# rgoldade/GeometricMultigridPressureSolver

Measured on AMD Instinct MI355X. Metric: V-cycles/sec, higher is better.
Workload: dtype f32

## Files before the change

geometricmultigridpressuresolver_amd/csrc/mgps_internal.h:

```cpp
#pragma once

#include <cstdint>
#include <cstdlib>
#include <cstddef>
#include <memory>
#include <string>
#include <utility>
#include <vector>

#include "mgps.h"

namespace mgps {

constexpr int kTile = 16;

constexpr int kChunkCells = 1024;
constexpr int kWaveChunkCells = 256;
constexpr int kSegCells = 32;

void *hostBigAlloc(size_t bytes);
void hostBigFree(void *p);
void setHostBigAllocator(void *(*alloc)(size_t), void (*release)(void *));
constexpr size_t kBigBlockBytes = size_t(1) << 20;

// ... 60 lines not shown
constexpr int kBandMaxDepth = 4;
constexpr int kBoxMaxNodes = 8192;
constexpr int kBoxMaxList = 4096;
constexpr int kBoxThreads = 1024;
constexpr int kBoxSlots = kBoxMaxList / kBoxThreads;
constexpr int kBoxMaxGeneral = 384;
constexpr int kBoxInfoInts = 16;
enum BoxNode : uint8_t { kBoxSkip = 0, kBoxFrozen = 1, kBoxZero = 2, kBoxGeneral = 3, kBoxSimple = 4, kBoxFrozenOut = 11, kBoxFrozenFar = 12 };
struct BandBoxes {
    int depth = 0;
    RawVec<int32_t> info;
    RawVec<uint32_t> list;
    RawVec<int32_t> general;
    size_t groups() const { return info.size() / kBoxInfoInts; }
};
void buildBandBoxes(const HostLevel &L, int depth, BandBoxes &out);
struct BandBoxesDev {
    int depth = 0, ngroups = 0;
    int32_t *info = nullptr, *general = nullptr;
    uint32_t *list = nullptr;
    size_t listCount = 0, generalInts = 0;
    bool anyGeneral = false;
};
inline bool boxPlaneFits(const Dims &d) { return size_t(d.nx) * size_t(d.ny) < (size_t(1) << 24); }
int compactBandBoxLists(void *stream, int32_t *info, const uint32_t *list, int ngroups, uint32_t *listOut, size_t *newCount);
int orderBandBoxes(void *stream, const Dims &d, const int32_t *info, int ngroups, int32_t *infoOut);

void buildSlabLevel(const HostLevel &G, int z0, int z1, const float *wx, const float *wy, const float *wz,
                    HostLevel &L, const float *rowsIn = nullptr);
int launchBoundaryRows(void *stream, const Dims &d, const uint8_t *labels, const float *wx, const float *wy, const float *wz,
                       const int32_t *cells, int n, float *rows, int *violations);
void checkInteriorCells(const uint8_t *labels, int nx, int ny, int nz, int *pass);
int hierarchyCreate(mgps_hierarchy **out, int nx, int ny, int nz, const uint8_t *labels, int mg_levels,
                    const mgps_options *opt, bool forceCoarseSolver, bool requireShell, const int *window = nullptr);
void chunkListsFromFlags(HostLevel &L, const uint8_t *segAct, int64_t nseg);
constexpr int kRunSizes[4] = {kChunkCells, kWaveChunkCells, 64, kSegCells};
int chooseRunCells(const int64_t nAct[4]);
inline double runCostFactor(int cells) { return cells >= kChunkCells ? 1.0 : cells >= kWaveChunkCells ? 1.02 : cells >= 64 ? 1.13 : 1.22; }
void runListFromFlags(HostLevel &L, const uint8_t *runAct, int64_t nq, int runCells);
void tileListsFromKinds(HostLevel &L, const int64_t *kind, int tileZOffset);
void tileListsFromKinds(HostLevel &L, const int32_t *kind, int tileZOffset);
int hierarchyLight(mgps_hierarchy **out, int nx, int ny, int nz, int levels, const uint8_t *coarsestLabels, const mgps_options &o,
                   bool needCoarseSolver);
void setLastGlobalError(const std::string &msg);
const char *lastGlobalError();
int apiException(const mgps_solver *h) noexcept;
extern void (*gSetHandleError)(const mgps_solver *h, const char *msg) noexcept;
#define MGPS_API_CATCH(h) catch (...) { return ::mgps::apiException(h); }

struct GridP {
    int nx, ny, nz;
    const uint8_t *lab;
    const float *wx, *wy, *wz;
    const int32_t *bnd;
    const float *rows;
    int nbnd;
    const uint8_t *bandDiag;
    int ghostLo, ghostHi;
    const int32_t *chunks;
    int nchunks, chunkCells;
    const int32_t *planeBlocks;
    int nplaneBlocks, planeZc;
    int streaming;
    int sweepPath;
    int xlo, xhi;
    const uint32_t *plainQ;
    const unsigned long long *plainT;
};
inline size_t plainQuadWords(size_t cells) { return ((cells / 4 + 63) / 64) * 2; }
int launchPlainQuads(void *stream, const uint8_t *lab, int nx, int ny, int nz, uint32_t *plainQ, unsigned long long *plainT);
int launchActiveXRange(void *stream, const uint8_t *lab, int nx, size_t cells, int *range);

struct MixScale {
    const float *sigma = nullptr;
    float c1 = 1.f, c2 = 1.f;
};

constexpr int kPlaneCols = 256;
constexpr int kPlaneRows = 16;
constexpr size_t kPlaneSweepMinPlaneBytes = size_t(4) << 20;
constexpr int kSlabEdgePlanes = kBandMaxDepth + 1;
struct PlaneTiles {
    unsigned nbx, nby, nbz;
    constexpr size_t layer() const { return size_t(nbx) * nby; }
    constexpr size_t count() const { return layer() * nbz; }
    constexpr size_t index(int bx, int by, int bz) const { return (size_t(bz) * nby + size_t(by)) * nbx + size_t(bx); }
};
constexpr PlaneTiles planeTiles(int nx, int ny, int nz, int zc)
{
    return PlaneTiles{unsigned((nx + kPlaneCols - 1) / kPlaneCols), unsigned((ny + kPlaneRows - 1) / kPlaneRows), zc > 0 ? unsigned((nz + zc - 1) / zc) : 0u};
}
inline int planeSweepZc(int nx, int ny, int nz)
{
    if ((nx & 3) != 0 || nx < kPlaneCols || ny < kPlaneRows) return 0;
    int zc = 32;
    while (zc > 4 && planeTiles(nx, ny, nz, zc).count() < 1024) zc >>= 1;
    return zc;
}
struct SeamLayout {
    unsigned ny, nseam;
    constexpr size_t planeFloats() const { return size_t(ny) * nseam * 8u; }
    constexpr unsigned entry(unsigned j, unsigned s, unsigned side) const { return (j * nseam + (s - 1u)) * 8u + side * 4u; }
};
constexpr SeamLayout seamLayout(int nx, int ny) { return SeamLayout{unsigned(ny), planeTiles(nx, ny, 0, 0).nbx - 1u}; }

enum StencilOp { OP_JACOBI = 0, OP_RESIDUAL = 1, OP_APPLY = 2 };

size_t stencilSweptCells(const GridP &g);
int stencilKernelOf(const GridP &g);
int forcedStencilPath();
bool setupTimingOn();
bool hostSetupRequested(const mgps_options &o);
int launchStencil(void *stream, StencilOp op, const GridP &g, float *out, const float *x, const float *b, float omega,
                  bool skipInactive);
size_t applyDotPartialCount(const GridP &g);
int launchApplyDot(void *stream, const GridP &g, float *out, const float *x, double *partials, double *resultDev);
int launchBandJacobi(void *stream, const GridP &g, float *x, const float *b, const int32_t *band, int nband,
                     float *bandTmp, float omega, double *dotPartials = nullptr);
unsigned bandScatterBlocks(int nband);
int launchStencilDot(void *stream, StencilOp op, const GridP &g, float *out, const float *x, const float *b, float omega,
                     double *partials, unsigned *nparts);
int launchFoldDot(void *stream, double *partials, unsigned nparts, double *resultDev);
int launchBandBox(void *stream, const GridP &g, const BandBoxesDev &bx, bool closure, const void *src, const float *b, void *dst, void *snap,
                  float omega, bool half = false, const MixScale &ms = MixScale{}, double *dotPartials = nullptr, const void *dotOld = nullptr,
                  bool outClosure = false);
int launchStrokeFront(void *stream, const GridP &g, const BandBoxesDev &bx, float *out, const float *x, const float *b, float *snap, float omega, const uint32_t *keep);
int launchMarkClosure(void *stream, const GridP &g, const BandBoxesDev &bx, uint32_t *bits);
int launchBandBoxCopy(void *stream, const GridP &g, const BandBoxesDev &bx, const void *src, void *dst, bool half = false);
struct HaloList {
    float *buf = nullptr;
    const int32_t *idx = nullptr;
    int n = 0;
    ptrdiff_t base = 0;
};
int launchHaloListPack(void *stream, const HaloList &lo, const HaloList &hi, const float *a0, const float *a1);
int launchHaloListUnpack(void *stream, const HaloList &lo, const HaloList &hi, float *a0, float *a1);
int launchTiledGS(void *stream, const GridP &g, float *x, const float *b, const int32_t *pureTiles, int npure,
                  const int32_t *mixedTiles, int nmixed, const int32_t *tileBndStart, int forward, double *dotPartials = nullptr,
                  float *snap = nullptr, const uint8_t *snapTile = nullptr);
int launchMarkSnapTiles(void *stream, const GridP &g, const BandBoxesDev &bx, uint8_t *tiles);
int launchTiledGSMixed(void *stream, const GridP &g, void *xH, const float *b, const int32_t *pureTiles, int npure, const int32_t *mixedTiles, int nmixed,
                       const int32_t *tileBndStart, int forward, const MixScale &ms);
int launchPatchSimpleCodes(void *stream, uint8_t *codes, const int32_t *band, const uint8_t *bandDiag, int nbnd, int nband);
int launchRestrict(void *stream, const GridP &coarse, float *coarseOut, const float *fine);
bool residualRestrictFits(const GridP &fine, const GridP &coarse);
std::vector<int32_t> planeBlockEdges(const GridP &g, const std::vector<uint8_t> &flags);
bool residualRestrictXFolds(const GridP &fine);
size_t rzxFloats(const GridP &fine);
int launchResidualZ(void *stream, const GridP &fine, float *rz, const float *x, const float *b, const int32_t *edges, int nedges, const float *rEdge = nullptr,
                    bool xfold = false);
int launchRestrictY(void *stream, const GridP &coarse, float *coarseOut, const float *rzx, const GridP &fine);
int launchResidualEdgePlanes(void *stream, const GridP &g, float *r, const float *x, const float *b);
int launchRestrictXY(void *stream, const GridP &coarse, float *coarseOut, const float *rz);
bool mixedPrecisionShapeOk(int nx, int ny, int nz);
int launchStencilMixed(void *stream, StencilOp op, const GridP &g, void *outH, const void *xH, const float *b, float omega, const MixScale &ms,
                       double *dotPartials = nullptr, unsigned *nparts = nullptr);
int launchScaleResult(void *stream, double *resultDev, const float *sigmaDev, float mul);
int launchRestrictMixed(void *stream, const GridP &coarse, float *coarseOut, const void *fineH, float fm);
int launchProlongAddMixed(void *stream, const GridP &fine, void *fineH, const float *coarse, float pm);
int launchFromHalf(void *stream, float *dst, const void *srcH, const float *sigmaDev, float mul, size_t cells);
int launchMixSigma(void *stream, const double *maxAbsDev, float *sigmaDev);
int launchZeroActiveHalf(void *stream, const GridP &g, void *aH);
int launchProlongAdd(void *stream, const GridP &fine, float *fineInOut, const float *coarse, float *snap = nullptr, const uint8_t *snapTile = nullptr);
bool prolongJacobiPlaneFits(const GridP &g);
int launchProlongJacobi(void *stream, const GridP &g, float *out, const float *x, const float *b, const float *coarse, float omega);
int launchBandBoxClosureProlonged(void *stream, const GridP &g, const BandBoxesDev &bx, const float *src, const float *coarse, const float *b, float *snap,
                                  float omega);
size_t planeBlockCount(const GridP &g);
int launchPlaneBlockFlags(void *stream, const GridP &g, uint8_t *flags);
int launchCoarseAssemble(void *stream, int n, int nx, int ny, const int32_t *cells, const int32_t *index, const uint8_t *lab, double *A,
                         const uint8_t *pinned = nullptr);
int launchCoarseNarrow(void *stream, int n, const double *A, float *inv);
int launchCoarseInverseProject(void *stream, int n, float *inv, const int32_t *comp, int ncomp, const int32_t *counts, double *w, double *T);
int launchCoarseSolve(void *stream, int n, const float *inverse, const int32_t *cells, float *x, const float *b,
                      float *gathered);
int launchAxpy(void *stream, const GridP &g, float *dst, const float *src, const float *scaleDev, float scaleHost,
               float sign);
int launchXpay(void *stream, const GridP &g, float *dst, const float *a, const float *s, const float *scaleDev,
               float scaleHost);
int launchScale(void *stream, const GridP &g, float *v, float scale);
int launchDiagInverse(void *stream, const GridP &g, float *dinv);
int launchMulMasked(void *stream, const GridP &g, float *dst, const float *a, const float *b);
constexpr int kReducePartials = 2048;
int launchReduce(void *stream, int kind, const GridP &g, const float *a, const float *b, double *partials,
                 double *resultDev);
int launchCgUpdate(void *stream, const GridP &g, float *x, const float *p, float *r, const float *t, float alpha, double *partials,
                   double *resultDev, const double *alphaDev = nullptr, double *maxAbsDev = nullptr, double *xWide = nullptr, bool xFirst = false);
int launchHalfDot(void *stream, const GridP &g, const void *xH, const float *r, const float *sigmaDev, float mul, double *partials, double *resultDev);
int launchXpayHalf(void *stream, const GridP &g, float *p, const void *xH, const float *sigmaDev, float mul, const float *betaDev, float betaHost);
int launchCgScalars(void *stream, double *scal, float *beta, int init);
int launchStencil64(void *stream, int mode, const GridP &g, double *out, const double *x, const float *b, float *out32,
                    double *partials, size_t capacity, double *resultDev, const float *dx = nullptr);
int launchNarrowSum(void *stream, const GridP &g, float *x32, const double *x64, bool addDx);
int launchCgUpdate64(void *stream, const GridP &g, double *x, const double *p, double *r, const double *t, double alpha, float *r32,
                     double *partials, size_t capacity, double *resultDev);
int launchXpay64(void *stream, const GridP &g, double *p, const float *z, double beta, int first);
int launchWiden(void *stream, double *dst, const float *src, size_t n);
int launchNarrow(void *stream, float *dst, const double *src, size_t n);
int deviceAlloc(void **p, size_t bytes);
int deviceFree(void *p);
void deviceTrim();
struct SlabWindow {
    int own0 = 0, own1 = 0, need = 0;
};
struct WeightView {
    const float *w[3] = {nullptr, nullptr, nullptr}, *lo[3] = {nullptr, nullptr, nullptr}, *hi[3] = {nullptr, nullptr, nullptr};
    int nz = 0, gw = 0, k0 = 0;
};
int launchCoarsenLabels(void *stream, const Dims &fine, const uint8_t *fineLab, uint8_t *coarseLab, int *activeFlag);
int launchAnyActive(void *stream, const Dims &d, const uint8_t *lab, int *activeFlag);
size_t planeCountScratch(size_t plane, int planes);
int launchPlaneCounts(void *stream, const uint8_t *lab, size_t plane, int planes, uint32_t *partials, uint32_t *counts);
int launchShellCheck(void *stream, const Dims &d, const uint8_t *lab, int *badFlag);
int launchMarkBoundary(void *stream, const Dims &d, uint8_t *lab);
size_t scanScratchInts(size_t n);
int launchExclusiveScan(void *stream, const int32_t *in, int32_t *out, size_t n, int32_t *scratch);
int launchBandCandidates(void *stream, const Dims &d, const uint8_t *lab, int32_t *tileKind, uint8_t *tileBits, int32_t *flags, int32_t *rank,
                         int32_t *list, int32_t *scanScratch, const SlabWindow *win = nullptr);
int launchBandMasks(void *stream, const Dims &d, const uint8_t *lab, int width, uint32_t *mask, uint16_t *prefix, int32_t *tileCount, int32_t *tileKind,
                    int *interiorBad, const int32_t *tiles, int ntiles, const SlabWindow *win = nullptr);
int launchBandFill(void *stream, const Dims &d, const uint32_t *mask, const uint16_t *prefix, const int32_t *tileStart, int32_t *band);
int launchBandClassify(void *stream, const Dims &d, const uint8_t *lab, const float *wx, const float *wy, const float *wz, const int32_t *band, int n,
                       uint8_t *diagS, int32_t *general, int *violations);
int launchBandSplit(void *stream, const Dims &d, const uint8_t *lab, const float *wx, const float *wy, const float *wz, const int32_t *band, int n,
                    const uint8_t *diagS, const int32_t *genRank, int32_t *bandDev, uint8_t *bandDiag, int32_t *bandEntry, float *rows);
int launchBandClassify(void *stream, const Dims &d, const uint8_t *lab, const WeightView &wv, const int32_t *band, int n, uint8_t *diagS, int32_t *general,
                       int *violations, const SlabWindow *win);
int launchBandSplit(void *stream, const Dims &d, const uint8_t *lab, const WeightView &wv, const int32_t *band, int n, const uint8_t *diagS, const int32_t *genRank,
                    int32_t *bandDev, uint8_t *bandDiag, int32_t *bandEntry, float *rows);
int launchShellCheckSlab(void *stream, const Dims &d, const uint8_t *lab, bool zFaceLo, bool zFaceHi, int *badFlag);
int launchOwnedFlags(void *stream, const int32_t *band, const int32_t *general, int n, int32_t c0, int32_t c1, int32_t *own, int32_t *ownGen);
int launchBandSplitOwned(void *stream, const int32_t *band, int n, int32_t c0, const uint8_t *diagS, const int32_t *ownRank, const int32_t *ownGenRank,
                         const int32_t *genRank, const float *rowsAll, int32_t *bandOut, uint8_t *diagOut, float *rowsOut);
int launchHaloMark(void *stream, int nx, int ny, int nzOwn, int ghost, const int32_t *info, const uint32_t *list, int ngroups, uint8_t *lo, uint8_t *hi, int *broken);
int launchAddInt(void *stream, int32_t *out, const int32_t *in, int n, int32_t delta);
int launchRebaseBoxes(void *stream, int32_t *info, int ngroups, int32_t delta);
int launchCheckIndex(void *stream, const int32_t *idx, int n, int32_t limit, int *bad);
int launchGhostPlaneBlockFlags(void *stream, const Dims &d, const uint8_t *lab, int k, int zc, uint8_t *flags);
int launchGather(void *stream, const int32_t *rank, const int32_t *start, int n, int32_t *out);
int launchActivityFlags(void *stream, const Dims &d, const uint8_t *lab, uint8_t *chunkFlags, uint8_t *planeFlags, int zc);
int launchCountRuns(void *stream, const uint8_t *segFlags, size_t nseg, int *counts);
int launchFoldRunFlags(void *stream, const uint8_t *segFlags, size_t nseg, int runCells, uint8_t *runFlags);
int launchRunList(void *stream, const Dims &d, const uint8_t *runFlags, size_t nq, int runCells, int32_t *tmpFlags, int32_t *rank, int32_t *scanScratch,
                  int32_t *base, int32_t *list, int listLen);
int launchBandTileList(void *stream, const int32_t *tileStart, int nt, int32_t *flags, int32_t *rank, int32_t *list, int32_t *scanScratch);
int launchTileClassList(void *stream, const Dims &d, const int32_t *kind, int odd, int mixed, int32_t *flags, int32_t *rank, int32_t *list,
                        int32_t *scanScratch, int tkOffset = 0);
int launchByteList(void *stream, const uint8_t *bytes, int n, int32_t *flags, int32_t *rank, int32_t *list, int32_t *scanScratch);
int launchBoxTileList(void *stream, const Dims &d, const int32_t *tileStart, int32_t *flags, int32_t *rank, int32_t *list, int32_t *scanScratch);
int launchBandBoxesCount(void *stream, const Dims &d, const uint8_t *lab, const uint32_t *mask, const uint16_t *prefix, const int32_t *tileStart,
                         const int32_t *bandEntry, const uint8_t *bandDiag, int depth, const int32_t *tiles, int ntiles, int32_t *const counts[3], int *broken,
                         const SlabWindow *win = nullptr);
int launchBandBoxesFill(void *stream, const Dims &d, const uint8_t *lab, const uint32_t *mask, const uint16_t *prefix, const int32_t *tileStart,
                        const int32_t *bandEntry, const uint8_t *bandDiag, int depth, const int32_t *tiles, int ntiles, const int32_t *const at[3],
                        int32_t *info, uint32_t *list, int32_t *general, int *broken, const SlabWindow *win = nullptr);
int enclosedComponentsDevice(void *stream, const Dims &d, const uint8_t *codes, const float *wx, const float *wy, const float *wz, int32_t **cells,
                             int32_t **offsets, int64_t *m, int64_t *cellCount);
struct EncSlab {
    Dims d;
    int32_t base = 0;
    int32_t *parent = nullptr, *flag = nullptr, *pos = nullptr, *rootRank = nullptr, *scan = nullptr;
    uint8_t *open = nullptr, *touch = nullptr;
    int32_t *sendRoots = nullptr, *recvRoots = nullptr;
    unsigned long long *keys = nullptr, *keysSorted = nullptr;
    void *sortTemp = nullptr;
    size_t sortBytes = 0;
    int32_t *payload = nullptr;
    int32_t *candLocal = nullptr;
    int *bad = nullptr;
    int64_t ncand = 0, npairs = 0;
};
int encSlabLabel(void *stream, EncSlab &st, const uint8_t *codes, const float *wx, const float *wy, const float *wz, const uint8_t *labLo,
                 const uint8_t *labHi);
int encSlabCandidates(void *stream, EncSlab &st, const uint8_t *codes, const uint8_t *labHi, const float *wz, int32_t hiFirst, int *badHost);
int encSlabLists(void *stream, EncSlab &st, const int32_t *grank, int64_t m, int32_t **cells, int32_t **offsets, int64_t *cellCount);
void encSlabRelease(EncSlab &st);
constexpr int kEncChunkCells = 4096;
int launchEnclosedSums(void *stream, const float *v, const int32_t *cells, const int32_t *chunks, int nchunks, const int32_t *compChunk, int64_t m,
                       double *partials, double *sum);
int launchEnclosedSums64(void *stream, const double *v, const int32_t *cells, const int32_t *chunks, int nchunks, const int32_t *compChunk, int64_t m,
                         double *partials, double *sum);
int launchEnclosedSubtract(void *stream, float *v, const int32_t *cells, const int32_t *chunks, int nchunks, const int32_t *count, const double *sum);
int launchEnclosedSubtract64(void *stream, double *v, const int32_t *cells, const int32_t *chunks, int nchunks, const int32_t *count, const double *sum);
int launchEnclosedRanks(void *stream, int32_t *rank, const int32_t *cells, const int32_t *chunks, int nchunks);
int launchWidenAdd(void *stream, double *x64, const float *x32, size_t n);
int launchZero(void *stream, float *a, size_t count);
int launchZeroInactive(void *stream, const GridP &g, float *a);
int launchZeroActive(void *stream, const GridP &g, float *a, bool ghostPlanes = false);
int launchPack(void *stream, float *buf, const float *a, const int32_t *idx, int n);
int launchUnpack(void *stream, float *a, const float *buf, const int32_t *idx, int n);

}

struct mgps_coupling;
struct mgps_fields_slab;
namespace mgps {
void couplingExtents(const mgps_coupling *c, int e[3]);
bool couplingOnSlab(const mgps_coupling *c, int planes[2], int *rank, int *size);
constexpr int kCouplingCommFailed = -1;
int couplingApply64(mgps_coupling *c, void *stream, double *t, const double *p, double *dotDev);
int couplingResidual64(mgps_coupling *c, void *stream, double *r, const double *x, float *r32, double *norm2Dev);
int coupledSolveRefusal(mgps_solver *h, mgps_coupling *coupling, const char *fn);
bool fieldsSlabWindow(const mgps_fields_slab *d, const char *fn);
}

namespace mgps {
// ... 31 lines not shown
```

geometricmultigridpressuresolver_amd/csrc/mgps_kernels.hip:

```cpp
#include <hip/hip_runtime.h>
#include <hip/hip_fp16.h>

#include <algorithm>
#include <cstdlib>
#include <type_traits>

#include "mgps_internal.h"

namespace mgps {

namespace {

typedef float v4f __attribute__((ext_vector_type(4)));
typedef unsigned char v4b __attribute__((ext_vector_type(4)));
__device__ __forceinline__ float4 streamLoad4(const float *p)
{
    const v4f v = __builtin_nontemporal_load(reinterpret_cast<const v4f *>(p));
    return make_float4(v.x, v.y, v.z, v.w);
}
__device__ __forceinline__ uchar4 streamLoad4(const uint8_t *p)
{
    const v4b v = __builtin_nontemporal_load(reinterpret_cast<const v4b *>(p));
    return make_uchar4(v.x, v.y, v.z, v.w);
}
// ... 618 lines not shown
        lc = lcn;
        lcn = lcq;
        buf ^= 1;
    }
}

template <bool XF>
__global__ __launch_bounds__(64 * kPlaneRows, 8) void residualZKernel(GridP g, float *__restrict__ rz, const float *__restrict__ x,
                                                                     const float *__restrict__ b, unsigned nbx, unsigned nby, int zc,
                                                                     const int32_t *__restrict__ blocks, const float *__restrict__ rEdge,
                                                                     float *__restrict__ seam)
{
    __shared__ float plane[2][kPlaneBufFloats];
    const PlaneTile t = planeTile(g, nbx, nby, zc, blocks);
    const bool live = t.live, valid = t.valid, rowTop = t.rowTop, rowBot = t.rowBot, colL = t.colL, colR = t.colR;
    const size_t sz = size_t(t.sz);
    const int k0 = t.k0, k1 = t.k1;
    const int ks = max(k0 - 1, 0), ke = min(k1, g.nz - 1);
    const unsigned offL = unsigned(t.jc) * unsigned(g.nx) + unsigned(min(max(t.ic, g.xlo), max(g.xhi - 4, g.xlo)));
    float *const mine0 = plane[0] + (t.ty + 1) * kPlanePitch + 4 + t.lane * 4;
    const unsigned offHy = (rowTop && t.jc > 0) ? offL - unsigned(g.nx) : (rowBot && t.jc < g.ny - 1) ? offL + unsigned(g.nx) : offL;
    {
        const float4 xm = gLoad4(t.planeOf(x, ks - 1), offL);
        *reinterpret_cast<float4 *>(mine0 + kPlaneBufFloats) = keepIf(xm, live);
    }
    const float *xk = t.planeOf(x, ks);
    float4 xc = gLoad4(xk, offL);
    float4 xp = gLoad4(t.planeOf(x, ks + 1), offL);
    float4 hy = gLoad4(xk, offHy);
    const bool useHx = live && t.hasHx();
    const unsigned offHx = t.offHx(useHx, offL);
    float hx = gLoad1(xk, offHx);
    constexpr float w0 = 0.125f, w1 = 0.375f, w2 = 0.375f, w3 = 0.125f;
    float accPrev[4] = {0.f, 0.f, 0.f, 0.f}, accCur[4] = {0.f, 0.f, 0.f, 0.f};
    const unsigned rowX = t.rowS * (unsigned(g.nx) >> 1) + t.bx * 128u;
    const bool storeX = t.i < g.nx && t.j < g.ny && t.ic >= g.xlo - 4 && t.ic < g.xhi + 4;
    const bool seamL = colL && t.bx > 0, seamR = colR && t.i + 4 < g.nx;
    const bool seamW = valid && (seamL || seamR);
    const SeamLayout sl = seamLayout(g.nx, g.ny);
    auto storeFolded = [&](int K, bool nt) {
        const float4 v = keepIf(make_float4(accPrev[0], accPrev[1], accPrev[2], accPrev[3]), valid);
        storeXFolded(v, scalarBase(rz + size_t(K) * (sz >> 1)), rowX + 2u * laneHere(), storeX, nt, scalarBase(seam + size_t(K) * sl.planeFloats()),
                     colL ? sl.entry(t.rowS, t.bx, 1u) : sl.entry(t.rowS, t.bx + 1u, 0u), seamW);
    };
    if (rEdge && k0 == 0 && g.ghostLo) {
        const float4 e = gLoad4(scalarBase(rEdge - ptrdiff_t(sz)), offL);
        accCur[0] = w0 * e.x;
        accCur[1] = w0 * e.y;
        accCur[2] = w0 * e.z;
        accCur[3] = w0 * e.w;
    }
    const unsigned long long *const pt = g.plainT;
    unsigned long long pw = pt ? plainWord64(pt, t.plainIdx(ks)) : 0ull;
    int buf = 0;
    for (int k = ks; k <= ke; ++k) {
        float *me = mine0 + buf * kPlaneBufFloats;
        xc = keepIf(xc, live);
        stagePlane(me, t, xc, keepIf(hy, live), hx, useHx);
        const float *bk = t.planeOf(b, k);
        const uint8_t *lk = scalarBase(g.lab + size_t(k) * sz);
        const float *xn = t.planeOf(x, k + 1), *xq2 = t.planeOf(x, k + 2);
        unsigned lcw = 0u;
        if (!plainLane(pw)) lcw = gLoadCodesWnt(lk, offL);
        if (pt) pw = plainWord64(pt, t.plainIdx(min(k + 1, g.nz - 1)));
        const float4 bc = gLoad4nt(bk, offL);
        const float hxn = gLoad1(xn, offHx);
        float4 hyn = hy;
        if (rowTop || rowBot) hyn = gLoad4(xn, offHy);
        const float4 xq = gLoad4(xq2, offL);
        __syncthreads();
        const StagedPlane n = readStaged(me, mine0 + (buf ^ 1) * kPlaneBufFloats);
        float res[4];
        simpleQuad<OP_RESIDUAL>(n.xl, xc, n.xr, n.ym, n.yp, n.zm, xp, bc, lcw, 0.f, res);
        if (k & 1) {
#pragma unroll
            for (int e = 0; e < 4; ++e) {
                accPrev[e] = accCur[e] + w2 * res[e];
                accCur[e] = w0 * res[e];
            }
        } else {
#pragma unroll
            for (int e = 0; e < 4; ++e) {
                accPrev[e] += w3 * res[e];
                accCur[e] += w1 * res[e];
            }
            if (XF) {
                if (k >= k0 + 2) storeFolded((k >> 1) - 1, true);
            } else if (valid && k >= k0 + 2) {
                gStore4nt(scalarBase(rz + size_t((k >> 1) - 1) * sz), offL, make_float4(accPrev[0], accPrev[1], accPrev[2], accPrev[3]));
            }
        }
        xc = xp;
        xp = xq;
        hy = hyn;
        hx = hxn;
        buf ^= 1;
    }
    if (k1 == g.nz) {
        if (valid && rEdge && g.ghostHi) {
            const float4 e = gLoad4(scalarBase(rEdge + ptrdiff_t(g.nz) * ptrdiff_t(sz)), offL);
            accPrev[0] += w3 * e.x;
            accPrev[1] += w3 * e.y;
            accPrev[2] += w3 * e.z;
            accPrev[3] += w3 * e.w;
        }
        if (XF) storeFolded((g.nz >> 1) - 1, false);
        else if (valid) gStore4(rz + size_t((g.nz >> 1) - 1) * sz, offL, make_float4(accPrev[0], accPrev[1], accPrev[2], accPrev[3]));
    }
}

template <bool XF>
__global__ __launch_bounds__(64 * kPlaneRows) void residualZEdgeKernel(GridP g, float *__restrict__ rz, const float *__restrict__ x, const float *__restrict__ b,
                                                                      unsigned nbx, unsigned nby, int zc, const int32_t *__restrict__ edges,
                                                                      float *__restrict__ seam)
{
    const unsigned side = unsigned(edges[blockIdx.x]) & 1u;
    PlaneCoords t;
    planeCoords(t, g, unsigned(edges[blockIdx.x]) >> 1, nbx, nby, zc);
    const int lane = t.lane, i = t.i, j = t.j;
    const int k = side == 0 ? t.k0 - 1 : t.k1, K = side == 0 ? (t.k0 >> 1) : (t.k1 >> 1) - 1;
    const float wz = 0.125f;
    if (k < 0 || k >= g.nz) return;
    if (j >= g.ny) return;
    if (!XF && i >= g.nx) return;
    const bool live = i < g.nx && i >= g.xlo && i < g.xhi;
    const size_t sy = size_t(g.nx), sz = size_t(g.nx) * g.ny;
    const size_t c = size_t(k) * sz + size_t(j) * sy + i;
    const float4 zero4 = make_float4(0.f, 0.f, 0.f, 0.f);
    const size_t cym = j > 0 ? c - sy : c, cyp = j < g.ny - 1 ? c + sy : c, czm = k > 0 ? c - sz : c, czp = k < g.nz - 1 ? c + sz : c;
    const float4 xc = live ? *reinterpret_cast<const float4 *>(x + c) : zero4;
    const float4 ym = live ? *reinterpret_cast<const float4 *>(x + cym) : zero4, yp = live ? *reinterpret_cast<const float4 *>(x + cyp) : zero4;
    const float4 zm = live ? *reinterpret_cast<const float4 *>(x + czm) : zero4, zp = live ? *reinterpret_cast<const float4 *>(x + czp) : zero4;
    const float4 bc = live ? *reinterpret_cast<const float4 *>(b + c) : zero4;
    const unsigned labw = live ? *reinterpret_cast<const unsigned *>(g.lab + c) : 0x01010101u * unsigned(MGPS_EXTERIOR_CELL);
    float left = __shfl_up(xc.w, 1), right = __shfl_down(xc.x, 1);
    if (lane == 0) left = (live && i > 0) ? x[c - 1] : 0.f;
    if (lane == kWave - 1 || i + 4 >= g.nx) right = (live && i + 4 < g.nx) ? x[c + 4] : 0.f;
    if (!XF && !live) return;
    float res[4];
    simpleQuad<OP_RESIDUAL>(left, xc, right, ym, yp, zm, zp, bc, labw, 0.f, res);
    const float4 wr = make_float4(wz * res[0], wz * res[1], wz * res[2], wz * res[3]);
    if (!XF) {
        *reinterpret_cast<float4 *>(rz + size_t(K) * sz + size_t(j) * sy + i) = wr;
        return;
    }
    const bool seamL = lane == 0 && t.bx > 0, seamR = lane == kWave - 1 && i + 4 < g.nx;
    const SeamLayout sl = seamLayout(g.nx, g.ny);
    const unsigned offX = unsigned(j) * (unsigned(g.nx) >> 1) + (unsigned(i) >> 1);
    const unsigned seamOff = seamL ? sl.entry(unsigned(j), t.bx, 1u) : sl.entry(unsigned(j), t.bx + 1u, 0u);
    const bool storeX = i < g.nx && i >= g.xlo - 4 && i < g.xhi + 4, seamW = live && (seamL || seamR);
    storeXFolded(keepIf(wr, live), rz + size_t(K) * (sz >> 1), offX, storeX, false, seam + size_t(K) * sl.planeFloats(), seamOff, seamW);
}

template <int OP, bool DOT = false>
__global__ void stencilScalarKernel(GridP g, float *__restrict__ out, const float *__restrict__ x,
                                    const float *__restrict__ b, float omega, double *__restrict__ dotPartials = nullptr)
{
    const size_t n = size_t(g.nx) * g.ny * g.nz;
    const size_t c = size_t(blockIdx.x) * blockDim.x + threadIdx.x;
    double acc = 0.0;
    if (c < n) {
        const unsigned l = g.lab[c];
        const float xc = x[c];
        if (!simpleCell(l)) out[c] = inactiveValue<OP>(xc);
        else {
            const size_t sy = size_t(g.nx), sz = size_t(g.nx) * g.ny;
            const float diag = simpleDiag(l);
            const float lap = diag * xc - (x[c - 1] + x[c + 1] + x[c - sy] + x[c + sy] + x[c - sz] + x[c + sz]);
            const float bc = OP == OP_APPLY ? 0.f : b[c];
            const float res = epilogueRcp<OP>(xc, bc, lap, simpleRcp(diag), omega);
            out[c] = res;
            acc = dotTerm<OP>(xc, bc, res);
        }
    }
    if (DOT) blockDotStore(acc, dotPartials, blockIdx.x);
}

template <int OP, bool DOT = false, class TX = float>
__global__ void boundaryOpKernel(GridP g, TX *__restrict__ out, const TX *__restrict__ x,
                                 const float *__restrict__ b, float omega, unsigned nblocks, double *__restrict__ dotPartials = nullptr,
                                 MixScale ms = MixScale{})
{
    constexpr bool kMixed = !std::is_same<TX, float>::value;
    const unsigned block = remapBlock(blockIdx.x, nblocks);
    const int t = int(block * blockDim.x + threadIdx.x);
    double acc = 0.0;
    if (t < g.nbnd) {
        const size_t c = size_t(g.bnd[t]);
        float lap, diag;
        boundaryRow(g, [&](size_t p) { return Cell<TX>::load1(x + p); }, t, c, lap, diag);
        const float xc = Cell<TX>::load1(x + c), bc = OP == OP_APPLY ? 0.f : b[c];
        float res;
        if (kMixed) {
            const float bm = mixRhsScale(ms);
            res = OP == OP_JACOBI ? xc + omega * ((bm * bc - lap) / diag) : OP == OP_RESIDUAL ? bm * bc - ms.c2 * lap : lap;
        } else
            res = epilogue<OP>(xc, bc, lap, diag, omega);
        Cell<TX>::store1(out + c, res);
        acc = dotTerm<OP>(xc, bc, kMixed ? __half2float(toHalfSat(res)) : res);
    }
    if (DOT) blockDotStore(acc, dotPartials, blockIdx.x);
}

__global__ void bandComputeKernel(GridP g, const float *__restrict__ x, const float *__restrict__ b,
                                  const int32_t *__restrict__ band, int nband, float *__restrict__ tmp, float omega,
                                  unsigned nblocks)
{
    const unsigned block = remapBlock(blockIdx.x, nblocks);
    const int t = int(block * blockDim.x + threadIdx.x);
    if (t >= nband) return;
    const size_t c = size_t(band[t]);
    const size_t sy = size_t(g.nx), sz = size_t(g.nx) * g.ny;
    const float xc = x[c];
    float lap, diag;
    if (t >= g.nbnd) {
        diag = float(g.bandDiag[t]);
        lap = diag * xc - (x[c - 1] + x[c + 1] + x[c - sy] + x[c + sy] + x[c - sz] + x[c + sz]);
        tmp[t] = xc + omega * ((b[c] - lap) * simpleRcp(diag));
    } else {
        boundaryRow(g, [&](size_t p) { return x[p]; }, t, c, lap, diag);
        tmp[t] = xc + omega * ((b[c] - lap) / diag);
    }
}
template <bool DOT = false, class TX = float>
__global__ void bandScatterKernel(TX *__restrict__ x, const int32_t *__restrict__ band, int nband,
                                  const float *__restrict__ tmp, unsigned nblocks, const float *__restrict__ b = nullptr,
                                  double *__restrict__ dotPartials = nullptr)
{
    const int t = int(remapBlock(blockIdx.x, nblocks) * blockDim.x + threadIdx.x);
    double acc = 0.0;
    if (t < nband) {
        const int32_t c = band[t];
        const float v = tmp[t];
        if (DOT) {
            const float stored = std::is_same<TX, float>::value ? v : __half2float(toHalfSat(v));
            acc = (double(stored) - double(Cell<TX>::load1(x + c))) * double(b[c]);
        }
        Cell<TX>::store1(x + c, v);
    }
    if (DOT) blockDotStore(acc, dotPartials, blockIdx.x);
}

__device__ __forceinline__ bool boxBand(unsigned cls) { return cls >= kBoxGeneral && cls <= kBoxSimple + 6; }

template <class TX, bool CLOSURE, bool DOT, bool GEN, bool XZERO, bool PRO = false>
__device__ __forceinline__ void bandBoxBody(const GridP &g, const TX *__restrict__ src, const float *__restrict__ b, TX *dst,
                                            TX *__restrict__ snap, const int32_t *__restrict__ info, const uint32_t *__restrict__ list,
                                            const int32_t *__restrict__ general, float omega, int depth, const MixScale &ms,
                                            double *__restrict__ dotPartials, const TX *dotOld, int outClosure, unsigned group, unsigned slot,
                                            const float *__restrict__ coarse = nullptr)
{
    static_assert(!PRO || (CLOSURE && !XZERO && std::is_same<TX, float>::value), "the prolonged input: closure mode, fp32");
    constexpr bool kMixed = !std::is_same<TX, float>::value;
    constexpr int kGenRows = GEN ? kBoxMaxGeneral : 1;
    __shared__ __attribute__((aligned(16))) float val[2][kBoxMaxNodes];
    __shared__ float grow[7][kGenRows];
    __shared__ float gbv[kGenRows];
    __shared__ uint16_t gnode[kGenRows], gring[kGenRows];
    constexpr bool kStaged = PRO && !GEN;
    constexpr int kCoarseBoxWords = 2048, kCoarseSlots = kCoarseBoxWords / kBoxThreads;
    __shared__ float cbox[kStaged ? kCoarseBoxWords : 1];
    const int32_t *gip = info + kBoxInfoInts * size_t(group);
    int gi[kBoxInfoInts];
#pragma unroll
    for (int q = 0; q < kBoxInfoInts; ++q) gi[q] = __builtin_amdgcn_readfirstlane(gip[q]);
    const int rx = gi[1] & 255, ry = (gi[1] >> 8) & 255, sxy = rx * ry;
    const unsigned sy = unsigned(g.nx), sz = unsigned(g.nx) * unsigned(g.ny);
    const ptrdiff_t origin = gi[0];
    if (!XZERO) src += origin;
    b += origin;
    if (dst) dst += origin;
    if (CLOSURE && snap) snap += origin;
    if (DOT) dotOld += origin;
    const uint32_t *U = list + gi[2];
    const int ngen = GEN ? gi[5] : 0, nList = CLOSURE ? gi[7] : gi[3];
    const int H = depth + (CLOSURE ? 1 : 0);
    const float bm = kMixed ? mixRhsScale(ms) : 1.f;
    const int tid = threadIdx.x;
    auto nodeOf = [&](uint32_t e) { return int(__umul24((e >> 10) & 31u, unsigned(sxy)) + __umul24((e >> 5) & 31u, unsigned(rx)) + (e & 31u)); };
    auto cellOf = [&](uint32_t e) { return (e & 31u) + __umul24((e >> 5) & 31u, sy) + __umul24((e >> 10) & 31u, sz); };
    auto rd = [&](const TX *base, unsigned c) { return Cell<TX>::load1(reinterpret_cast<const TX *>(reinterpret_cast<const char *>(base) + c * unsigned(sizeof(TX)))); };
    auto rdf = [&](const float *base, unsigned c) { return *reinterpret_cast<const float *>(reinterpret_cast<const char *>(base) + c * 4u); };
    auto wr = [&](TX *base, unsigned c, float v) { Cell<TX>::store1(reinterpret_cast<TX *>(reinterpret_cast<char *>(base) + c * unsigned(sizeof(TX))), v); };
    int cbLo[3] = {0, 0, 0}, cbN[3] = {1, 1, 1};
    bool staged = false;
    if (kStaged) {
        const int o3[3] = {int(origin % g.nx), int((origin / g.nx) % g.ny), int(origin / sz)};
        const int r3[3] = {rx, ry, (gi[1] >> 16) & 255}, cn3[3] = {g.nx >> 1, g.ny >> 1, g.nz >> 1};
#pragma unroll
        for (int a = 0; a < 3; ++a) {
            cbLo[a] = min(max((o3[a] - 1) >> 1, 0), cn3[a] - 2);
            cbN[a] = min(max((o3[a] + r3[a] - 2) >> 1, 0), cn3[a] - 2) + 2 - cbLo[a];
        }
        staged = cbN[0] * cbN[1] * cbN[2] <= kCoarseBoxWords;
    }
    uint32_t ue[kBoxSlots];
    float bv[kBoxSlots];
    {
        float cv[kCoarseSlots];
        if (kStaged && staged) {
            const unsigned csy = unsigned(g.nx >> 1), csz = csy * unsigned(g.ny >> 1);
            const unsigned nxy = unsigned(cbN[0] * cbN[1]), nbox = nxy * unsigned(cbN[2]);
            const float *cb = scalarBase(coarse + (size_t(cbLo[2]) * csz + size_t(cbLo[1]) * csy + size_t(cbLo[0])));
#pragma unroll
            for (int m = 0; m < kCoarseSlots; ++m) {
                const unsigned q = unsigned(tid) + unsigned(m) * kBoxThreads, qq = q < nbox ? q : 0u;
// ... 1727 lines not shown
    return int(hipGetLastError());
}
__global__ __launch_bounds__(256) void zeroChunksHalfKernel(__half *__restrict__ a, const int32_t *__restrict__ chunks, int chunkCells, size_t nq)
{
    size_t q;
    if (!listQuad(chunks, chunkCells, blockIdx.x, q)) return;
    if (q < nq) reinterpret_cast<uint2 *>(a)[q] = make_uint2(0u, 0u);
}
int launchZeroActiveHalf(void *stream, const GridP &g, void *aH)
{
    const size_t n = size_t(g.nx) * g.ny * g.nz;
    if (!g.chunks || (n & 3) != 0) return int(hipMemsetAsync(aH, 0, n * sizeof(__half), static_cast<hipStream_t>(stream)));
    const unsigned nb = unsigned(g.nchunks) / unsigned(kChunkCells / g.chunkCells);
    if (nb > 0) zeroChunksHalfKernel<<<nb, 256, 0, static_cast<hipStream_t>(stream)>>>(static_cast<__half *>(aH), g.chunks, g.chunkCells, n >> 2);
    return int(hipGetLastError());
}

int launchTiledGS(void *stream, const GridP &g, float *x, const float *b, const int32_t *pureTiles, int npure,
                  const int32_t *mixedTiles, int nmixed, const int32_t *tileBndStart, int forward, double *dotPartials, float *snap, const uint8_t *snapTile)
{
    hipStream_t s = static_cast<hipStream_t>(stream);
    if (snap && !snapTile) return int(hipErrorInvalidValue);
    if (nmixed > 0 && npure > 0 && nmixed + npure <= 768) {
        if (dotPartials) tiledGSBothKernel<true><<<unsigned(nmixed + npure), 256, 0, s>>>(g, x, b, mixedTiles, nmixed, pureTiles, tileBndStart, forward, dotPartials, snap, snapTile);
        else tiledGSBothKernel<<<unsigned(nmixed + npure), 256, 0, s>>>(g, x, b, mixedTiles, nmixed, pureTiles, tileBndStart, forward, nullptr, snap, snapTile);
        return int(hipGetLastError());
    }
    if (dotPartials) {
        if (nmixed > 0) tiledGSMixedKernel<true><<<unsigned(nmixed), 256, 0, s>>>(g, x, b, mixedTiles, tileBndStart, forward, dotPartials, MixScale{}, snap, snapTile);
        if (npure > 0) tiledGSPureKernel<true><<<unsigned(npure), 256, 0, s>>>(g, x, b, pureTiles, forward, dotPartials + nmixed, MixScale{}, snap, snapTile);
        return int(hipGetLastError());
    }
    if (nmixed > 0) tiledGSMixedKernel<<<unsigned(nmixed), 256, 0, s>>>(g, x, b, mixedTiles, tileBndStart, forward, nullptr, MixScale{}, snap, snapTile);
    if (npure > 0) tiledGSPureKernel<<<unsigned(npure), 256, 0, s>>>(g, x, b, pureTiles, forward, nullptr, MixScale{}, snap, snapTile);
    return int(hipGetLastError());
}

int launchTiledGSMixed(void *stream, const GridP &g, void *xH, const float *b, const int32_t *pureTiles, int npure, const int32_t *mixedTiles, int nmixed,
                       const int32_t *tileBndStart, int forward, const MixScale &ms)
{
    hipStream_t s = static_cast<hipStream_t>(stream);
    __half *x = static_cast<__half *>(xH);
    if (nmixed > 0) tiledGSMixedKernel<false, __half><<<unsigned(nmixed), 256, 0, s>>>(g, x, b, mixedTiles, tileBndStart, forward, nullptr, ms);
    if (npure > 0) tiledGSPureKernel<false, __half><<<unsigned(npure), 256, 0, s>>>(g, x, b, pureTiles, forward, nullptr, ms);
    return int(hipGetLastError());
}

__global__ void patchSimpleCodesKernel(uint8_t *codes, const int32_t *band, const uint8_t *bandDiag, int nbnd, int nband)
{
    const int t = nbnd + int(blockIdx.x * blockDim.x + threadIdx.x);
    if (t >= nband) return;
    const int32_t c = band[t];
    if (codes[c] == MGPS_BOUNDARY_CELL) codes[c] = uint8_t(kCodeSimple + bandDiag[t]);
}

int launchPatchSimpleCodes(void *stream, uint8_t *codes, const int32_t *band, const uint8_t *bandDiag, int nbnd, int nband)
{
    if (nband > nbnd)
        patchSimpleCodesKernel<<<blocksFor(size_t(nband - nbnd), 256), 256, 0, static_cast<hipStream_t>(stream)>>>(codes, band, bandDiag, nbnd, nband);
    return int(hipGetLastError());
}

int launchRestrict(void *stream, const GridP &coarse, float *coarseOut, const float *fine)
{
    const size_t n = size_t(coarse.nx) * coarse.ny * coarse.nz;
    int kc = 16;
    const unsigned nbx = (coarse.nx + 63) / 64, nby = (coarse.ny + 7) / 8;
    while (kc > 4 && size_t(nbx) * nby * ((coarse.nz + kc - 1) / kc) < 8192) kc >>= 1;
    const unsigned nbz = (coarse.nz + kc - 1) / kc;
    const bool runsWin = coarse.chunks && double(coarse.nchunks) * coarse.chunkCells * 1.3 * runCostFactor(coarse.chunkCells) < 0.8 * double(n);
    if (!runsWin && coarse.nx >= 64 && coarse.nz >= kc && nbx * nby * nbz >= 2048u) {
        if ((coarse.nx & 1) == 0) restrictTileKernel<<<nbx * nby * nbz, 256, 0, static_cast<hipStream_t>(stream)>>>(coarse, coarseOut, fine, kc, nbx, nby);
        else restrictMarchKernel<<<nbx * nby * nbz, 256, 0, static_cast<hipStream_t>(stream)>>>(coarse, coarseOut, fine, kc, nbx, nby);
        return int(hipGetLastError());
    }
    const unsigned nb = coarse.chunks ? unsigned(size_t(coarse.nchunks) * size_t(coarse.chunkCells) / 256) : blocksFor(n, 256);
    if (nb > 0) restrictKernel<<<nb, 256, 0, static_cast<hipStream_t>(stream)>>>(coarse, coarseOut, fine);
    return int(hipGetLastError());
}

bool residualRestrictFits(const GridP &fine, const GridP &coarse)
{
    return fine.planeZc >= 4 && (fine.planeZc & 1) == 0 && (fine.nz & 1) == 0 && coarse.nx >= 64 && (coarse.nx & 1) == 0 && 2 * coarse.nx == fine.nx &&
           2 * coarse.ny == fine.ny && 2 * coarse.nz == fine.nz;
}
std::vector<int32_t> planeBlockEdges(const GridP &g, const std::vector<uint8_t> &flags)
{
    const int zc = g.planeZc > 0 ? g.planeZc : 1;
    const PlaneTiles pt = planeTiles(g.nx, g.ny, g.nz, zc);
    const size_t layer = pt.layer(), nbz = pt.nbz;
    std::vector<int32_t> edges;
    for (size_t bid = 0; bid < flags.size() && bid < layer * nbz; ++bid) {
        if (flags[bid]) continue;
        const size_t bz = bid / layer;
        if (bz > 0 && flags[bid - layer]) edges.push_back(int32_t(2 * bid));
        if (bz + 1 < nbz && flags[bid + layer]) edges.push_back(int32_t(2 * bid + 1));
    }
    return edges;
}
int launchResidualEdgePlanes(void *stream, const GridP &g, float *r, const float *x, const float *b)
{
    const size_t sz = size_t(g.nx) * g.ny;
    for (int side = 0; side < 2; ++side) {
        if (!(side == 0 ? g.ghostLo : g.ghostHi)) continue;
        const int k = side == 0 ? 0 : g.nz - 1;
        GridP p = g;
        p.nz = 1;
        p.lab = g.lab + size_t(k) * sz;
        p.plainQ = nullptr;
        p.plainT = nullptr;
        p.ghostLo = (k > 0 || g.ghostLo) ? 1 : 0;
        p.ghostHi = (k < g.nz - 1 || g.ghostHi) ? 1 : 0;
        p.chunks = nullptr;
        p.nchunks = 0;
        p.planeBlocks = nullptr;
        p.nplaneBlocks = 0;
        p.planeZc = 0;
        p.sweepPath = 1;
        p.nbnd = 0;
        p.streaming = 0;
        const int e = launchStencil(stream, OP_RESIDUAL, p, r + size_t(k) * sz, x + size_t(k) * sz, b + size_t(k) * sz, 0.f, true);
        if (e) return e;
    }
    if (g.nbnd > 0) {
        const unsigned nb = blocksFor(size_t(g.nbnd), 256);
        boundaryOpKernel<OP_RESIDUAL><<<nb, 256, 0, static_cast<hipStream_t>(stream)>>>(g, r, x, b, 0.f, nb);
    }
    return int(hipGetLastError());
}
bool residualRestrictXFolds(const GridP &fine) { return fine.nbnd == 0; }
static size_t rzxGridFloats(const GridP &fine) { return (size_t(fine.nx) * fine.ny * fine.nz / 4 + 3) & ~size_t(3); }
size_t rzxFloats(const GridP &fine) { return rzxGridFloats(fine) + size_t(fine.nz / 2) * seamLayout(fine.nx, fine.ny).planeFloats(); }
int launchResidualZ(void *stream, const GridP &fine, float *rz, const float *x, const float *b, const int32_t *edges, int nedges, const float *rEdge, bool xfold)
{
    if (xfold && fine.nbnd > 0) return int(hipErrorInvalidValue);
    const int zc = fine.planeZc;
    const PlaneTiles pt = planeTiles(fine.nx, fine.ny, fine.nz, zc);
    const unsigned nbx = pt.nbx, nby = pt.nby;
    hipStream_t s = static_cast<hipStream_t>(stream);
    const bool list = fine.planeBlocks != nullptr;
    const unsigned nb = list ? unsigned(fine.nplaneBlocks) : unsigned(pt.count());
    if (xfold) {
        float *seam = rz + rzxGridFloats(fine);
        if (nb > 0) residualZKernel<true><<<nb, 64 * kPlaneRows, 0, s>>>(fine, rz, x, b, nbx, nby, zc, list ? fine.planeBlocks : nullptr, rEdge, seam);
        if (list && nedges > 0) residualZEdgeKernel<true><<<unsigned(nedges), 64 * kPlaneRows, 0, s>>>(fine, rz, x, b, nbx, nby, zc, edges, seam);
        return int(hipGetLastError());
    }
    if (nb > 0) residualZKernel<false><<<nb, 64 * kPlaneRows, 0, s>>>(fine, rz, x, b, nbx, nby, zc, list ? fine.planeBlocks : nullptr, rEdge, nullptr);
    if (list && nedges > 0) residualZEdgeKernel<false><<<unsigned(nedges), 64 * kPlaneRows, 0, s>>>(fine, rz, x, b, nbx, nby, zc, edges, nullptr);
    if (fine.nbnd > 0)
        for (int phase = 0; phase < 4; ++phase) residualZGeneralKernel<<<blocksFor(size_t(fine.nbnd), 256), 256, 0, s>>>(fine, rz, x, b, phase);
    return int(hipGetLastError());
}
int launchRestrictXY(void *stream, const GridP &coarse, float *coarseOut, const float *rz)
{
    int kc = 16;
    const unsigned nbx = (coarse.nx + kRtI - 1) / kRtI, nby = (coarse.ny + kRtJ - 1) / kRtJ;
    while (kc > 1 && size_t(nbx) * nby * ((coarse.nz + kc - 1) / kc) < 8192) kc >>= 1;
    const unsigned nbz = (coarse.nz + kc - 1) / kc;
    restrictXYKernel<<<nbx * nby * nbz, 256, 0, static_cast<hipStream_t>(stream)>>>(coarse, coarseOut, rz, kc, nbx, nby);
    return int(hipGetLastError());
}

int launchRestrictY(void *stream, const GridP &coarse, float *coarseOut, const float *rzx, const GridP &fine)
{
    int kc = 16;
    const unsigned nbx = (coarse.nx + kRyI - 1) / kRyI, nby = (coarse.ny + kRyJ - 1) / kRyJ;
    while (kc > 1 && size_t(nbx) * nby * ((coarse.nz + kc - 1) / kc) < 8192) kc >>= 1;
    const unsigned nbz = (coarse.nz + kc - 1) / kc;
    restrictYKernel<<<nbx * nby * nbz, 256, 0, static_cast<hipStream_t>(stream)>>>(coarse, coarseOut, rzx, rzx + rzxGridFloats(fine), kc, nbx, nby);
    return int(hipGetLastError());
}

int launchRestrictMixed(void *stream, const GridP &coarse, float *coarseOut, const void *fineH, float fm)
{
    const __half *fine = static_cast<const __half *>(fineH);
    const size_t n = size_t(coarse.nx) * coarse.ny * coarse.nz;
    const int kc = 16;
    const unsigned nbx = (coarse.nx + 63) / 64, nby = (coarse.ny + 7) / 8, nbz = (coarse.nz + kc - 1) / kc;
    const bool runsWin = coarse.chunks && double(coarse.nchunks) * coarse.chunkCells * 1.3 * runCostFactor(coarse.chunkCells) < 0.8 * double(n);
    if (!runsWin && coarse.nx >= 64 && coarse.nz >= kc && nbx * nby * nbz >= 2048u) {
        restrictMarchKernel<__half><<<nbx * nby * nbz, 256, 0, static_cast<hipStream_t>(stream)>>>(coarse, coarseOut, fine, kc, nbx, nby, fm);
        return int(hipGetLastError());
    }
    const unsigned nb = coarse.chunks ? unsigned(size_t(coarse.nchunks) * size_t(coarse.chunkCells) / 256) : blocksFor(n, 256);
    if (nb > 0) restrictKernel<__half><<<nb, 256, 0, static_cast<hipStream_t>(stream)>>>(coarse, coarseOut, fine, fm);
    return int(hipGetLastError());
}

int launchProlongAddMixed(void *stream, const GridP &fine, void *fineH, const float *coarse, float pm)
{
    const int npj = fine.ny / 2 - 1;
    const int kp0 = 0, kp1 = fine.nz / 2 - 2;
    const size_t total = size_t(fine.nx >> 2) * npj * size_t(std::max(kp1 - kp0 + 1, 0));
    const unsigned nb = blocksFor(total, 256);
    if (nb > 0)
        prolongAddBlockKernel<__half><<<nb, 256, 0, static_cast<hipStream_t>(stream)>>>(fine, static_cast<__half *>(fineH), coarse, nb, npj, kp0, total, pm);
    return int(hipGetLastError());
}
bool mixedPrecisionShapeOk(int nx, int ny, int nz) { return (nx & 3) == 0 && nx >= 8 && (ny & 1) == 0 && (nz & 1) == 0 && ny >= 4 && nz >= 2; }

int launchProlongAdd(void *stream, const GridP &fine, float *fineInOut, const float *coarse, float *snap, const uint8_t *snapTile)
{
    if (snap && !snapTile) return int(hipErrorInvalidValue);
    const size_t n = size_t(fine.nx) * fine.ny * fine.nz;
    const bool runsWin = fine.chunks && double(fine.nchunks) * fine.chunkCells * 3.4 * runCostFactor(fine.chunkCells) < 0.8 * double(n);
    if (!runsWin && (fine.nx & 3) == 0 && fine.nx >= 8 && (fine.ny & 1) == 0 && (fine.nz & 1) == 0 && fine.ny >= 4 && fine.nz >= 2) {
        const int npj = fine.ny / 2 - 1;
        const int kp0 = fine.ghostLo ? -1 : 0, kp1 = fine.ghostHi ? fine.nz / 2 - 1 : fine.nz / 2 - 2;
        const size_t total = size_t(fine.nx >> 2) * npj * size_t(std::max(kp1 - kp0 + 1, 0));
        const unsigned nb = blocksFor(total, 256);
        if (nb > 0)
            prolongAddBlockKernel<<<nb, 256, 0, static_cast<hipStream_t>(stream)>>>(fine, fineInOut, coarse, nb, npj, kp0, total, 1.f, snap, snapTile);
    } else if ((fine.nx & 3) == 0 && fine.nx >= 8) {
        const unsigned nb = fine.chunks ? unsigned(fine.nchunks) / unsigned(kChunkCells / fine.chunkCells) : blocksFor(n >> 2, 256);
        if (nb > 0) prolongAddQuadKernel<<<nb, 256, 0, static_cast<hipStream_t>(stream)>>>(fine, fineInOut, coarse, nb, snap, snapTile);
    } else
        prolongAddKernel<<<blocksFor(n, 256), 256, 0, static_cast<hipStream_t>(stream)>>>(fine, fineInOut, coarse, snap, snapTile);
    return int(hipGetLastError());
}

bool prolongJacobiPlaneFits(const GridP &g)
{
    return g.planeZc > 0 && (g.planeZc & 1) == 0 && (g.nx & 3) == 0 && g.nx >= 8 && (g.ny & 1) == 0 && (g.nz & 1) == 0 && g.ny >= 4 && g.nz >= 4 &&
           !g.ghostLo && !g.ghostHi;
}
int launchProlongJacobi(void *stream, const GridP &g, float *out, const float *x, const float *b, const float *coarse, float omega)
{
    if (!prolongJacobiPlaneFits(g) || !out || !x || !coarse || out == x || g.nbnd > 0) return int(hipErrorInvalidValue);
    const int zc = g.planeZc;
    const PlaneTiles pt = planeTiles(g.nx, g.ny, g.nz, zc);
    const unsigned nb = g.planeBlocks ? unsigned(g.nplaneBlocks) : unsigned(pt.count());
    if (nb > 0) prolongJacobiPlaneKernel<<<nb, 64 * kPlaneRows, 0, static_cast<hipStream_t>(stream)>>>(g, out, x, b, coarse, omega, pt.nbx, pt.nby, zc, g.planeBlocks);
    return int(hipGetLastError());
}

__global__ __launch_bounds__(256) void planeBlockFlagsKernel(const int32_t *__restrict__ blocks, int n, uint8_t *__restrict__ flags)
{
    const int t = int(blockIdx.x * blockDim.x + threadIdx.x);
    if (t < n) flags[blocks[t]] = 1;
}
size_t planeBlockCount(const GridP &g)
{
    return planeTiles(g.nx, g.ny, g.nz, g.planeZc > 0 ? g.planeZc : 1).count();
}
int launchPlaneBlockFlags(void *stream, const GridP &g, uint8_t *flags)
{
    if (!g.planeBlocks || g.nplaneBlocks <= 0) return 0;
    planeBlockFlagsKernel<<<blocksFor(size_t(g.nplaneBlocks), 256), 256, 0, static_cast<hipStream_t>(stream)>>>(g.planeBlocks, g.nplaneBlocks, flags);
    return int(hipGetLastError());
}

__global__ __launch_bounds__(256) void coarseAssembleKernel(int n, int nx, int ny, const int32_t *__restrict__ cells, const int32_t *__restrict__ index,
                                                            const uint8_t *__restrict__ lab, const uint8_t *__restrict__ pinned, double *__restrict__ A)
{
    const int r = int(blockIdx.x * blockDim.x + threadIdx.x);
    if (r >= n) return;
    if (pinned && pinned[r]) {
        A[size_t(r) * n + r] = 1.0;
        return;
    }
    const ptrdiff_t c = cells[r], off[6] = {-1, 1, -ptrdiff_t(nx), ptrdiff_t(nx), -ptrdiff_t(nx) * ny, ptrdiff_t(nx) * ny};
    double diag = 0.0;
#pragma unroll
    for (int q = 0; q < 6; ++q) {
        const unsigned l = lab[c + off[q]];
        if (activeLabel(l)) {
            const int32_t u = index[c + off[q]];
            if (!(pinned && pinned[u])) A[size_t(r) * n + u] = -1.0;
            diag += 1.0;
        } else if (l == MGPS_DIRICHLET_CELL)
            diag += 1.0;
    }
    A[size_t(r) * n + r] = diag;
}
__global__ __launch_bounds__(256) void coarseNarrowKernel(int n, const double *__restrict__ A, float *__restrict__ inv)
{
    const size_t t = blockIdx.x * size_t(blockDim.x) + threadIdx.x;
    if (t >= size_t(n) * n) return;
    const size_t r = t / n, c = t - r * n;
    inv[t] = float(r <= c ? A[t] : A[c * n + r]);
}
int launchCoarseAssemble(void *stream, int n, int nx, int ny, const int32_t *cells, const int32_t *index, const uint8_t *lab, double *A, const uint8_t *pinned)
{
    coarseAssembleKernel<<<blocksFor(size_t(n), 256), 256, 0, static_cast<hipStream_t>(stream)>>>(n, nx, ny, cells, index, lab, pinned, A);
    return int(hipGetLastError());
}
__global__ __launch_bounds__(256) void coarseProjRowKernel(int n, const float *__restrict__ inv, const int32_t *__restrict__ comp,
                                                           const int32_t *__restrict__ counts, double *__restrict__ w)
{
    const int row = blockIdx.x * (blockDim.x / kWave) + threadIdx.x / kWave;
    const int lane = threadIdx.x & (kWave - 1);
    if (row >= n) return;
    const int c = comp[row];
    double acc = 0.0;
    if (c >= 0)
        for (int k = lane; k < n; k += kWave)
            if (comp[k] == c) acc += double(inv[size_t(row) * n + k]);
#pragma unroll
    for (int off = kWave / 2; off > 0; off >>= 1) acc += __shfl_down(acc, off);
    if (lane == 0) w[row] = c >= 0 ? acc / double(counts[c]) : 0.0;
}
__global__ __launch_bounds__(64) void coarseProjMeanKernel(int n, int ncomp, const int32_t *__restrict__ comp, const int32_t *__restrict__ counts,
                                                          const double *__restrict__ w, double *__restrict__ T)
{
    const int c = blockIdx.x * blockDim.x + threadIdx.x;
// ... 778 lines not shown
```

geometricmultigridpressuresolver_amd/csrc/mgps_solver.hip:

```cpp
#include <hip/hip_runtime.h>

#include <dlfcn.h>

#include <algorithm>
#include <chrono>
#include <cmath>
#include <cstdio>
#include <cstring>
#include <functional>
#include <limits>
#include <string>
#include <atomic>
#include <mutex>
#include <thread>
#include <unordered_map>
#include <map>
#include <memory>
#include <vector>

#include "mgps_fields.h"
#include "mgps_internal.h"

using namespace mgps;

namespace {
inline hipError_t cacheMalloc(void **p, size_t bytes) { return hipError_t(mgps::deviceAlloc(p, bytes)); }
inline hipError_t cacheFree(void *p) { return hipError_t(mgps::deviceFree(p)); }
}

namespace {

struct DevLevel {
    Dims d;
    GridP g{};
    uint8_t *codes = nullptr;
    float *x = nullptr, *b = nullptr;
    float *r = nullptr, *tmp = nullptr;
    int32_t *band = nullptr;
    int nband = 0;
    int nbndGeneral = 0;
    float *bandTmp = nullptr;
    float *rows = nullptr;
    uint8_t *bandDiag = nullptr;
    int32_t *pure[2] = {nullptr, nullptr}, *mixed[2] = {nullptr, nullptr};
    int npure[2] = {0, 0}, nmixed[2] = {0, 0};
    int32_t *tileBndStart = nullptr;
    int z0 = 0, z1 = 0;
    int32_t *bandPlane[4] = {nullptr, nullptr, nullptr, nullptr};
    int nbandPlane[4] = {0, 0, 0, 0};
    float *packBuf[4] = {nullptr, nullptr, nullptr, nullptr};
    int32_t *chunks = nullptr, *planeBlocks = nullptr;
    int edgeChunks = 0, edgePlaneBlocks = 0;
    BandBoxesDev bandBoxes;
    uint8_t *planeFlags = nullptr;
    int32_t *rzEdges = nullptr;
    int nrzEdges = 0;
    float *rz = nullptr;
    uint8_t *snapTile = nullptr;
    uint32_t *keepBits = nullptr;
    struct BoxHalo {
        int32_t *sendIdx[2] = {nullptr, nullptr}, *recvIdx[2] = {nullptr, nullptr};
        int nsend[2] = {0, 0}, nrecv[2] = {0, 0};
        float *sendBuf[2] = {nullptr, nullptr}, *recvBuf[2] = {nullptr, nullptr};
    } halo;
    bool boxForm = false;
    bool hasBandPlanes = false;
    GridP gBox{};
    float *extRows = nullptr;
    uint32_t *plainQ = nullptr;
    unsigned long long *plainT = nullptr;
    int elo = 0;
};

}

struct mgps_solver {
    mgps_hierarchy *hier = nullptr;
    std::vector<mgps_hierarchy *> retiredHier;
    mgps_options opt{};
    bool useGS = false;
    int device = 0;
    hipStream_t stream = nullptr;
    std::vector<DevLevel> lv;
    float *w[3] = {nullptr, nullptr, nullptr};
    bool weightsBorrowed = false;
    int cn = 0;
    float *cinv = nullptr, *cvec = nullptr;
    std::shared_ptr<void> cinvShared;
    int32_t *ccells = nullptr;
    bool tailOfSlabRun = false;
    double *partials = nullptr, *resultDev = nullptr, *resultHost = nullptr;
    double *dotPartials = nullptr;
    double *cg64[4] = {nullptr, nullptr, nullptr, nullptr};
    mgps_coupling *coupling = nullptr;
    bool gatherDot = false;
    unsigned dotUsed = 0;
    size_t dotCapacity = 0;
    double *dotTarget = nullptr;
    double *cgScal = nullptr;
    float *pcg[4] = {nullptr, nullptr, nullptr, nullptr};
    float *dinv = nullptr;
    void *mixX = nullptr, *mixTmp = nullptr, *mixR = nullptr;
    float *mixSigma = nullptr;
    int mixExp = 0;
    double *mixMax = nullptr;
    void *mixResult = nullptr;
    std::vector<void *> userGrids;
    int ghost = 1;
    bool dist = false;
    mgps_comm comm{};
    int64_t exchanges = 0;
    std::vector<int> splits;
    int distLevels = 0;
    int totalLevels = 0;
    int requestedLevels = 0;
    mgps_solver *tail = nullptr;
    float *tailX = nullptr, *tailB = nullptr;
    bool profiling = false;
    bool stageProfiling = false;
    std::vector<hipEvent_t> profEvents;
    size_t profUsed = 0;
    int profSweeps = 0;
    struct StageMark {
        int stage, level;
    };
    std::vector<StageMark> stageMarks;
    std::vector<hipEvent_t> stageEvents;
    double stageMs[6] = {0, 0, 0, 0, 0, 0};
    double stageMsFine[6] = {0, 0, 0, 0, 0, 0};
    double stageMsFineLast[6] = {0, 0, 0, 0, 0, 0};
    int stageCycles = 0;
    int64_t encM = 0, encCells = 0;
    int32_t *encCellList = nullptr, *encOffsets = nullptr, *encChunks = nullptr, *encCompChunk = nullptr, *encCount = nullptr;
    std::vector<int32_t> encCountHost;
    int encNChunks = 0;
    double *encPartials = nullptr, *encSum = nullptr;
    std::vector<double> encSumHost;
    float *encB = nullptr;
    std::string lastError = "";
};

namespace {
void setHandleError(const mgps_solver *h, const char *msg) noexcept
{
    try {
        const_cast<mgps_solver *>(h)->lastError = msg;
    } catch (...) {
    }
}
const bool handleErrorHookInstalled = [] {
    mgps::gSetHandleError = setHandleError;
    return true;
}();
}

namespace {

int failH(mgps_solver *h, int code, const std::string &msg)
{
    static std::mutex guard;
    std::lock_guard<std::mutex> lock(guard);
    if (h) h->lastError = msg;
    else setLastGlobalError(msg);
    return code;
}

#define MGPS_HIP(h, call)                                                                                 \
    do {                                                                                                  \
        hipError_t e_ = (call);                                                                           \
        if (e_ != hipSuccess)                                                                             \
            return failH(h, MGPS_ERR_HIP, std::string(#call) + ": " + hipGetErrorString(e_));             \
    } while (0)
#define MGPS_LAUNCH(h, call)                                                                              \
    do {                                                                                                  \
        int e_ = (call);                                                                                  \
        if (e_ != 0)                                                                                      \
            return failH(h, MGPS_ERR_HIP, std::string(#call) + ": " + hipGetErrorString(hipError_t(e_))); \
    } while (0)
#define MGPS_TRY(call)                \
    do {                              \
        int s_ = (call);              \
        if (s_ != MGPS_OK) return s_; \
    } while (0)
#define MGPS_COMM(h, call)                                                           \
    do {                                                                             \
        int s_ = (call);                                                             \
        if (s_ != 0) return failH(h, MGPS_ERR_COMM, std::string(#call) + " failed"); \
    } while (0)
#define MGPS_COUPLE(h, call)                                                                                                     \
    do {                                                                                                                         \
        int e_ = (call);                                                                                                         \
        if (e_ == mgps::kCouplingCommFailed) return failH(h, MGPS_ERR_COMM, std::string(#call) + ": the all-reduce of g failed"); \
        if (e_ != 0) return failH(h, MGPS_ERR_HIP, std::string(#call) + ": " + hipGetErrorString(hipError_t(e_)));              \
    } while (0)


struct DeviceCache {
    struct Block {
        void *p;
        uint64_t age;
    };
    using FreeMap = std::multimap<std::pair<int, size_t>, Block>;
    std::mutex guard;
    FreeMap free;
    std::unordered_map<void *, std::pair<int, size_t>> live;
    uint64_t clock = 0;
    struct PerDevice {
        size_t cached = 0, cap = 0;
        bool capKnown = false;
        std::map<uint64_t, FreeMap::iterator> byAge;
    };
    std::map<int, PerDevice> dev;
// ... 47 lines not shown
        const auto it = c.free.find({dev, want});
        if (it != c.free.end()) {
            *p = it->second.p;
            D.cached -= want;
            D.byAge.erase(it->second.age);
            c.free.erase(it);
            return hipSuccess;
        }
    }
    if (needCap) {
        const size_t cap = deviceCapOfCurrent();
        std::lock_guard<std::mutex> lock(c.guard);
        DeviceCache::PerDevice &D = c.dev[dev];
        if (!D.capKnown) {
            D.cap = cap;
            D.capKnown = true;
        }
    }
    hipError_t e = hipMalloc(p, want);
    if (e != hipSuccess) {
        (void)hipGetLastError();
        std::vector<void *> drop;
        {
            std::lock_guard<std::mutex> lock(c.guard);
            deviceTrimLocked(c, drop);
        }
        for (void *b : drop) (void)hipFree(b);
        e = hipMalloc(p, want);
    }
    if (e != hipSuccess) return int(e);
    std::lock_guard<std::mutex> lock(c.guard);
    c.live[*p] = {dev, want};
    return hipSuccess;
}
int deviceFree(void *p)
{
    if (!p) return hipSuccess;
    DeviceCache &c = deviceCache();
    std::vector<void *> drop;
    {
        std::lock_guard<std::mutex> lock(c.guard);
        const auto it = c.live.find(p);
        if (it == c.live.end()) drop.push_back(p);
        else {
            DeviceCache::PerDevice &D = c.dev[it->second.first];
            if (it->second.second > D.cap) {
                c.live.erase(it);
                drop.push_back(p);
            } else {
                const uint64_t age = c.clock++;
                D.byAge[age] = c.free.emplace(it->second, DeviceCache::Block{p, age});
                D.cached += it->second.second;
                while (D.cached > D.cap && !D.byAge.empty()) {
                    const auto oldest = D.byAge.begin()->second;
                    drop.push_back(oldest->second.p);
                    D.cached -= oldest->first.second;
                    c.live.erase(oldest->second.p);
                    c.free.erase(oldest);
                    D.byAge.erase(D.byAge.begin());
                }
            }
        }
    }
    hipError_t e = hipSuccess;
    for (void *b : drop) {
        const hipError_t eb = hipFree(b);
        if (eb != hipSuccess) e = eb;
    }
    return int(e);
}
void deviceTrim()
{
    DeviceCache &c = deviceCache();
    std::vector<void *> drop;
    {
        std::lock_guard<std::mutex> lock(c.guard);
        deviceTrimLocked(c, drop);
    }
    for (void *b : drop) (void)hipFree(b);
}
}
namespace {

template <class T>
int devAlloc(mgps_solver *h, T **p, size_t count, bool zero)
{
    *p = nullptr;
    if (count == 0) count = 1;
    hipError_t e = cacheMalloc(reinterpret_cast<void **>(p), count * sizeof(T));
    if (e != hipSuccess) return failH(h, MGPS_ERR_ALLOC, std::string("hipMalloc: ") + hipGetErrorString(e));
    if (zero) MGPS_HIP(h, hipMemsetAsync(*p, 0, count * sizeof(T), h->stream));
    return MGPS_OK;
}

template <class T, class A>
int devUpload(mgps_solver *h, T **p, const std::vector<T, A> &v)
{
    MGPS_TRY(devAlloc(h, p, v.size(), false));
    if (!v.empty()) MGPS_HIP(h, hipMemcpy(*p, v.data(), v.size() * sizeof(T), hipMemcpyHostToDevice));
    return MGPS_OK;
}

int gridAlloc(mgps_solver *h, float **p, const Dims &d)
{
    const size_t plane = size_t(d.nx) * d.ny;
    float *base = nullptr;
    MGPS_TRY(devAlloc(h, &base, (size_t(d.nz) + 2 * size_t(h->ghost)) * plane, true));
    *p = base + size_t(h->ghost) * plane;
    return MGPS_OK;
}
void gridFree(const mgps_solver *h, float *p, const Dims &d)
{
    if (p) (void)cacheFree(p - size_t(h->ghost) * size_t(d.nx) * d.ny);
}

void freeAll(mgps_solver *h)
{
    if (!h) return;
    (void)hipSetDevice(h->device);
    (void)hipDeviceSynchronize();
    if (h->tail) freeAll(h->tail);
    for (auto &L : h->lv) {
        (void)cacheFree(L.codes);
        gridFree(h, L.x, L.d);
        gridFree(h, L.b, L.d);
        gridFree(h, L.r, L.d);
        gridFree(h, L.tmp, L.d);
        (void)cacheFree(L.band);
        (void)cacheFree(L.bandTmp);
        (void)cacheFree(L.rows);
        (void)cacheFree(L.bandDiag);
        for (int c = 0; c < 2; ++c) {
            (void)cacheFree(L.pure[c]);
            (void)cacheFree(L.mixed[c]);
        }
        (void)cacheFree(L.tileBndStart);
        for (int q = 0; q < 4; ++q) {
            (void)cacheFree(L.bandPlane[q]);
            (void)cacheFree(L.packBuf[q]);
        }
        (void)cacheFree(L.chunks);
        (void)cacheFree(L.planeBlocks);
        for (int q = 0; q < 2; ++q) {
            (void)cacheFree(L.halo.sendIdx[q]);
            (void)cacheFree(L.halo.recvIdx[q]);
            (void)cacheFree(L.halo.sendBuf[q]);
            (void)cacheFree(L.halo.recvBuf[q]);
        }
        (void)cacheFree(L.extRows);
        (void)cacheFree(L.bandBoxes.info);
        (void)cacheFree(L.bandBoxes.list);
        (void)cacheFree(L.planeFlags);
        (void)cacheFree(L.keepBits);
        (void)cacheFree(L.snapTile);
        (void)cacheFree(L.rz);
        (void)cacheFree(L.rzEdges);
        (void)cacheFree(L.bandBoxes.general);
        (void)cacheFree(L.plainQ);
        (void)cacheFree(L.plainT);
    }
    for (int a = 0; a < 3 && !h->weightsBorrowed; ++a) (void)cacheFree(h->w[a]);
    if (!h->cinvShared) (void)cacheFree(h->cinv);
    (void)cacheFree(h->cvec);
    (void)cacheFree(h->ccells);
    (void)cacheFree(h->partials);
    (void)cacheFree(h->resultDev);
    (void)cacheFree(h->dotPartials);
    (void)cacheFree(h->cgScal);
    (void)cacheFree(h->mixX);
    (void)cacheFree(h->mixTmp);
    (void)cacheFree(h->mixR);
    (void)cacheFree(h->mixSigma);
    (void)cacheFree(h->mixMax);
    for (double *g64 : h->cg64)
        if (g64) (void)cacheFree(g64 - size_t(h->lv[0].d.nx) * h->lv[0].d.ny);
    if (h->resultHost) (void)hipHostFree(h->resultHost);
    if (!h->lv.empty()) {
        for (int q = 0; q < 4; ++q) gridFree(h, h->pcg[q], h->lv[0].d);
        gridFree(h, h->dinv, h->lv[0].d);
    }
    for (void *p : {(void *)h->encCellList, (void *)h->encOffsets, (void *)h->encChunks, (void *)h->encCompChunk, (void *)h->encPartials, (void *)h->encSum, (void *)h->encCount})
        (void)cacheFree(p);
    if (!h->lv.empty()) gridFree(h, h->encB, h->lv[0].d);
    for (void *p : h->userGrids) (void)cacheFree(p);
    for (hipEvent_t e : h->profEvents) (void)hipEventDestroy(e);
    for (hipEvent_t e : h->stageEvents) (void)hipEventDestroy(e);
    mgps_hierarchy_destroy(h->hier);
    for (mgps_hierarchy *r : h->retiredHier) mgps_hierarchy_destroy(r);
    delete h;
}

int checkLevel(mgps_solver *h, int level, const char *who)
{
    if (!h) return failH(nullptr, MGPS_ERR_INVALID_ARGUMENT, std::string(who) + ": NULL handle");
    if (level < 0 || level >= int(h->lv.size()))
        return failH(h, MGPS_ERR_INVALID_ARGUMENT, std::string(who) + ": level out of range");
    (void)hipSetDevice(h->device);
    return MGPS_OK;
}


enum GhostMode { GHOST_NONE = 0, GHOST_FULL = 1, GHOST_BAND = 2 };

int exchangeGhosts(mgps_solver *h, int l, float *a, GhostMode mode = GHOST_FULL, hipStream_t on = nullptr)
{
    if (!h->dist || mode == GHOST_NONE) return MGPS_OK;
    DevLevel &L = h->lv[l];
    const size_t plane = size_t(L.d.nx) * L.d.ny;
    const bool lo = h->comm.rank > 0, hi = h->comm.rank < h->comm.size - 1;
    if (mode == GHOST_BAND && !L.hasBandPlanes) mode = GHOST_FULL;
    if (mode == GHOST_FULL) {
        const size_t bytes = plane * sizeof(float);
        ++h->exchanges;
        MGPS_COMM(h, h->comm.exchange(h->comm.user, lo ? a : nullptr, bytes, lo ? a - plane : nullptr, bytes,
                                      hi ? a + (size_t(L.d.nz) - 1) * plane : nullptr, bytes,
                                      hi ? a + size_t(L.d.nz) * plane : nullptr, bytes, on ? on : h->stream));
        return MGPS_OK;
    }
    const int *n = L.nbandPlane;
    if (lo) MGPS_LAUNCH(h, launchPack(h->stream, L.packBuf[0], a, L.bandPlane[0], n[0]));
    if (hi) MGPS_LAUNCH(h, launchPack(h->stream, L.packBuf[2], a, L.bandPlane[2], n[2]));
    ++h->exchanges;
    MGPS_COMM(h, h->comm.exchange(h->comm.user, lo ? L.packBuf[0] : nullptr, size_t(n[0]) * sizeof(float),
                                  lo ? L.packBuf[1] : nullptr, size_t(n[1]) * sizeof(float),
                                  hi ? L.packBuf[2] : nullptr, size_t(n[2]) * sizeof(float),
                                  hi ? L.packBuf[3] : nullptr, size_t(n[3]) * sizeof(float), h->stream));
    if (lo) MGPS_LAUNCH(h, launchUnpack(h->stream, a, L.packBuf[1], L.bandPlane[1], n[1]));
    if (hi) MGPS_LAUNCH(h, launchUnpack(h->stream, a, L.packBuf[3], L.bandPlane[3], n[3]));
    return MGPS_OK;
}


int haloListExchange(mgps_solver *h, int l, float *a0, float *a1, bool withPlane)
{
    DevLevel &L = h->lv[l];
    DevLevel::BoxHalo &H = L.halo;
    const size_t plane = size_t(L.d.nx) * L.d.ny, G = size_t(h->ghost);
    const bool lo = h->comm.rank > 0, hi = h->comm.rank < h->comm.size - 1;
    if (!lo && !hi) return MGPS_OK;
    const size_t per = a1 ? 2 : 1;
    HaloList sLo, sHi, rLo, rHi;
    if (lo) {
        sLo = HaloList{H.sendBuf[0], H.sendIdx[0], H.nsend[0], 0};
        rLo = HaloList{H.recvBuf[0], H.recvIdx[0], H.nrecv[0], -ptrdiff_t(G * plane)};
    }
    if (hi) {
        sHi = HaloList{H.sendBuf[1], H.sendIdx[1], H.nsend[1], 0};
        rHi = HaloList{H.recvBuf[1], H.recvIdx[1], H.nrecv[1], ptrdiff_t(size_t(L.d.nz) * plane)};
    }
    MGPS_LAUNCH(h, launchHaloListPack(h->stream, sLo, sHi, a0, a1));
    const size_t pb = plane * sizeof(float);
    const size_t sb[2] = {size_t(H.nsend[0]) * per * sizeof(float), size_t(H.nsend[1]) * per * sizeof(float)};
    const size_t rb[2] = {size_t(H.nrecv[0]) * per * sizeof(float), size_t(H.nrecv[1]) * per * sizeof(float)};
    ++h->exchanges;
    if (withPlane && h->comm.exchange2) {
        mgps_xfer2 seg[4];
        if (lo) {
            seg[0] = mgps_xfer2{{a0, H.sendBuf[0]}, {pb, sb[0]}};
            seg[1] = mgps_xfer2{{a0 - plane, H.recvBuf[0]}, {pb, rb[0]}};
        }
        if (hi) {
            seg[2] = mgps_xfer2{{a0 + (size_t(L.d.nz) - 1) * plane, H.sendBuf[1]}, {pb, sb[1]}};
            seg[3] = mgps_xfer2{{a0 + size_t(L.d.nz) * plane, H.recvBuf[1]}, {pb, rb[1]}};
        }
        MGPS_COMM(h, h->comm.exchange2(h->comm.user, lo ? &seg[0] : nullptr, lo ? &seg[1] : nullptr, hi ? &seg[2] : nullptr, hi ? &seg[3] : nullptr, h->stream));
    } else {
        if (withPlane) MGPS_TRY(exchangeGhosts(h, l, a0, GHOST_FULL));
        MGPS_COMM(h, h->comm.exchange(h->comm.user, lo ? H.sendBuf[0] : nullptr, sb[0], lo ? H.recvBuf[0] : nullptr, rb[0], hi ? H.sendBuf[1] : nullptr, sb[1],
                                      hi ? H.recvBuf[1] : nullptr, rb[1], h->stream));
    }
    MGPS_LAUNCH(h, launchHaloListUnpack(h->stream, rLo, rHi, a0, a1));
    return MGPS_OK;
}

double *takeDotSink(mgps_solver *h, unsigned n)
{
    double *p = h->dotPartials + h->dotUsed;
    h->dotUsed += n;
    return p;
}

bool levelHasBoxes(const mgps_solver *h, int l)
{
    if (h->lv[l].boxForm) return true;
    return h->lv[l].bandBoxes.ngroups > 0 && h->lv[l].bandBoxes.depth == h->opt.band_iterations;
}
int boxesUnavailable(mgps_solver *h, int l)
{
    if (l == 0 && h->opt.precision == 1)
        return failH(h, MGPS_ERR_INVALID_ARGUMENT,
                     "options.precision = 1 (mixed precision) needs the fused band stage on the fine level: with band_iterations = 4 a band "
                     "box of this domain holds more than " + std::to_string(kBoxMaxGeneral) + " general cells (use band_iterations <= 3)");
    if (h->opt.print_stats) std::printf("  level %d: band boxes exceed %d general cells per group; band stage pass by pass\n", l, kBoxMaxGeneral);
    return MGPS_OK;
}
const GridP &boxGrid(const mgps_solver *h, int l) { return h->lv[l].boxForm ? h->lv[l].gBox : h->lv[l].g; }

int bandPasses(mgps_solver *h, int l, float *x, const float *b, GhostMode first, bool dot = false)
{
    DevLevel &L = h->lv[l];
    if (levelHasBoxes(h, l)) {
        double *s = dot ? takeDotSink(h, unsigned(L.bandBoxes.ngroups)) : nullptr;
        if (x == L.r || b == L.r) return failH(h, MGPS_ERR_INVALID_ARGUMENT, "band stage: the level's residual grid is its scratch");
        if (L.boxForm) MGPS_TRY(haloListExchange(h, l, x, const_cast<float *>(b), true));
        MGPS_LAUNCH(h, launchBandBox(h->stream, boxGrid(h, l), L.bandBoxes, false, x, b, L.r, nullptr, h->opt.jacobi_weight, false, MixScale{}, s, x));
        MGPS_LAUNCH(h, launchBandBoxCopy(h->stream, L.g, L.bandBoxes, L.r, x));
        return MGPS_OK;
    }
    for (int it = 0; it < h->opt.band_iterations; ++it) {
        MGPS_TRY(exchangeGhosts(h, l, x, it == 0 ? first : GHOST_BAND));
        double *sink = dot && L.nband > 0 ? takeDotSink(h, bandScatterBlocks(L.nband)) : nullptr;
        MGPS_LAUNCH(h, launchBandJacobi(h->stream, L.g, x, b, L.band, L.nband, L.bandTmp, h->opt.jacobi_weight, sink));
    }
    return MGPS_OK;
}

enum Stage { ST_BAND = 0, ST_SMOOTH = 1, ST_RESIDUAL = 2, ST_RESTRICT = 3, ST_COARSE = 4, ST_PROLONG = 5 };
const char *const kStageNames[6] = {"Boundary smoother time", "Smoother time", "Compute residual time", "Downsample time", "Direct solve time",
                                    "Upsample and add time"};
inline bool stageTimingOn(const mgps_solver *h) { return (h->opt.print_stats || h->stageProfiling) && !h->tailOfSlabRun; }
void stageFlush(mgps_solver *h);
struct StageScope {
    mgps_solver *h;
    bool on;
    size_t slot = 0;
    StageScope(mgps_solver *hh, int stage, int level) : h(hh), on(stageTimingOn(hh))
    {
        if (!on) return;
        if (h->stageMarks.size() >= 65536) stageFlush(h);
        slot = h->stageMarks.size();
        while (h->stageEvents.size() < 2 * (slot + 1)) {
            hipEvent_t e = nullptr;
            if (hipEventCreate(&e) != hipSuccess) {
                on = false;
                return;
            }
            h->stageEvents.push_back(e);
        }
        h->stageMarks.push_back({stage, level});
        (void)hipEventRecord(h->stageEvents[2 * slot], h->stream);
    }
    ~StageScope()
    {
        if (on) (void)hipEventRecord(h->stageEvents[2 * slot + 1], h->stream);
    }
};
void stageFlush(mgps_solver *h)
{
    if (h->stageMarks.empty()) return;
    (void)hipStreamSynchronize(h->stream);
    for (size_t q = 0; q < h->stageMarks.size(); ++q) {
        float ms = 0.f;
        if (hipEventElapsedTime(&ms, h->stageEvents[2 * q], h->stageEvents[2 * q + 1]) != hipSuccess) continue;
        h->stageMs[h->stageMarks[q].stage] += ms;
        if (h->stageMarks[q].level == 0) h->stageMsFine[h->stageMarks[q].stage] += ms;
        if (h->opt.print_stats && (!h->dist || h->comm.rank == 0))
            std::printf("      level %d  %s: %.4f ms\n", h->stageMarks[q].level, kStageNames[h->stageMarks[q].stage], double(ms));
    }
    h->stageMarks.clear();
}

void stageCycleDone(mgps_solver *h)
{
    if (stageTimingOn(h)) ++h->stageCycles;
    if (h->opt.print_stats) stageFlush(h);
}

int profMark(mgps_solver *h, bool begin)
{
    if (begin && h->profUsed + 2 > h->profEvents.size()) {
        hipEvent_t e0, e1;
        MGPS_HIP(h, hipEventCreate(&e0));
        MGPS_HIP(h, hipEventCreate(&e1));
        h->profEvents.push_back(e0);
        h->profEvents.push_back(e1);
    }
    MGPS_HIP(h, hipEventRecord(h->profEvents[h->profUsed + (begin ? 0 : 1)], h->stream));
    if (!begin) h->profUsed += 2;
    return MGPS_OK;
}
template <class Launch> int timedSweep(mgps_solver *h, bool on, int sweeps, Launch &&launch)
{
    if (on) MGPS_TRY(profMark(h, true));
    MGPS_TRY(launch());
    if (!on) return MGPS_OK;
    MGPS_TRY(profMark(h, false));
    h->profSweeps += sweeps;
    return MGPS_OK;
}
inline bool sweepTimed(const mgps_solver *h, int l) { return h->profiling && l == 0; }

int gsHalfSweep(mgps_solver *h, int l, float *x, const float *b, int odd, int forward, GhostMode ghosts = GHOST_FULL, bool dot = false,
                bool snap = false, bool timed = false, int sweeps = 0)
{
    DevLevel &L = h->lv[l];
    MGPS_TRY(exchangeGhosts(h, l, x, ghosts));
    double *sink = dot ? takeDotSink(h, unsigned(L.npure[odd] + L.nmixed[odd])) : nullptr;
    return timedSweep(h, timed, sweeps, [&]() -> int {
        MGPS_LAUNCH(h, launchTiledGS(h->stream, L.g, x, b, L.pure[odd], L.npure[odd], L.mixed[odd], L.nmixed[odd], L.tileBndStart, forward, sink,
                                     snap ? L.r : nullptr, snap ? L.snapTile : nullptr));
        return MGPS_OK;
    });
}
int gsSweep(mgps_solver *h, int l, float *x, const float *b, bool down, GhostMode before, bool dot, bool snap = false)
{
    const int first = down ? 1 : 0, forward = down ? 1 : 0;
    MGPS_TRY(gsHalfSweep(h, l, x, b, first, forward, before, dot, snap, sweepTimed(h, l), 0));
    return gsHalfSweep(h, l, x, b, 1 - first, forward, GHOST_FULL, dot, snap, sweepTimed(h, l), 1);
}

int ensureSnapTiles(mgps_solver *h, int l)
{
    DevLevel &L = h->lv[l];
    if (L.snapTile) return MGPS_OK;
    const size_t nt = size_t((L.d.nx + kTile - 1) / kTile) * size_t((L.d.ny + kTile - 1) / kTile) * size_t((L.d.nz + kTile - 1) / kTile);
    MGPS_TRY(devAlloc(h, &L.snapTile, nt, true));
    MGPS_LAUNCH(h, launchMarkSnapTiles(h->stream, L.g, L.bandBoxes, L.snapTile));
    return MGPS_OK;
}
int ensureKeepBits(mgps_solver *h, int l)
{
    DevLevel &L = h->lv[l];
    if (L.keepBits) return MGPS_OK;
    MGPS_TRY(devAlloc(h, &L.keepBits, L.d.cells() / 32, true));
    MGPS_LAUNCH(h, launchMarkClosure(h->stream, L.g, L.bandBoxes, L.keepBits));
    return MGPS_OK;
}

enum StrokeForm {
    SF_GS_SNAPSHOT,
    SF_THREE_LAUNCH,
    SF_FRONT,
    SF_PROLONG_FUSED,
    SF_FIRST_FUSED,
    SF_GENERIC,
};

StrokeForm strokeForm(const mgps_solver *h, int l, bool down, const float *cur, const float *other, const float *b, bool dot)
{
    static const bool gsSnapshots = [] {
        const char *e = getenv("MGPS_GS_SNAPSHOT");
        return !(e && e[0] == '0');
    }();
    static const int fuseUp = [] {
        const char *e = getenv("MGPS_FUSE_UP");
        return !e ? -1 : (e[0] == '0' ? 0 : 1);
    }();
    const DevLevel &L = h->lv[l];
    const bool boxes = h->opt.band_iterations > 0 && levelHasBoxes(h, l) && (!L.r || (cur != L.r && other != L.r && b != L.r));
    if (h->useGS) return boxes && gsSnapshots && !h->dist ? SF_GS_SNAPSHOT : SF_GENERIC;
    const int reps = down ? h->opt.pre_sweeps : h->opt.post_sweeps;
    if (!boxes || reps != 1) return boxes && reps > 1 && !L.boxForm ? SF_FIRST_FUSED : SF_GENERIC;
    const bool planes = size_t(L.g.nx) * L.g.ny * sizeof(float) >= kPlaneSweepMinPlaneBytes;
    if (!down && fuseUp != 0 && (fuseUp > 0 || planes) && l + 1 < int(h->lv.size()) && !dot && !h->dist && !h->tailOfSlabRun && h->opt.precision == 0 &&
        !L.boxForm && prolongJacobiPlaneFits(L.g) && boxPlaneFits(L.d))
        return SF_PROLONG_FUSED;
    if (!dot && !sweepTimed(h, l) && !stageTimingOn(h) && !h->dist && L.d.cells() <= (size_t(1) << 24) && stencilKernelOf(L.g) == 1 && (L.d.cells() & 31) == 0)
        return SF_FRONT;
    return SF_THREE_LAUNCH;
}

bool strokeTakesZero(const mgps_solver *h, int l, const float *cur, const float *other, const float *b, bool dot)
{
    static const bool allowed = [] {
        const char *e = getenv("MGPS_ZERO_START");
        return !(e && e[0] == '0');
    }();
    const StrokeForm f = strokeForm(h, l, true, cur, other, b, dot);
    return allowed && !dot && (f == SF_THREE_LAUNCH || f == SF_FRONT) && (!h->dist || h->lv[l].boxForm) && stencilKernelOf(h->lv[l].g) != 3 && !sweepTimed(h, l);
}

bool residualRestrictFuses(const mgps_solver *h, int l)
{
    static const int mode = [] {
        const char *e = getenv("MGPS_FUSE_RR");
        return !e ? -1 : (e[0] == '0' ? 0 : 1);
    }();
    if (mode == 0 || l + 1 >= int(h->lv.size()) || (h->opt.precision != 0 && l == 0)) return false;
    const GridP &F = h->lv[l].g;
    if (mode < 0 && size_t(F.nx) * F.ny * sizeof(float) < kPlaneSweepMinPlaneBytes) return false;
    return residualRestrictFits(F, h->lv[l + 1].g);
}
bool residualRestrictXFolded(const mgps_solver *h, int l)
{
    static const bool allowed = [] {
        const char *e = getenv("MGPS_RZ_XFOLD");
        return !(e && e[0] == '0');
    }();
    return allowed && residualRestrictFuses(h, l) && residualRestrictXFolds(h->lv[l].g);
}
int residualRestrict(mgps_solver *h, int l, const float *x, const float *rhs, float *out = nullptr)
{
    DevLevel &F = h->lv[l], &C = h->lv[l + 1];
    const bool xfold = residualRestrictXFolded(h, l);
    if (!F.rz) {
        MGPS_TRY(devAlloc(h, &F.rz, xfold ? rzxFloats(F.g) : F.d.cells() / 2, true));
        if (F.g.planeBlocks) {
            if (!F.planeFlags) {
                MGPS_TRY(devAlloc(h, &F.planeFlags, planeBlockCount(F.g), true));
                MGPS_LAUNCH(h, launchPlaneBlockFlags(h->stream, F.g, F.planeFlags));
            }
            std::vector<uint8_t> flags(planeBlockCount(F.g));
            MGPS_HIP(h, hipMemcpyAsync(flags.data(), F.planeFlags, flags.size(), hipMemcpyDeviceToHost, h->stream));
            MGPS_HIP(h, hipStreamSynchronize(h->stream));
            const std::vector<int32_t> edges = planeBlockEdges(F.g, flags);
            F.nrzEdges = int(edges.size());
            if (F.nrzEdges) MGPS_TRY(devUpload(h, &F.rzEdges, edges));
        }
    }
    {
        StageScope scope(h, ST_RESIDUAL, l);
        const bool cut = h->dist && (F.g.ghostLo || F.g.ghostHi);
        if (cut) {
            MGPS_TRY(exchangeGhosts(h, l, const_cast<float *>(x), F.boxForm ? GHOST_FULL : h->opt.band_iterations > 0 ? GHOST_BAND : GHOST_FULL));
            MGPS_LAUNCH(h, launchResidualEdgePlanes(h->stream, F.g, F.r, x, rhs));
            MGPS_TRY(exchangeGhosts(h, l, F.r, GHOST_FULL));
        }
        MGPS_LAUNCH(h, launchResidualZ(h->stream, F.g, F.rz, x, rhs, F.rzEdges, F.nrzEdges, cut ? F.r : nullptr, xfold));
    }
    StageScope scope(h, ST_RESTRICT, l);
    if (xfold) MGPS_LAUNCH(h, launchRestrictY(h->stream, C.g, out ? out : C.b, F.rz, F.g));
    else MGPS_LAUNCH(h, launchRestrictXY(h->stream, C.g, out ? out : C.b, F.rz));
    return MGPS_OK;
}

int prolongAdd(mgps_solver *h, int l, float *cur, float *coarse, bool snap)
{
    DevLevel &F = h->lv[l];
    StageScope scope(h, ST_PROLONG, l);
    MGPS_TRY(exchangeGhosts(h, l + 1, coarse));
    if (snap) MGPS_TRY(ensureSnapTiles(h, l));
    MGPS_LAUNCH(h, launchProlongAdd(h->stream, F.g, cur, coarse, snap ? F.r : nullptr, snap ? F.snapTile : nullptr));
    return MGPS_OK;
}

int gsSnapshotStroke(mgps_solver *h, int l, float *cur, const float *b, bool down, bool fresh, bool dot, bool preSnap)
{
    DevLevel &L = h->lv[l];
    MGPS_TRY(ensureSnapTiles(h, l));
    {
        StageScope scope(h, ST_BAND, l);
        if (down && fresh)
            MGPS_LAUNCH(h, launchBandBox(h->stream, L.g, L.bandBoxes, false, nullptr, b, cur, nullptr, h->opt.jacobi_weight));
        else if (preSnap)
            MGPS_LAUNCH(h, launchBandBox(h->stream, L.g, L.bandBoxes, false, L.r, b, cur, nullptr, h->opt.jacobi_weight));
        else
            MGPS_TRY(bandPasses(h, l, cur, b, GHOST_NONE));
    }
    const int reps = down ? h->opt.pre_sweeps : h->opt.post_sweeps;
    for (int rep = 0; rep < reps; ++rep) {
        StageScope scope(h, ST_SMOOTH, l);
        const bool last = rep == reps - 1;
        MGPS_TRY(gsSweep(h, l, cur, b, down, GHOST_NONE, dot && last, last));
    }
    StageScope scope(h, ST_BAND, l);
    double *sink = dot ? takeDotSink(h, unsigned(L.bandBoxes.ngroups)) : nullptr;
    MGPS_LAUNCH(h, launchBandBox(h->stream, L.g, L.bandBoxes, false, L.r, b, cur, nullptr, h->opt.jacobi_weight, false, MixScale{}, sink, L.r));
    return MGPS_OK;
}

int threeLaunchStroke(mgps_solver *h, int l, float *&cur, float *&other, const float *b, bool dot, bool xZero)
{
    DevLevel &L = h->lv[l];
    const float *src = xZero ? nullptr : cur;
    {
        StageScope scope(h, ST_BAND, l);
        if (L.boxForm && xZero) MGPS_TRY(haloListExchange(h, l, const_cast<float *>(b), nullptr, false));
        else if (L.boxForm) MGPS_TRY(haloListExchange(h, l, cur, const_cast<float *>(b), true));
        MGPS_LAUNCH(h, launchBandBox(h->stream, boxGrid(h, l), L.bandBoxes, true, src, b, nullptr, L.r, h->opt.jacobi_weight));
    }
    {
        StageScope scope(h, ST_SMOOTH, l);
        MGPS_TRY(timedSweep(h, sweepTimed(h, l), 1, [&]() -> int {
            if (dot) {
                unsigned used = 0;
                MGPS_LAUNCH(h, launchStencilDot(h->stream, OP_JACOBI, L.g, other, cur, b, h->opt.jacobi_weight, h->dotPartials + h->dotUsed, &used));
                h->dotUsed += used;
                return MGPS_OK;
            }
            GridP gs = L.g;
            gs.nbnd = 0;
            MGPS_LAUNCH(h, launchStencil(h->stream, OP_JACOBI, gs, other, src, b, h->opt.jacobi_weight, true));
            return MGPS_OK;
        }));
    }
    double *sinkB = dot ? takeDotSink(h, unsigned(L.bandBoxes.ngroups)) : nullptr;
    StageScope scope(h, ST_BAND, l);
    std::swap(cur, other);
    if (L.boxForm) MGPS_TRY(haloListExchange(h, l, L.r, nullptr, false));
    MGPS_LAUNCH(h, launchBandBox(h->stream, boxGrid(h, l), L.bandBoxes, false, L.r, b, cur, nullptr, h->opt.jacobi_weight, false, MixScale{}, sinkB, cur, true));
    return MGPS_OK;
}

int frontStroke(mgps_solver *h, int l, float *&cur, float *&other, const float *b, bool xZero)
{
    DevLevel &L = h->lv[l];
    MGPS_TRY(ensureKeepBits(h, l));
    MGPS_LAUNCH(h, launchStrokeFront(h->stream, L.g, L.bandBoxes, other, xZero ? nullptr : cur, b, L.r, h->opt.jacobi_weight, L.keepBits));
    std::swap(cur, other);
    MGPS_LAUNCH(h, launchBandBox(h->stream, L.g, L.bandBoxes, false, L.r, b, cur, nullptr, h->opt.jacobi_weight, false, MixScale{}, nullptr, nullptr, true));
    return MGPS_OK;
}

int prolongFusedStroke(mgps_solver *h, int l, float *&cur, float *&other, const float *b, const float *coarse)
{
    DevLevel &L = h->lv[l];
    {
        StageScope scope(h, ST_BAND, l);
        MGPS_LAUNCH(h, launchBandBoxClosureProlonged(h->stream, L.g, L.bandBoxes, cur, coarse, b, L.r, h->opt.jacobi_weight));
    }
    {
        StageScope scope(h, ST_SMOOTH, l);
        GridP gs = L.g;
        gs.nbnd = 0;
        MGPS_TRY(timedSweep(h, sweepTimed(h, l), 1, [&]() -> int {
            MGPS_LAUNCH(h, launchProlongJacobi(h->stream, gs, other, cur, b, coarse, h->opt.jacobi_weight));
            return MGPS_OK;
        }));
    }
    StageScope scope(h, ST_BAND, l);
    std::swap(cur, other);
    MGPS_LAUNCH(h, launchBandBox(h->stream, L.g, L.bandBoxes, false, L.r, b, cur, nullptr, h->opt.jacobi_weight, false, MixScale{}, nullptr, nullptr, true));
    return MGPS_OK;
}

int sweepsThenBands(mgps_solver *h, int l, float *&cur, float *&other, const float *b, bool down, int from, GhostMode before, bool dot)
{
    DevLevel &L = h->lv[l];
    const int reps = down ? h->opt.pre_sweeps : h->opt.post_sweeps;
    for (int rep = from; rep < reps; ++rep) {
        StageScope scope(h, ST_SMOOTH, l);
        const GhostMode ghosts = rep == from ? before : GHOST_FULL;
        const bool d = dot && rep == reps - 1;
        if (h->useGS) {
            MGPS_TRY(gsSweep(h, l, cur, b, down, ghosts, d));
            continue;
        }
        MGPS_TRY(exchangeGhosts(h, l, cur, ghosts));
        MGPS_TRY(timedSweep(h, sweepTimed(h, l), 1, [&]() -> int {
            if (d) {
                unsigned used = 0;
                MGPS_LAUNCH(h, launchStencilDot(h->stream, OP_JACOBI, L.g, other, cur, b, h->opt.jacobi_weight, h->dotPartials + h->dotUsed, &used));
                h->dotUsed += used;
            } else
                MGPS_LAUNCH(h, launchStencil(h->stream, OP_JACOBI, L.g, other, cur, b, h->opt.jacobi_weight, true));
            return MGPS_OK;
        }));
        std::swap(cur, other);
    }
    StageScope scope(h, ST_BAND, l);
    return bandPasses(h, l, cur, b, GHOST_FULL, dot);
}

int firstFusedStroke(mgps_solver *h, int l, float *&cur, float *&other, const float *b, bool down, bool dot)
{
    DevLevel &L = h->lv[l];
    {
        StageScope scope(h, ST_SMOOTH, l);
        GridP gs = L.g;
        gs.nbnd = 0;
        MGPS_TRY(timedSweep(h, sweepTimed(h, l), 1, [&]() -> int {
            MGPS_LAUNCH(h, launchStencil(h->stream, OP_JACOBI, gs, other, cur, b, h->opt.jacobi_weight, true));
            return MGPS_OK;
        }));
    }
    {
        StageScope scope(h, ST_BAND, l);
        MGPS_LAUNCH(h, launchBandBox(h->stream, L.g, L.bandBoxes, true, cur, b, other, nullptr, h->opt.jacobi_weight));
        std::swap(cur, other);
    }
    return sweepsThenBands(h, l, cur, other, b, down, 1, GHOST_FULL, dot);
}

int smoothStroke(mgps_solver *h, int l, float *&cur, float *&other, const float *b, bool down, bool ghostsFresh, bool dot = false, bool xZero = false,
                 float *coarse = nullptr)
{
    const StrokeForm form = strokeForm(h, l, down, cur, other, b, dot);
    if (coarse && form != SF_PROLONG_FUSED) MGPS_TRY(prolongAdd(h, l, cur, coarse, form == SF_GS_SNAPSHOT));
    switch (form) {
    case SF_GS_SNAPSHOT: return gsSnapshotStroke(h, l, cur, b, down, ghostsFresh, dot, coarse != nullptr);
    case SF_THREE_LAUNCH: return threeLaunchStroke(h, l, cur, other, b, dot, xZero);
    case SF_FRONT: return frontStroke(h, l, cur, other, b, xZero);
    case SF_PROLONG_FUSED: return prolongFusedStroke(h, l, cur, other, b, coarse);
    case SF_FIRST_FUSED: return firstFusedStroke(h, l, cur, other, b, down, dot);
    case SF_GENERIC: break;
    }
    {
        StageScope scope(h, ST_BAND, l);
        MGPS_TRY(bandPasses(h, l, cur, b, ghostsFresh ? GHOST_NONE : GHOST_FULL));
    }
    const GhostMode afterBands = h->opt.band_iterations > 0 ? GHOST_BAND : (ghostsFresh ? GHOST_NONE : GHOST_FULL);
    return sweepsThenBands(h, l, cur, other, b, down, 0, afterBands, dot);
}

int vcycle(mgps_solver *h, float *x, const float *b, bool useInitialGuess, bool ownGrid = false, bool wantDot = false);

int poisonSpares(mgps_solver *h, int l, float *a, float *b2)
{
    static const bool on = [] {
        const char *e = getenv("MGPS_POISON_SPARES");
        return e && e[0] == '1';
    }();
    if (!on) return MGPS_OK;
    const float nan = std::numeric_limits<float>::quiet_NaN();
    MGPS_LAUNCH(h, launchScale(h->stream, h->lv[l].g, a, nan));
    MGPS_LAUNCH(h, launchScale(h->stream, h->lv[l].g, b2, nan));
    return MGPS_OK;
}

int collapsedTail(mgps_solver *h)
{
    DevLevel &C = h->lv[h->distLevels];
    const size_t bytes = C.d.cells() * sizeof(float);
    const int P = h->comm.size;
    bool uniform = true;
    for (int r = 1; r < P; ++r) uniform = uniform && (h->splits[size_t(r) + 1] - h->splits[size_t(r)]) == (h->splits[1] - h->splits[0]);
    std::vector<size_t> counts, displs;
    if (!uniform) {
        const size_t planeBytes = size_t(C.d.nx) * C.d.ny * sizeof(float);
        for (int r = 0; r < P; ++r) {
            displs.push_back(size_t(h->splits[size_t(r)] >> h->distLevels) * planeBytes);
            counts.push_back(size_t((h->splits[size_t(r) + 1] - h->splits[size_t(r)]) >> h->distLevels) * planeBytes);
        }
    }
    if (uniform) MGPS_COMM(h, h->comm.gather(h->comm.user, C.b, h->comm.rank == 0 ? h->tailB : nullptr, bytes, 0, h->stream));
    else MGPS_COMM(h, h->comm.gatherv(h->comm.user, C.b, bytes, h->comm.rank == 0 ? h->tailB : nullptr, counts.data(), displs.data(), 0, h->stream));
    if (h->comm.rank == 0) {
        h->tail->stream = h->stream;
        const int rc = vcycle(h->tail, h->tailX, h->tailB, false);
        if (rc != MGPS_OK) return failH(h, rc, "collapsed tail: " + h->tail->lastError);
    }
    if (uniform) MGPS_COMM(h, h->comm.scatter(h->comm.user, h->comm.rank == 0 ? h->tailX : nullptr, C.x, bytes, 0, h->stream));
    else MGPS_COMM(h, h->comm.scatterv(h->comm.user, h->comm.rank == 0 ? h->tailX : nullptr, counts.data(), displs.data(), C.x, bytes, 0, h->stream));
    return MGPS_OK;
}

int zeroGrid(mgps_solver *h, float *a, const Dims &d, bool withGhosts)
{
    const size_t plane = size_t(d.nx) * d.ny;
    if (withGhosts) MGPS_LAUNCH(h, launchZero(h->stream, a - plane, d.cells() + 2 * plane));
    else MGPS_LAUNCH(h, launchZero(h->stream, a, d.cells()));
    return MGPS_OK;
}

int zeroOwnGrid(mgps_solver *h, int l, float *a, bool withGhosts)
{
    DevLevel &L = h->lv[l];
    MGPS_LAUNCH(h, launchZeroActive(h->stream, L.g, a, withGhosts && h->dist));
    return MGPS_OK;
}

int downStrokeFromZero(mgps_solver *h, int l, float *&cur, float *&other, const float *b, bool own, bool dot)
{
    const bool zero = own && strokeTakesZero(h, l, cur, other, b, dot);
    if (zero) MGPS_TRY(poisonSpares(h, l, cur, other));
    else if (own) MGPS_TRY(zeroOwnGrid(h, l, cur, true));
    else MGPS_TRY(zeroGrid(h, cur, h->lv[l].d, h->dist));
    return smoothStroke(h, l, cur, other, b, true, true, dot, zero);
}

int cycleLevels(mgps_solver *h, int first, float *&x, float *spare, const float *b, bool poll)
{
    const int nlv = int(h->lv.size()), bottom = nlv - 1;
    std::vector<float *> cur(nlv, nullptr), other(nlv, nullptr);
    cur[first] = x;
    other[first] = spare;
    auto rhsOf = [&](int l) -> const float * { return l == first ? b : h->lv[l].b; };
    auto stopRequested = [&] { return poll && h->opt.interrupt && h->opt.interrupt(h->opt.interrupt_user); };
    for (int l = first; l < bottom; ++l) {
        DevLevel &F = h->lv[l], &C = h->lv[l + 1];
        if (l > 0) {
            if (stopRequested()) return failH(h, MGPS_ERR_INTERRUPTED, "mgps_apply_vcycle: interrupted");
            if (l > first) {
                cur[l] = F.x;
                other[l] = F.tmp;
            }
            MGPS_TRY(downStrokeFromZero(h, l, cur[l], other[l], rhsOf(l), true, false));
        }
        if (residualRestrictFuses(h, l)) {
            MGPS_TRY(residualRestrict(h, l, cur[l], rhsOf(l)));
            continue;
        }
        {
            StageScope scope(h, ST_RESIDUAL, l);
            MGPS_TRY(exchangeGhosts(h, l, cur[l], F.boxForm ? GHOST_FULL : h->opt.band_iterations > 0 ? GHOST_BAND : GHOST_FULL));
            MGPS_LAUNCH(h, launchStencil(h->stream, OP_RESIDUAL, F.g, F.r, cur[l], rhsOf(l), 0.f, true));
        }
        StageScope scope(h, ST_RESTRICT, l);
        MGPS_TRY(exchangeGhosts(h, l, F.r));
        MGPS_LAUNCH(h, launchRestrict(h->stream, C.g, C.b, F.r));
    }
    DevLevel &B = h->lv[bottom];
    {
        StageScope scope(h, ST_COARSE, bottom);
        if (h->dist) MGPS_TRY(collapsedTail(h));
        else MGPS_LAUNCH(h, launchCoarseSolve(h->stream, h->cn, h->cinv, h->ccells, B.x, B.b, h->cvec));
    }
    cur[bottom] = B.x;
    for (int l = bottom - 1; l >= first; --l) {
        if (stopRequested()) return failH(h, MGPS_ERR_INTERRUPTED, "mgps_apply_vcycle: interrupted");
        MGPS_TRY(smoothStroke(h, l, cur[l], other[l], rhsOf(l), false, false, h->gatherDot && l == 0, false, cur[l + 1]));
    }
    x = cur[first];
    return MGPS_OK;
}

int vcycle(mgps_solver *h, float *x, const float *b, bool useInitialGuess, bool ownGrid, bool wantDot)
{
    h->gatherDot = wantDot && !h->dist && h->dotPartials != nullptr;
    h->dotUsed = 0;
    const int nlv = int(h->lv.size());
    if (h->tailOfSlabRun && nlv == 1) {
        MGPS_TRY(zeroGrid(h, x, h->lv[0].d, false));
        MGPS_LAUNCH(h, launchCoarseSolve(h->stream, h->cn, h->cinv, h->ccells, x, b, h->cvec));
        return MGPS_OK;
    }
    const bool hasBottom = nlv > 1;
    float *cur = x, *other = h->lv[0].tmp;
    if (useInitialGuess) MGPS_TRY(smoothStroke(h, 0, cur, other, b, true, false, h->gatherDot && !hasBottom));
    else MGPS_TRY(downStrokeFromZero(h, 0, cur, other, b, ownGrid, h->gatherDot && !hasBottom));
    if (hasBottom) MGPS_TRY(cycleLevels(h, 0, cur, other, b, !h->dist && !h->tailOfSlabRun));
    if (cur != x)
        MGPS_HIP(h, hipMemcpyAsync(x, cur, h->lv[0].d.cells() * sizeof(float), hipMemcpyDeviceToDevice, h->stream));
    if (h->gatherDot) MGPS_LAUNCH(h, launchFoldDot(h->stream, h->dotPartials, h->dotUsed, h->dotTarget ? h->dotTarget : h->resultDev));
    stageCycleDone(h);
    return MGPS_OK;
}

int ensureMixedGrids(mgps_solver *h)
{
    if (h->mixX) return MGPS_OK;
    const size_t n = h->lv[0].d.cells();
    uint16_t *p[3] = {nullptr, nullptr, nullptr};
    for (int q = 0; q < 3; ++q) MGPS_TRY(devAlloc(h, &p[q], n, true));
    h->mixX = p[0];
    h->mixTmp = p[1];
    h->mixR = p[2];
    MGPS_TRY(devAlloc(h, &h->mixSigma, 1, true));
    MGPS_TRY(devAlloc(h, &h->mixMax, 1, true));
    const Dims d = h->lv[0].d;
    const double bound = 0.5 * double(std::max(d.nx, std::max(d.ny, d.nz))) * double(std::max(d.nx, std::max(d.ny, d.nz)));
    h->mixExp = std::max(0, int(std::ceil(std::log2(bound / 16384.0))));
    return MGPS_OK;
}

int vcycleMixed(mgps_solver *h, float *x, const float *b, bool useInitialGuess, const double *maxAbsDev = nullptr, double *dotDev = nullptr)
{
    MGPS_TRY(ensureMixedGrids(h));
    DevLevel &F = h->lv[0];
    if (useInitialGuess && x) {
        MGPS_LAUNCH(h, launchStencil(h->stream, OP_RESIDUAL, F.g, F.r, x, b, 0.f, true));
        MGPS_TRY(vcycleMixed(h, nullptr, F.r, false));
        MGPS_LAUNCH(h, launchXpayHalf(h->stream, F.g, x, h->mixResult, h->mixSigma, std::ldexp(1.f, h->mixExp), nullptr, 1.f));
        return MGPS_OK;
    }
    const int nlv = int(h->lv.size());
    const size_t n = F.d.cells();
    const float xs = std::ldexp(1.f, -h->mixExp), xsInv = std::ldexp(1.f, h->mixExp);
    const float omega = h->opt.jacobi_weight;
    if (!maxAbsDev) {
        MGPS_LAUNCH(h, launchReduce(h->stream, 3, F.g, b, nullptr, h->partials, h->mixMax));
        maxAbsDev = h->mixMax;
    }
    MGPS_LAUNCH(h, launchMixSigma(h->stream, maxAbsDev, h->mixSigma));
    void *cur = h->mixX, *other = h->mixTmp;
    const bool gatherDown = dotDev != nullptr && h->dotPartials != nullptr && nlv == 1;
    const bool zeroStart = strokeTakesZero(h, 0, h->lv[0].x, h->lv[0].tmp, b, gatherDown) && (F.g.nx & 3) == 0;
    if (!zeroStart) MGPS_LAUNCH(h, launchZeroActiveHalf(h->stream, F.g, cur));
    const MixScale smooth{h->mixSigma, xs, 1.f};
    const bool gather = dotDev != nullptr && h->dotPartials != nullptr && !h->useGS;
    h->dotUsed = 0;
    auto bandStage = [&](bool dot) -> int {
        double *sink = dot && F.bandBoxes.ngroups > 0 ? takeDotSink(h, unsigned(F.bandBoxes.ngroups)) : nullptr;
        MGPS_LAUNCH(h, launchBandBox(h->stream, F.g, F.bandBoxes, false, cur, b, h->mixR, nullptr, omega, true, smooth, sink, cur));
        MGPS_LAUNCH(h, launchBandBoxCopy(h->stream, F.g, F.bandBoxes, h->mixR, cur, true));
        return MGPS_OK;
    };
    auto sweep = [&](bool d, bool patchGeneral, bool xZero) -> int {
        unsigned used = 0;
        GridP gs = F.g;
        if (!patchGeneral) gs.nbnd = 0;
        MGPS_TRY(timedSweep(h, h->profiling, 1, [&]() -> int {
            MGPS_LAUNCH(h, launchStencilMixed(h->stream, OP_JACOBI, gs, other, xZero ? nullptr : cur, b, omega, smooth, d ? h->dotPartials + h->dotUsed : nullptr, &used));
            return MGPS_OK;
        }));
        h->dotUsed += used;
        return MGPS_OK;
    };
    auto stroke = [&](bool down, bool dot, bool xZero) -> int {
        const int reps = down ? h->opt.pre_sweeps : h->opt.post_sweeps;
        if (reps == 1 && F.bandBoxes.ngroups > 0 && !h->useGS) {
            MGPS_LAUNCH(h, launchBandBox(h->stream, F.g, F.bandBoxes, true, xZero ? nullptr : cur, b, nullptr, h->mixR, omega, true, smooth));
            MGPS_TRY(sweep(dot, dot, xZero));
            double *sinkB = dot ? takeDotSink(h, unsigned(F.bandBoxes.ngroups)) : nullptr;
            std::swap(cur, other);
            MGPS_LAUNCH(h, launchBandBox(h->stream, F.g, F.bandBoxes, false, h->mixR, b, cur, nullptr, omega, true, smooth, sinkB, cur, true));
            return MGPS_OK;
        }
        MGPS_TRY(bandStage(false));
        for (int rep = 0; rep < reps; ++rep) {
            if (h->useGS) {
                const int first = down ? 1 : 0, forward = down ? 1 : 0;
                MGPS_TRY(timedSweep(h, h->profiling, 1, [&]() -> int {
                    for (int pass = 0; pass < 2; ++pass) {
                        const int odd = pass == 0 ? first : 1 - first;
                        MGPS_LAUNCH(h, launchTiledGSMixed(h->stream, F.g, cur, b, F.pure[odd], F.npure[odd], F.mixed[odd], F.nmixed[odd], F.tileBndStart, forward, smooth));
                    }
                    return MGPS_OK;
                }));
                continue;
            }
            MGPS_TRY(sweep(dot && rep == reps - 1, true, false));
            std::swap(cur, other);
        }
        MGPS_TRY(bandStage(dot));
        return MGPS_OK;
    };
    MGPS_TRY(stroke(true, gather && nlv == 1, zeroStart));
    if (nlv > 1) {
        DevLevel &C = h->lv[1];
        const MixScale res{h->mixSigma, 256.f, 256.f * xsInv};
        MGPS_LAUNCH(h, launchStencilMixed(h->stream, OP_RESIDUAL, F.g, h->mixR, cur, b, 0.f, res));
        MGPS_LAUNCH(h, launchRestrictMixed(h->stream, C.g, C.b, h->mixR, 1.f / 256.f));
        float *corr = C.x;
        MGPS_TRY(cycleLevels(h, 1, corr, C.tmp, C.b, false));
        MGPS_LAUNCH(h, launchProlongAddMixed(h->stream, F.g, cur, corr, xs));
        MGPS_TRY(stroke(false, gather, false));
    }
    if (gather) {
        MGPS_LAUNCH(h, launchFoldDot(h->stream, h->dotPartials, h->dotUsed, dotDev));
        MGPS_LAUNCH(h, launchScaleResult(h->stream, dotDev, h->mixSigma, xsInv));
    }
    h->mixResult = cur;
    if (dotDev && !gather) MGPS_LAUNCH(h, launchHalfDot(h->stream, F.g, cur, b, h->mixSigma, xsInv, h->partials, dotDev));
    if (x) MGPS_LAUNCH(h, launchFromHalf(h->stream, x, cur, h->mixSigma, xsInv, n));
    stageCycleDone(h);
    return MGPS_OK;
}

int fetchReduction(mgps_solver *h, int kind, double *out)
{
    MGPS_HIP(h, hipMemcpyAsync(h->resultHost, h->resultDev, sizeof(double), hipMemcpyDeviceToHost, h->stream));
    MGPS_HIP(h, hipStreamSynchronize(h->stream));
    *out = *h->resultHost;
    if (h->dist) MGPS_COMM(h, h->comm.allreduce(h->comm.user, out, 1, kind <= 1 ? 0 : 1));
    return MGPS_OK;
}

int reduceToHost(mgps_solver *h, int kind, int level, const float *a, const float *b, double *out)
{
    DevLevel &L = h->lv[level];
    MGPS_LAUNCH(h, launchReduce(h->stream, kind, L.g, a, b, h->partials, h->resultDev));
    return fetchReduction(h, kind, out);
}

int ensurePcgGrids(mgps_solver *h, bool needDiag)
{
    for (int q = 0; q < 4; ++q)
        if (!h->pcg[q]) MGPS_TRY(gridAlloc(h, &h->pcg[q], h->lv[0].d));
    if (!h->cgScal) MGPS_TRY(devAlloc(h, &h->cgScal, 8, true));
    if (!h->dotPartials) {
        const DevLevel &F = h->lv[0];
        const size_t tiles = size_t(F.npure[0]) + F.npure[1] + F.nmixed[0] + F.nmixed[1];
        const size_t scatters = size_t(std::max(1, h->opt.band_iterations)) * bandScatterBlocks(F.nband) + 2 * size_t(F.bandBoxes.ngroups);
        h->dotCapacity = applyDotPartialCount(F.g) + tiles + scatters + 64 + 2048;
        MGPS_TRY(devAlloc(h, &h->dotPartials, h->dotCapacity, true));
    }
    if (needDiag && !h->dinv) {
        MGPS_TRY(gridAlloc(h, &h->dinv, h->lv[0].d));
        MGPS_LAUNCH(h, launchDiagInverse(h->stream, h->lv[0].g, h->dinv));
    }
    return MGPS_OK;
}

// ... 2870 lines not shown
    if (rc != MGPS_OK) return bail(rc);
    int tailRc = MGPS_OK;
    if (rank == 0) {
        tailRc = [&]() -> int {
            const HostLevel &C = hier->lv[D];
            mgps_hierarchy *tailHier = nullptr;
            int trc = hierarchyCreate(&tailHier, C.d.nx, C.d.ny, C.d.nz, C.labels.data(), hier->levels - D, &o, true, false);
            if (trc != MGPS_OK) return failH(h, trc, std::string("collapsed tail hierarchy: ") + lastGlobalError());
            trc = createWhole(&h->tail, tailHier, nullptr, nullptr, nullptr, h->useGS, o, device, true);
            if (trc != MGPS_OK) return failH(h, trc, std::string("collapsed tail: ") + lastGlobalError());
            trc = gridAlloc(h->tail, &h->tailX, C.d);
            if (trc == MGPS_OK) trc = gridAlloc(h->tail, &h->tailB, C.d);
            if (trc != MGPS_OK) return trc;
            h->tail->userGrids.push_back(h->tailX - size_t(C.d.nx) * C.d.ny);
            h->tail->userGrids.push_back(h->tailB - size_t(C.d.nx) * C.d.ny);
            if (hipDeviceSynchronize() != hipSuccess) return failH(h, MGPS_ERR_HIP, "device synchronize failed");
            return MGPS_OK;
        }();
    }
    sclock.lap("slab: common state + tail");
    double failed = tailRc != MGPS_OK ? double(tailRc) : 0.0;
    if (h->comm.allreduce(h->comm.user, &failed, 1, 1) != 0) return bail(failH(h, MGPS_ERR_COMM, "all-reduce failed during set-up"));
    if (failed != 0.0) {
        if (tailRc == MGPS_OK) failH(h, int(failed), "the collapsed tail could not be built on rank 0 (status " + std::to_string(int(failed)) + ")");
        return bail(tailRc != MGPS_OK ? tailRc : int(failed));
    }
    if (int rc2 = setupEnclosedSlab(h, sclock); rc2 != MGPS_OK) return bail(rc2);
    *out = h;
    return MGPS_OK;
}
}
extern "C" {
int mgps_create_slab_ranges(mgps_solver **out, int nx, int ny, int nz_global, const uint8_t *labels_global_host, const float *wx_slab,
                            const float *wy_slab, const float *wz_slab, int mg_levels, int use_gauss_seidel, const mgps_options *opt,
                            const mgps_comm *comm, const int *splits)
try {
    return createSlabImpl(out, nx, ny, nz_global, labels_global_host, wx_slab, wy_slab, wz_slab, mg_levels, use_gauss_seidel, opt, comm, splits, false);
}
MGPS_API_CATCH(nullptr)
int mgps_create_slab_device_weights(mgps_solver **out, int nx, int ny, int nz_global, const uint8_t *labels_global_host, const float *wx_slab_dev,
                                    const float *wy_slab_dev, const float *wz_slab_dev, int mg_levels, int use_gauss_seidel, const mgps_options *opt,
                                    const mgps_comm *comm, const int *splits)
try {
    return createSlabImpl(out, nx, ny, nz_global, labels_global_host, wx_slab_dev, wy_slab_dev, wz_slab_dev, mg_levels, use_gauss_seidel, opt, comm, splits, true);
}
MGPS_API_CATCH(nullptr)
int mgps_create_slab_device_labels(mgps_solver **out, int nx, int ny, int nz_global, const uint8_t *labels_slab_dev, const float *wx_slab_dev,
                                   const float *wy_slab_dev, const float *wz_slab_dev, int mg_levels, int use_gauss_seidel, const mgps_options *opt,
                                   const mgps_comm *comm, const int *splits)
try {
    if (!labels_slab_dev) {
        if (out) *out = nullptr;
        return failH(nullptr, MGPS_ERR_INVALID_ARGUMENT, "mgps_create_slab_device_labels: the rank's label planes are required");
    }
    return createSlabImpl(out, nx, ny, nz_global, nullptr, wx_slab_dev, wy_slab_dev, wz_slab_dev, mg_levels, use_gauss_seidel, opt, comm, splits, true, labels_slab_dev);
}
MGPS_API_CATCH(nullptr)

int mgps_create_slab(mgps_solver **out, int nx, int ny, int nz_global, const uint8_t *labels_global_host, const float *wx_slab,
                     const float *wy_slab, const float *wz_slab, int mg_levels, int use_gauss_seidel, const mgps_options *opt,
                     const mgps_comm *comm)
try {
    if (!comm || comm->size < 1) return failH(nullptr, MGPS_ERR_INVALID_ARGUMENT, "mgps_create_slab: a comm is required");
    if (nz_global % comm->size != 0)
        return failH(nullptr, MGPS_ERR_INVALID_ARGUMENT, "mgps_create_slab: nz must divide evenly over the ranks (or pass cuts to mgps_create_slab_ranges)");
    std::vector<int> cuts(size_t(comm->size) + 1);
    for (int r = 0; r <= comm->size; ++r) cuts[size_t(r)] = nz_global / comm->size * r;
    return mgps_create_slab_ranges(out, nx, ny, nz_global, labels_global_host, wx_slab, wy_slab, wz_slab, mg_levels, use_gauss_seidel, opt, comm,
                                   cuts.data());
}
MGPS_API_CATCH(nullptr)

void mgps_destroy(mgps_solver *h) { freeAll(h); }
int mgps_levels(const mgps_solver *h) { return h ? h->totalLevels : 0; }
const mgps_hierarchy *mgps_get_hierarchy(const mgps_solver *hc)
try {
    auto *h = const_cast<mgps_solver *>(hc);
    if (h && h->hier && h->hier->windowed) {
        mgps_hierarchy *full = nullptr;
        const Dims d0 = h->hier->lv[0].d;
        if (hierarchyCreate(&full, d0.nx, d0.ny, d0.nz, h->hier->lv[0].labels.data(), h->totalLevels, &h->opt, false, true) != MGPS_OK) {
            failH(h, MGPS_ERR_HIERARCHY, std::string("mgps_get_hierarchy: ") + lastGlobalError());
            return nullptr;
        }
        h->retiredHier.push_back(h->hier);
        h->hier = full;
        return full;
    }
    if (!h || !h->hier || !h->hier->light) return h ? h->hier : nullptr;
    if (h->dist) {
        failH(h, MGPS_ERR_INVALID_ARGUMENT, "mgps_get_hierarchy: a slab rank set up on the device has no host hierarchy (options.host_setup = 1 builds one)");
        return nullptr;
    }
    (void)hipSetDevice(h->device);
    const Dims d = h->lv[0].d;
    RawVec<uint8_t> labels(d.cells());
    if (hipMemcpy(labels.data(), h->lv[0].g.lab, d.cells(), hipMemcpyDeviceToHost) != hipSuccess) {
        failH(h, MGPS_ERR_HIP, "mgps_get_hierarchy: copying the labels to the host failed");
        return nullptr;
    }
    for (uint8_t &l : labels)
        if (l > MGPS_BOUNDARY_CELL) l = MGPS_BOUNDARY_CELL;
    mgps_hierarchy *full = nullptr;
    if (hierarchyCreate(&full, d.nx, d.ny, d.nz, labels.data(), h->requestedLevels, &h->opt, false, true) != MGPS_OK) {
        failH(h, MGPS_ERR_HIERARCHY, std::string("mgps_get_hierarchy: ") + lastGlobalError());
        return nullptr;
    }
    mgps_hierarchy_destroy(h->hier);
    h->hier = full;
    return full;
} catch (...) {
    return nullptr;
}

int mgps_level_array(mgps_solver *h, int level, int which, void *out, int64_t *count)
try {
    MGPS_TRY(checkLevel(h, level, "mgps_level_array"));
    if (!count) return failH(h, MGPS_ERR_INVALID_ARGUMENT, "mgps_level_array: count is NULL");
    const DevLevel &L = h->lv[level];
    const int nt = ((L.d.nx + kTile - 1) / kTile) * ((L.d.ny + kTile - 1) / kTile) * ((L.d.nz + kTile - 1) / kTile);
    const void *src = nullptr;
    size_t n = 0, elem = 4;
    switch (which) {
    case 0: src = L.g.lab, n = L.d.cells(), elem = 1; break;
    case 1: src = L.band, n = size_t(L.nband); break;
    case 2: src = L.bandDiag, n = size_t(L.nband), elem = 1; break;
    case 3: src = L.rows, n = size_t(7) * size_t(L.nbndGeneral); break;
    case 4: src = L.chunks, n = size_t(L.g.nchunks); break;
    case 5: src = L.planeBlocks, n = size_t(L.g.nplaneBlocks); break;
    case 6: src = L.pure[0], n = size_t(L.npure[0]); break;
    case 7: src = L.pure[1], n = size_t(L.npure[1]); break;
    case 8: src = L.mixed[0], n = size_t(L.nmixed[0]); break;
    case 9: src = L.mixed[1], n = size_t(L.nmixed[1]); break;
    case 10: src = L.tileBndStart, n = size_t(nt) + 1; break;
    case 11: src = L.bandBoxes.info, n = size_t(kBoxInfoInts) * size_t(L.bandBoxes.ngroups); break;
    case 12: src = L.bandBoxes.list, n = L.bandBoxes.listCount; break;
    case 13: src = L.bandBoxes.general, n = L.bandBoxes.generalInts; break;
    case 14: {
        if (level != 0 || h->opt.enclosed_liquid != 1)
            return failH(h, MGPS_ERR_INVALID_ARGUMENT, "mgps_level_array: array 14 exists on level 0 with options.enclosed_liquid only");
        *count = int64_t(L.d.cells());
        if (!out) return MGPS_OK;
        int32_t *rank = nullptr;
        MGPS_TRY(devAlloc(h, &rank, L.d.cells(), false));
        int rc = MGPS_OK;
        if (hipMemsetAsync(rank, 0xff, L.d.cells() * sizeof(int32_t), h->stream) != hipSuccess ||
            launchEnclosedRanks(h->stream, rank, h->encCellList, h->encChunks, h->encNChunks) != 0 || hipStreamSynchronize(h->stream) != hipSuccess ||
            hipMemcpy(out, rank, L.d.cells() * sizeof(int32_t), hipMemcpyDeviceToHost) != hipSuccess)
            rc = failH(h, MGPS_ERR_HIP, "mgps_level_array: enclosed-component ranks");
        (void)cacheFree(rank);
        return rc;
    }
    case 15: src = L.g.plainQ, n = L.g.plainQ ? (L.d.cells() / 4 + 31) / 32 : 0; break;
    case 16: src = L.g.plainT, n = L.g.plainT ? size_t(L.d.ny) * L.d.nz * planeTiles(L.d.nx, L.d.ny, L.d.nz, 0).nbx : 0, elem = 8; break;
    default: return failH(h, MGPS_ERR_INVALID_ARGUMENT, "mgps_level_array: unknown array");
    }
    *count = int64_t(n);
    if (out && n) {
        MGPS_HIP(h, hipStreamSynchronize(h->stream));
        MGPS_HIP(h, hipMemcpy(out, src, n * elem, hipMemcpyDeviceToHost));
    }
    return MGPS_OK;
}
MGPS_API_CATCH(h)
int mgps_distributed_levels(const mgps_solver *h) { return h ? h->distLevels : 0; }
int mgps_ghost_planes(const mgps_solver *h) { return h ? h->ghost : 1; }
int mgps_residual_restrict_fused(const mgps_solver *h, int level, int *fused)
try {
    if (!h || !fused || level < 0 || level >= int(h->lv.size())) return MGPS_ERR_INVALID_ARGUMENT;
    *fused = residualRestrictFuses(h, level) ? 1 : 0;
    return MGPS_OK;
}
MGPS_API_CATCH(h)
int mgps_residual_restrict_xfolded(const mgps_solver *h, int level, int *xfolded)
try {
    if (!h || !xfolded || level < 0 || level >= int(h->lv.size())) return MGPS_ERR_INVALID_ARGUMENT;
    *xfolded = residualRestrictXFolded(h, level) ? 1 : 0;
    return MGPS_OK;
}
MGPS_API_CATCH(h)
int mgps_up_stroke_fused(const mgps_solver *h, int level, int *fused)
try {
    if (!h || !fused || level < 0 || level >= int(h->lv.size())) return MGPS_ERR_INVALID_ARGUMENT;
    *fused = strokeForm(h, level, false, nullptr, nullptr, nullptr, false) == SF_PROLONG_FUSED ? 1 : 0;
    return MGPS_OK;
}
MGPS_API_CATCH(h)
int mgps_band_stage_form(const mgps_solver *h, int level, int *form)
try {
    if (!h || !form || level < 0 || level >= int(h->lv.size())) return MGPS_ERR_INVALID_ARGUMENT;
    *form = levelHasBoxes(h, level) ? 1 : 0;
    return MGPS_OK;
}
MGPS_API_CATCH(h)
int64_t mgps_overlapped_exchanges(const mgps_solver *) { return 0; }
int64_t mgps_exchange_count(const mgps_solver *h) { return h ? h->exchanges : 0; }

int mgps_level_dims(const mgps_solver *h, int level, int out_dims[3])
try {
    if (!h || !out_dims || level < 0) return failH(nullptr, MGPS_ERR_INVALID_ARGUMENT, "mgps_level_dims: bad arguments");
    if (level < int(h->lv.size())) {
        out_dims[0] = h->lv[level].d.nx;
        out_dims[1] = h->lv[level].d.ny;
        out_dims[2] = h->lv[level].d.nz;
        return MGPS_OK;
    }
    return mgps_hierarchy_level_dims(h->hier, level, out_dims);
}
MGPS_API_CATCH(h)

int mgps_slab_range(const mgps_solver *h, int level, int *z0, int *z1)
try {
    if (!h || !z0 || !z1 || level < 0 || level >= int(h->lv.size()))
        return failH(nullptr, MGPS_ERR_INVALID_ARGUMENT, "mgps_slab_range: bad arguments");
    *z0 = h->lv[level].z0;
    *z1 = h->lv[level].z1;
    return MGPS_OK;
}
MGPS_API_CATCH(h)

int mgps_set_stream(mgps_solver *h, void *hip_stream)
try {
    if (!h) return failH(nullptr, MGPS_ERR_INVALID_ARGUMENT, "mgps_set_stream: NULL handle");
    h->stream = static_cast<hipStream_t>(hip_stream);
    return MGPS_OK;
}
MGPS_API_CATCH(h)

int mgps_synchronize(mgps_solver *h)
try {
    MGPS_TRY(checkLevel(h, 0, "mgps_synchronize"));
    MGPS_HIP(h, hipStreamSynchronize(h->stream));
    return MGPS_OK;
}
MGPS_API_CATCH(h)

int mgps_grid_alloc(mgps_solver *h, int level, float **out_dev)
try {
    MGPS_TRY(checkLevel(h, level, "mgps_grid_alloc"));
    if (!out_dev) return failH(h, MGPS_ERR_INVALID_ARGUMENT, "mgps_grid_alloc: out is NULL");
    MGPS_TRY(gridAlloc(h, out_dev, h->lv[level].d));
    h->userGrids.push_back(*out_dev - size_t(h->ghost) * size_t(h->lv[level].d.nx) * h->lv[level].d.ny);
    return MGPS_OK;
}
MGPS_API_CATCH(h)

int mgps_grid_free(mgps_solver *h, float *dev)
try {
    MGPS_TRY(checkLevel(h, 0, "mgps_grid_free"));
    for (auto it = h->userGrids.begin(); it != h->userGrids.end(); ++it)
        for (const DevLevel &L : h->lv)
            if (static_cast<float *>(*it) + size_t(h->ghost) * size_t(L.d.nx) * L.d.ny == dev) {
                void *base = *it;
                h->userGrids.erase(it);
                MGPS_HIP(h, hipStreamSynchronize(h->stream));
                MGPS_HIP(h, cacheFree(base));
                return MGPS_OK;
            }
    return failH(h, MGPS_ERR_INVALID_ARGUMENT, "mgps_grid_free: not a grid of this solver");
}
MGPS_API_CATCH(h)

int mgps_grid_upload(mgps_solver *h, int level, float *dst_dev, const float *src_host)
try {
    MGPS_TRY(checkLevel(h, level, "mgps_grid_upload"));
    if (!dst_dev || !src_host) return failH(h, MGPS_ERR_INVALID_ARGUMENT, "mgps_grid_upload: NULL pointer");
    MGPS_HIP(h, hipMemcpyAsync(dst_dev, src_host, h->lv[level].d.cells() * sizeof(float), hipMemcpyHostToDevice, h->stream));
    MGPS_HIP(h, hipStreamSynchronize(h->stream));
    return MGPS_OK;
}
MGPS_API_CATCH(h)

int mgps_grid_download(mgps_solver *h, int level, float *dst_host, const float *src_dev)
try {
    MGPS_TRY(checkLevel(h, level, "mgps_grid_download"));
    if (!dst_host || !src_dev) return failH(h, MGPS_ERR_INVALID_ARGUMENT, "mgps_grid_download: NULL pointer");
    MGPS_HIP(h, hipMemcpyAsync(dst_host, src_dev, h->lv[level].d.cells() * sizeof(float), hipMemcpyDeviceToHost, h->stream));
    MGPS_HIP(h, hipStreamSynchronize(h->stream));
    return MGPS_OK;
}
MGPS_API_CATCH(h)

int mgps_copy_to_host(mgps_solver *h, void *dst_host, const void *src_dev, size_t bytes)
try {
    MGPS_TRY(checkLevel(h, 0, "mgps_copy_to_host"));
    MGPS_HIP(h, hipMemcpyAsync(dst_host, src_dev, bytes, hipMemcpyDeviceToHost, h->stream));
    MGPS_HIP(h, hipStreamSynchronize(h->stream));
    return MGPS_OK;
}
MGPS_API_CATCH(h)

int mgps_copy_to_device(mgps_solver *h, void *dst_dev, const void *src_host, size_t bytes)
try {
    MGPS_TRY(checkLevel(h, 0, "mgps_copy_to_device"));
    MGPS_HIP(h, hipMemcpyAsync(dst_dev, src_host, bytes, hipMemcpyHostToDevice, h->stream));
    MGPS_HIP(h, hipStreamSynchronize(h->stream));
    return MGPS_OK;
}
MGPS_API_CATCH(h)

int mgps_apply_vcycle(mgps_solver *h, float *x_dev, const float *b_dev, int use_initial_guess)
try {
    MGPS_TRY(checkLevel(h, 0, "mgps_apply_vcycle"));
    if (!x_dev || !b_dev || x_dev == b_dev) return failH(h, MGPS_ERR_INVALID_ARGUMENT, "mgps_apply_vcycle: bad grid pointers");
    if (h->opt.precision == 1) return vcycleMixed(h, x_dev, b_dev, use_initial_guess != 0);
    if (hasEnclosed(h)) {
        const float *pb = nullptr;
        MGPS_TRY(projectedRhs(h, b_dev, &pb));
        MGPS_TRY(vcycle(h, x_dev, pb, use_initial_guess != 0));
        return projectEnclosed(h, x_dev);
    }
    return vcycle(h, x_dev, b_dev, use_initial_guess != 0);
}
MGPS_API_CATCH(h)

int mgps_jacobi_smooth(mgps_solver *h, int level, float *x_dev, const float *b_dev)
try {
    MGPS_TRY(checkLevel(h, level, "mgps_jacobi_smooth"));
    if (!x_dev || !b_dev) return failH(h, MGPS_ERR_INVALID_ARGUMENT, "mgps_jacobi_smooth: NULL grid");
    DevLevel &L = h->lv[level];
    if (!L.tmp) return failH(h, MGPS_ERR_INVALID_ARGUMENT, "mgps_jacobi_smooth: level has no work grids");
    MGPS_TRY(applyOp(h, OP_JACOBI, level, L.tmp, x_dev, b_dev));
    MGPS_HIP(h, hipMemcpyAsync(x_dev, L.tmp, L.d.cells() * sizeof(float), hipMemcpyDeviceToDevice, h->stream));
    return MGPS_OK;
}
MGPS_API_CATCH(h)

int mgps_tiled_gs_smooth(mgps_solver *h, int level, float *x_dev, const float *b_dev, int smooth_odd_tiles,
                         int smooth_forward)
try {
    MGPS_TRY(checkLevel(h, level, "mgps_tiled_gs_smooth"));
    if (!x_dev || !b_dev) return failH(h, MGPS_ERR_INVALID_ARGUMENT, "mgps_tiled_gs_smooth: NULL grid");
    return gsHalfSweep(h, level, x_dev, b_dev, smooth_odd_tiles ? 1 : 0, smooth_forward != 0);
}
MGPS_API_CATCH(h)

int mgps_boundary_jacobi_smooth(mgps_solver *h, int level, float *x_dev, const float *b_dev)
try {
    MGPS_TRY(checkLevel(h, level, "mgps_boundary_jacobi_smooth"));
    if (!x_dev || !b_dev) return failH(h, MGPS_ERR_INVALID_ARGUMENT, "mgps_boundary_jacobi_smooth: NULL grid");
    DevLevel &L = h->lv[level];
    MGPS_TRY(exchangeGhosts(h, level, x_dev));
    MGPS_LAUNCH(h, launchBandJacobi(h->stream, L.g, x_dev, b_dev, L.band, L.nband, L.bandTmp, h->opt.jacobi_weight));
    return MGPS_OK;
}
MGPS_API_CATCH(h)

int mgps_boundary_jacobi_stage(mgps_solver *h, int level, float *x_dev, const float *b_dev)
try {
    MGPS_TRY(checkLevel(h, level, "mgps_boundary_jacobi_stage"));
    if (!x_dev || !b_dev) return failH(h, MGPS_ERR_INVALID_ARGUMENT, "mgps_boundary_jacobi_stage: NULL grid");
    return bandPasses(h, level, x_dev, b_dev, GHOST_FULL);
}
MGPS_API_CATCH(h)

int mgps_apply_poisson(mgps_solver *h, int level, float *y_dev, const float *x_dev)
try {
    MGPS_TRY(checkLevel(h, level, "mgps_apply_poisson"));
    if (!y_dev || !x_dev || y_dev == x_dev) return failH(h, MGPS_ERR_INVALID_ARGUMENT, "mgps_apply_poisson: bad grid pointers");
    return applyOp(h, OP_APPLY, level, y_dev, const_cast<float *>(x_dev), nullptr);
}
MGPS_API_CATCH(h)

int mgps_residual(mgps_solver *h, int level, float *r_dev, const float *x_dev, const float *b_dev)
try {
    MGPS_TRY(checkLevel(h, level, "mgps_residual"));
    if (!r_dev || !x_dev || !b_dev || r_dev == x_dev)
        return failH(h, MGPS_ERR_INVALID_ARGUMENT, "mgps_residual: bad grid pointers");
    return applyOp(h, OP_RESIDUAL, level, r_dev, const_cast<float *>(x_dev), b_dev);
}
MGPS_API_CATCH(h)

int mgps_downsample(mgps_solver *h, int fine_level, float *coarse_dev, const float *fine_dev)
try {
    MGPS_TRY(checkLevel(h, fine_level + 1, "mgps_downsample"));
    if (fine_level < 0 || !coarse_dev || !fine_dev) return failH(h, MGPS_ERR_INVALID_ARGUMENT, "mgps_downsample: bad arguments");
    MGPS_TRY(exchangeGhosts(h, fine_level, const_cast<float *>(fine_dev)));
    MGPS_LAUNCH(h, launchZero(h->stream, coarse_dev, h->lv[fine_level + 1].d.cells()));
    MGPS_LAUNCH(h, launchRestrict(h->stream, h->lv[fine_level + 1].g, coarse_dev, fine_dev));
    return MGPS_OK;
}
MGPS_API_CATCH(h)

int mgps_residual_downsample(mgps_solver *h, int fine_level, float *coarse_dev, const float *x_dev, const float *b_dev)
try {
    MGPS_TRY(checkLevel(h, fine_level + 1, "mgps_residual_downsample"));
    if (fine_level < 0 || !coarse_dev || !x_dev || !b_dev) return failH(h, MGPS_ERR_INVALID_ARGUMENT, "mgps_residual_downsample: bad arguments");
    if (h->opt.precision == 1 && fine_level == 0) return failH(h, MGPS_ERR_INVALID_ARGUMENT, "mgps_residual_downsample: fp32 levels only");
    DevLevel &F = h->lv[fine_level];
    MGPS_LAUNCH(h, launchZero(h->stream, coarse_dev, h->lv[fine_level + 1].d.cells()));
    if (residualRestrictFuses(h, fine_level)) return residualRestrict(h, fine_level, x_dev, b_dev, coarse_dev);
    if (!F.r) return failH(h, MGPS_ERR_INVALID_ARGUMENT, "mgps_residual_downsample: level has no work grids");
    MGPS_TRY(applyOp(h, OP_RESIDUAL, fine_level, F.r, const_cast<float *>(x_dev), b_dev, true));
    MGPS_TRY(exchangeGhosts(h, fine_level, F.r));
    MGPS_LAUNCH(h, launchRestrict(h->stream, h->lv[fine_level + 1].g, coarse_dev, F.r));
    return MGPS_OK;
}
MGPS_API_CATCH(h)

int mgps_upsample_add(mgps_solver *h, int fine_level, float *fine_dev, const float *coarse_dev)
try {
    MGPS_TRY(checkLevel(h, fine_level + 1, "mgps_upsample_add"));
    if (fine_level < 0 || !coarse_dev || !fine_dev) return failH(h, MGPS_ERR_INVALID_ARGUMENT, "mgps_upsample_add: bad arguments");
    MGPS_TRY(exchangeGhosts(h, fine_level + 1, const_cast<float *>(coarse_dev)));
    MGPS_LAUNCH(h, launchProlongAdd(h->stream, h->lv[fine_level].g, fine_dev, coarse_dev));
    return MGPS_OK;
}
MGPS_API_CATCH(h)

int mgps_coarse_solve(mgps_solver *h, float *x_dev, const float *b_dev)
try {
    MGPS_TRY(checkLevel(h, 0, "mgps_coarse_solve"));
    if (!x_dev || !b_dev) return failH(h, MGPS_ERR_INVALID_ARGUMENT, "mgps_coarse_solve: NULL grid");
    if (h->dist) return failH(h, MGPS_ERR_INVALID_ARGUMENT, "mgps_coarse_solve: not available on a slab solver");
    MGPS_LAUNCH(h, launchCoarseSolve(h->stream, h->cn, h->cinv, h->ccells, x_dev, b_dev, h->cvec));
    return MGPS_OK;
}
MGPS_API_CATCH(h)

int mgps_dot(mgps_solver *h, int level, const float *a_dev, const float *b_dev, double *out)
try {
    MGPS_TRY(checkLevel(h, level, "mgps_dot"));
    if (!a_dev || !b_dev || !out) return failH(h, MGPS_ERR_INVALID_ARGUMENT, "mgps_dot: NULL pointer");
    return reduceToHost(h, 0, level, a_dev, b_dev, out);
}
MGPS_API_CATCH(h)

int mgps_squared_l2_norm(mgps_solver *h, int level, const float *a_dev, double *out)
try {
    MGPS_TRY(checkLevel(h, level, "mgps_squared_l2_norm"));
    if (!a_dev || !out) return failH(h, MGPS_ERR_INVALID_ARGUMENT, "mgps_squared_l2_norm: NULL pointer");
    return reduceToHost(h, 1, level, a_dev, nullptr, out);
}
MGPS_API_CATCH(h)

int mgps_l2_norm(mgps_solver *h, int level, const float *a_dev, double *out)
try {
    MGPS_TRY(mgps_squared_l2_norm(h, level, a_dev, out));
    *out = std::sqrt(*out);
    return MGPS_OK;
}
MGPS_API_CATCH(h)

int mgps_inf_norm(mgps_solver *h, int level, const float *a_dev, int reference_signed_max, double *out)
try {
    MGPS_TRY(checkLevel(h, level, "mgps_inf_norm"));
    if (!a_dev || !out) return failH(h, MGPS_ERR_INVALID_ARGUMENT, "mgps_inf_norm: NULL pointer");
    return reduceToHost(h, reference_signed_max ? 2 : 3, level, a_dev, nullptr, out);
}
MGPS_API_CATCH(h)

int mgps_add_to_vector(mgps_solver *h, int level, float *dst_dev, const float *src_dev, double scale)
try {
    MGPS_TRY(checkLevel(h, level, "mgps_add_to_vector"));
    if (!dst_dev || !src_dev) return failH(h, MGPS_ERR_INVALID_ARGUMENT, "mgps_add_to_vector: NULL grid");
    MGPS_LAUNCH(h, launchAxpy(h->stream, h->lv[level].g, dst_dev, src_dev, nullptr, float(scale), 1.f));
    return MGPS_OK;
}
MGPS_API_CATCH(h)

int mgps_add_vectors(mgps_solver *h, int level, float *dst_dev, const float *a_dev, const float *scaled_dev, double scale)
try {
    MGPS_TRY(checkLevel(h, level, "mgps_add_vectors"));
    if (!dst_dev || !a_dev || !scaled_dev) return failH(h, MGPS_ERR_INVALID_ARGUMENT, "mgps_add_vectors: NULL grid");
    MGPS_LAUNCH(h, launchXpay(h->stream, h->lv[level].g, dst_dev, a_dev, scaled_dev, nullptr, float(scale)));
    return MGPS_OK;
}
MGPS_API_CATCH(h)

int mgps_scale_vector(mgps_solver *h, int level, float *v_dev, double scale)
try {
    MGPS_TRY(checkLevel(h, level, "mgps_scale_vector"));
    if (!v_dev) return failH(h, MGPS_ERR_INVALID_ARGUMENT, "mgps_scale_vector: NULL grid");
    MGPS_LAUNCH(h, launchScale(h->stream, h->lv[level].g, v_dev, float(scale)));
    return MGPS_OK;
}
MGPS_API_CATCH(h)

int mgps_zero_inactive(mgps_solver *h, int level, float *grid_dev)
try {
    MGPS_TRY(checkLevel(h, level, "mgps_zero_inactive"));
    if (!grid_dev) return failH(h, MGPS_ERR_INVALID_ARGUMENT, "mgps_zero_inactive: NULL grid");
    MGPS_LAUNCH(h, launchZeroInactive(h->stream, h->lv[level].g, grid_dev));
    return MGPS_OK;
}
MGPS_API_CATCH(h)

int mgps_solve_pcg(mgps_solver *h, float *x_dev, const float *b_dev, double tolerance, int max_iterations,
                   int use_mg_preconditioner, mgps_pcg_stats *stats)
try {
    MGPS_TRY(checkLevel(h, 0, "mgps_solve_pcg"));
    if (!x_dev || !b_dev || x_dev == b_dev || !(tolerance >= 0) || max_iterations < 0)
        return failH(h, MGPS_ERR_INVALID_ARGUMENT, "mgps_solve_pcg: bad arguments");
    return pcg(h, x_dev, const_cast<float *>(b_dev), tolerance, max_iterations, use_mg_preconditioner != 0, stats);
}
MGPS_API_CATCH(h)

}

namespace mgps {
int coupledSolveRefusal(mgps_solver *h, mgps_coupling *coupling, const char *fn)
{
    if (h->opt.precision == 1)
        return failH(h, MGPS_ERR_INVALID_ARGUMENT, std::string(fn) + ": not available with options.precision = 1 (mixed precision)");
    int planes[2], cplRank = 0, cplSize = 1;
    const bool slabCoupling = couplingOnSlab(coupling, planes, &cplRank, &cplSize), slabSolver = h->dist || h->tailOfSlabRun;
    if (slabSolver && !slabCoupling)
        return failH(h, MGPS_ERR_INVALID_ARGUMENT,
                     std::string(fn) + ": a slab solver cannot take a whole-grid coupling (its list lives on one device); make one with mgps_coupling_create_slab");
    if (!slabSolver && slabCoupling)
        return failH(h, MGPS_ERR_INVALID_ARGUMENT, std::string(fn) + ": a slab coupling needs the slab solver of its ranks, this solver holds a whole grid");
    if (h->tailOfSlabRun) return failH(h, MGPS_ERR_INVALID_ARGUMENT, std::string(fn) + ": the collapsed tail of a slab run takes no coupling");
    if (hasEnclosed(h))
        return failH(h, MGPS_ERR_INVALID_ARGUMENT,
                     std::string(fn) + ": the solver has an enclosed liquid component (options.enclosed_liquid); a moving body changes its null space");
    int e[3];
    couplingExtents(coupling, e);
    const Dims &d = h->lv[0].d;
    const int nzWhole = slabSolver ? h->splits.back() : d.nz;
    if (e[0] != d.nx || e[1] != d.ny || e[2] != nzWhole)
        return failH(h, MGPS_ERR_INVALID_ARGUMENT,
                     std::string(fn) + ": the coupling's expanded extents " + std::to_string(e[0]) + " x " + std::to_string(e[1]) + " x " + std::to_string(e[2]) +
                         " differ from the solver's " + std::to_string(d.nx) + " x " + std::to_string(d.ny) + " x " + std::to_string(nzWhole));
    if (slabSolver && (planes[0] != h->lv[0].z0 || planes[1] != h->lv[0].z1 || cplRank != h->comm.rank || cplSize != h->comm.size))
        return failH(h, MGPS_ERR_INVALID_ARGUMENT,
                     std::string(fn) + ": the coupling's window, expanded planes " + std::to_string(planes[0]) + " .. " + std::to_string(planes[1]) + " of rank " +
                         std::to_string(cplRank) + " of " + std::to_string(cplSize) + ", is not this slab solver's (planes " + std::to_string(h->lv[0].z0) + " .. " +
                         std::to_string(h->lv[0].z1) + " of rank " + std::to_string(h->comm.rank) + " of " + std::to_string(h->comm.size) + ")");
    return MGPS_OK;
}
}

extern "C" {

int mgps_solve_pcg_coupled(mgps_solver *h, mgps_coupling *coupling, float *x_dev, const float *b_dev, double tolerance, int max_iterations,
                           int use_mg_preconditioner, mgps_pcg_stats *stats)
try {
    const char *fn = "mgps_solve_pcg_coupled";
    MGPS_TRY(checkLevel(h, 0, fn));
    if (!coupling) return failH(h, MGPS_ERR_INVALID_ARGUMENT, std::string(fn) + ": NULL coupling");
    if (!x_dev || !b_dev || x_dev == b_dev || !(tolerance >= 0) || max_iterations < 0)
        return failH(h, MGPS_ERR_INVALID_ARGUMENT, std::string(fn) + ": bad arguments");
    MGPS_TRY(mgps::coupledSolveRefusal(h, coupling, fn));
    mgps_pcg_stats local{};
    if (!stats) stats = &local;
    std::memset(stats, 0, sizeof(*stats));
    struct Attached {
        mgps_solver *h;
// ... 235 lines not shown
```

geometricmultigridpressuresolver_amd/solver.py:

```python
import ctypes as C

import numpy as np
import torch

from . import _lib
from ._lib import Options, PcgStats, check, lib

PCG_OUTCOMES = {0: "converged", 1: "rhs_zero", 2: "already_converged", 3: "max_iterations"}


def _pcg_stats(st):
    return {
        "outcome": PCG_OUTCOMES.get(st.outcome, st.outcome),
        "iterations": st.iterations,
        "rel_residual": st.rel_residual,
        "rel_residual_recomputed": st.rel_residual_recomputed,
        "rhs_norm2": st.rhs_norm2,
        "solve_ms": st.solve_ms,
    }


def _check_pcg(status, handle, st):
    try:
        check(status, handle)
# ... 56 lines not shown


def unit_test_boundary_cells(labels, weights=None):
    labels = _np_u8(labels)
    nz, ny, nx = labels.shape
    ok = C.c_int()
    w = [None] * 3 if weights is None else [_p(_np_f32(a)) for a in weights]
    keep = weights
    check(lib().mgps_check_boundary_cells(_p(labels), w[0], w[1], w[2], nx, ny, nz, C.byref(ok)))
    return bool(ok.value)


def unit_test_exterior_cells(labels):
    labels = _np_u8(labels)
    nz, ny, nx = labels.shape
    ok = C.c_int()
    check(lib().mgps_check_exterior_cells(_p(labels), nx, ny, nz, C.byref(ok)))
    return bool(ok.value)


def unit_test_coarsening(coarse, fine):
    coarse, fine = _np_u8(coarse), _np_u8(fine)
    nz, ny, nx = fine.shape
    ok = C.c_int()
    check(lib().mgps_check_coarsening(_p(coarse), _p(fine), nx, ny, nz, C.byref(ok)))
    return bool(ok.value)


class Hierarchy:

    def __init__(self, labels=None, mg_levels=None, options=None, _borrowed=None):
        self._own = _borrowed is None
        if _borrowed is not None:
            self.h = C.c_void_p(_borrowed)
            return
        labels = _np_u8(labels)
        nz, ny, nx = labels.shape
        h = C.c_void_p()
        opt = options if options is not None else default_options()
        check(lib().mgps_hierarchy_create(C.byref(h), nx, ny, nz, _p(labels), int(mg_levels), C.byref(opt)))
        self.h = h

    def close(self):
        if self._own and self.h:
            lib().mgps_hierarchy_destroy(self.h)
        self.h = None

    def __del__(self):
        try:
            self.close()
        except Exception:
            pass

    @property
    def levels(self):
        return lib().mgps_hierarchy_levels(self.h)

    def level_shape(self, level):
        d = (C.c_int * 3)()
        check(lib().mgps_hierarchy_level_dims(self.h, level, d))
        return (d[2], d[1], d[0])

    def level_labels(self, level):
        out = np.empty(self.level_shape(level), dtype=np.uint8)
        check(lib().mgps_hierarchy_level_labels(self.h, level, _p(out)))
        return out

    def band_cells(self, level):
        n = lib().mgps_hierarchy_band_count(self.h, level)
        out = np.empty((max(n, 0), 3), dtype=np.int32)
        if n > 0:
            check(lib().mgps_hierarchy_band_cells(self.h, level, _p(out)))
        return out

    def check_band_boxes(self, level, depth=3, weights=None):
        g, n, q = C.c_int64(), C.c_int64(), C.c_int64()
        w = [None, None, None]
        if weights is not None:
            w = [_np_f32(a) for a in weights]
        check(lib().mgps_hierarchy_check_band_boxes(self.h, int(level), int(depth), *[(_p(a) if a is not None else None) for a in w],
                                                    C.byref(g), C.byref(n), C.byref(q)))
        return g.value, n.value, q.value

    @property
    def coarse_unknowns(self):
        return lib().mgps_hierarchy_coarse_unknowns(self.h)

    def coarse_solve(self, b):
        b = _np_f32(b)
        x = np.zeros_like(b)
        check(lib().mgps_hierarchy_coarse_solve(self.h, _p(x), _p(b)))
        return x


class GeometricMultigridPoissonSolver:

    def __init__(self, labels, weights, mg_levels, use_gauss_seidel, do_print_stats=False, device=None, options=None):
        on_device = all(torch.is_tensor(a) and a.is_cuda for a in weights)
        labels_on_device = on_device and torch.is_tensor(labels) and labels.is_cuda and labels.dtype == torch.uint8
        if labels_on_device:
            labels = labels.contiguous()
        else:
            if torch.is_tensor(labels):
                labels = labels.cpu().numpy()
            labels = _np_u8(labels)
        nz, ny, nx = labels.shape
        if on_device:
            w = [a.contiguous() for a in weights]
            assert all(a.dtype == torch.float32 for a in w)
        else:
            w = [_np_f32(a) for a in weights]
        assert tuple(w[0].shape) == (nz, ny, nx + 1) and tuple(w[1].shape) == (nz, ny + 1, nx) and tuple(w[2].shape) == (nz + 1, ny, nx)
        opt = options if options is not None else default_options()
        opt.print_stats = int(do_print_stats) if not isinstance(do_print_stats, bool) else int(do_print_stats)
        if device is not None:
            opt.device = torch.device(device).index if not isinstance(device, int) else device
        elif on_device:
            opt.device = w[0].device.index
        self.h = C.c_void_p()
        wp = [C.c_void_p(a.data_ptr()) for a in w] if on_device else [_p(a) for a in w]
        create = lib().mgps_create_device if labels_on_device else lib().mgps_create_device_weights if on_device else lib().mgps_create
        lp = C.c_void_p(labels.data_ptr()) if labels_on_device else _p(labels)
        check(create(C.byref(self.h), nx, ny, nz, lp, wp[0], wp[1], wp[2], int(mg_levels), int(bool(use_gauss_seidel)), C.byref(opt)))
        self.shape = (nz, ny, nx)
        self.use_gauss_seidel = bool(use_gauss_seidel)
        dev_index = opt.device if opt.device >= 0 else torch.cuda.current_device()
        self.device = torch.device("cuda", dev_index)
        self.use_torch_stream()

    def close(self):
        if getattr(self, "h", None):
            lib().mgps_destroy(self.h)
            self.h = None

    def __del__(self):
        try:
            self.close()
        except Exception:
            pass

    def use_torch_stream(self):
        s = torch.cuda.current_stream(self.device).cuda_stream
        check(lib().mgps_set_stream(self.h, C.c_void_p(s)), self.h)

    def synchronize(self):
        check(lib().mgps_synchronize(self.h), self.h)

    def hierarchy(self):
        return Hierarchy(_borrowed=lib().mgps_get_hierarchy(self.h))

    LEVEL_ARRAYS = {"codes": (0, np.uint8), "band": (1, np.int32), "band_diag": (2, np.uint8), "rows": (3, np.float32), "chunks": (4, np.int32),
                    "plane_blocks": (5, np.int32), "pure_even": (6, np.int32), "pure_odd": (7, np.int32), "mixed_even": (8, np.int32),
                    "mixed_odd": (9, np.int32), "tile_bnd_start": (10, np.int32), "box_info": (11, np.int32), "box_list": (12, np.uint32),
                    "box_general": (13, np.int32), "plain_quads": (15, np.uint32), "plain_tiles": (16, np.uint64)}

    def level_array(self, level, name):
        which, dt = self.LEVEL_ARRAYS[name]
        n = C.c_int64()
        check(lib().mgps_level_array(self.h, int(level), which, None, C.byref(n)), self.h)
        out = np.empty(n.value, dtype=dt)
        if n.value:
            check(lib().mgps_level_array(self.h, int(level), which, _p(out), C.byref(n)), self.h)
        return out

    def level_shape(self, level):
        d = (C.c_int * 3)()
        check(lib().mgps_level_dims(self.h, level, d), self.h)
        return (d[2], d[1], d[0])

    def new_grid(self, level=0):
        return torch.zeros(self.level_shape(level), dtype=torch.float32, device=self.device)

    def to_device(self, a, level=0):
        t = torch.from_numpy(_np_f32(a)).to(self.device)
        assert tuple(t.shape) == self.level_shape(level)
        return t

    def _g(self, t, level=0):
        assert t.is_cuda and t.dtype == torch.float32 and t.is_contiguous() and t.device == self.device
        assert tuple(t.shape) == self.level_shape(level), (tuple(t.shape), self.level_shape(level))
        return C.c_void_p(t.data_ptr())

    def getMGLevels(self):
        return lib().mgps_levels(self.h)

    def applyVCycle(self, solution, rhs, use_initial_guess=False):
        check(lib().mgps_apply_vcycle(self.h, self._g(solution), self._g(rhs), int(bool(use_initial_guess))), self.h)

    def jacobiPoissonSmoother(self, solution, rhs, level=0):
        check(lib().mgps_jacobi_smooth(self.h, level, self._g(solution, level), self._g(rhs, level)), self.h)

    def tiledGaussSeidelPoissonSmoother(self, solution, rhs, do_smooth_odd_tiles, do_smooth_forward, level=0):
        check(
            lib().mgps_tiled_gs_smooth(
                self.h, level, self._g(solution, level), self._g(rhs, level), int(bool(do_smooth_odd_tiles)), int(bool(do_smooth_forward))
            ),
            self.h,
        )

    def boundaryJacobiPoissonSmoother(self, solution, rhs, level=0):
        check(lib().mgps_boundary_jacobi_smooth(self.h, level, self._g(solution, level), self._g(rhs, level)), self.h)

    def boundaryJacobiStage(self, solution, rhs, level=0):
        check(lib().mgps_boundary_jacobi_stage(self.h, level, self._g(solution, level), self._g(rhs, level)), self.h)

    def applyPoissonMatrix(self, destination, source, level=0):
        check(lib().mgps_apply_poisson(self.h, level, self._g(destination, level), self._g(source, level)), self.h)

    def computePoissonResidual(self, residual, solution, rhs, level=0):
        check(lib().mgps_residual(self.h, level, self._g(residual, level), self._g(solution, level), self._g(rhs, level)), self.h)

    def downsample(self, destination, source, fine_level=0):
        check(lib().mgps_downsample(self.h, fine_level, self._g(destination, fine_level + 1), self._g(source, fine_level)), self.h)

    def residualDownsample(self, destination, solution, rhs, fine_level=0):
        check(lib().mgps_residual_downsample(self.h, fine_level, self._g(destination, fine_level + 1), self._g(solution, fine_level), self._g(rhs, fine_level)), self.h)

    def upsampleAndAdd(self, destination, source, fine_level=0):
        check(lib().mgps_upsample_add(self.h, fine_level, self._g(destination, fine_level), self._g(source, fine_level + 1)), self.h)

    def coarseDirectSolve(self, solution, rhs):
        L = self.getMGLevels() - 1
        check(lib().mgps_coarse_solve(self.h, self._g(solution, L), self._g(rhs, L)), self.h)

    def dotProduct(self, a, b, level=0):
        out = C.c_double()
        check(lib().mgps_dot(self.h, level, self._g(a, level), self._g(b, level), C.byref(out)), self.h)
        return out.value

    def squaredL2Norm(self, a, level=0):
        out = C.c_double()
        check(lib().mgps_squared_l2_norm(self.h, level, self._g(a, level), C.byref(out)), self.h)
        return out.value

    def l2Norm(self, a, level=0):
        out = C.c_double()
        check(lib().mgps_l2_norm(self.h, level, self._g(a, level), C.byref(out)), self.h)
        return out.value

    def infNorm(self, a, level=0, reference_signed_max=True):
        out = C.c_double()
        check(lib().mgps_inf_norm(self.h, level, self._g(a, level), int(bool(reference_signed_max)), C.byref(out)), self.h)
        return out.value

    def addToVector(self, destination, source, scale, level=0):
        check(lib().mgps_add_to_vector(self.h, level, self._g(destination, level), self._g(source, level), C.c_double(scale)), self.h)

    def addVectors(self, destination, source, scaled_source, scale, level=0):
        check(
            lib().mgps_add_vectors(
                self.h, level, self._g(destination, level), self._g(source, level), self._g(scaled_source, level), C.c_double(scale)
            ),
            self.h,
        )

    def scaleVector(self, vector, scale, level=0):
        check(lib().mgps_scale_vector(self.h, level, self._g(vector, level), C.c_double(scale)), self.h)

    def zeroInactive(self, grid, level=0):
        check(lib().mgps_zero_inactive(self.h, level, self._g(grid, level)), self.h)

    def solveGeometricConjugateGradient(self, solution, rhs, tolerance=1e-5, max_iterations=2500, use_mg_preconditioner=True):
        st = PcgStats()
        _check_pcg(
            lib().mgps_solve_pcg(
                self.h, self._g(solution), self._g(rhs), C.c_double(tolerance), int(max_iterations), int(bool(use_mg_preconditioner)), C.byref(st)
            ),
            self.h,
            st,
        )
        return _pcg_stats(st)

    def solve_pcg_coupled(self, coupling, solution, rhs, tolerance=1e-5, max_iterations=2500, use_mg_preconditioner=True):
        st = PcgStats()
        _check_pcg(
            lib().mgps_solve_pcg_coupled(
                self.h, coupling.h, self._g(solution), self._g(rhs), C.c_double(tolerance), int(max_iterations), int(bool(use_mg_preconditioner)), C.byref(st)
            ),
            self.h,
            st,
        )
        return _pcg_stats(st)

    def enclosed_components(self):
        m, n = C.c_int64(), C.c_int64()
        check(lib().mgps_enclosed_components(self.h, C.byref(m), C.byref(n)), self.h)
        return m.value, n.value

    def enclosed_ranks(self):
        n = C.c_int64()
        check(lib().mgps_level_array(self.h, 0, 14, None, C.byref(n)), self.h)
        out = np.empty(n.value, dtype=np.int32)
        check(lib().mgps_level_array(self.h, 0, 14, _p(out), C.byref(n)), self.h)
        return out

    def project_enclosed(self, v):
        out = C.c_double()
        check(lib().mgps_project_enclosed(self.h, self._g(v), C.byref(out)), self.h)
        return out.value

    def profile_enable(self, on=True):
        check(lib().mgps_profile_enable(self.h, int(on)), self.h)

    def profile_read(self):
        ms, n = C.c_double(), C.c_int()
        check(lib().mgps_profile_read(self.h, C.byref(ms), C.byref(n)), self.h)
        return ms.value, n.value

    def stage_times(self):
        ms = (C.c_double * 6)()
        n = C.c_int()
        check(lib().mgps_stage_times(self.h, ms, C.byref(n)), self.h)
        names = ("boundary_smoother", "smoother", "residual", "downsample", "direct_solve", "upsample_add")
        out = {k: ms[i] for i, k in enumerate(names)}
        out["cycles"] = n.value
        fine = (C.c_double * 6)()
        check(lib().mgps_stage_times_fine(self.h, fine), self.h)
        out["fine"] = {k: fine[i] for i, k in enumerate(names)}
        return out

    def swept_cells(self, level=0):
        a, b = C.c_longlong(), C.c_longlong()
        check(lib().mgps_swept_cells(self.h, int(level), C.byref(a), C.byref(b)), self.h)
        return a.value, b.value

    def residual_restrict_fused(self, level=0):
        f = C.c_int()
        check(lib().mgps_residual_restrict_fused(self.h, int(level), C.byref(f)), self.h)
        return bool(f.value)

    def residual_restrict_xfolded(self, level=0):
        f = C.c_int()
        check(lib().mgps_residual_restrict_xfolded(self.h, int(level), C.byref(f)), self.h)
        return bool(f.value)

    def up_stroke_fused(self, level=0):
        f = C.c_int()
        check(lib().mgps_up_stroke_fused(self.h, int(level), C.byref(f)), self.h)
        return bool(f.value)

    def stencil_kernel(self, level=0):
        k = C.c_int()
        check(lib().mgps_stencil_kernel(self.h, int(level), C.byref(k)), self.h)
        return {1: "quad", 2: "plane", 3: "scalar"}[k.value]

    def applyVCycleHost(self, solution, rhs, use_initial_guess=False):
        if np.asarray(solution).dtype == np.float64:
            x = np.ascontiguousarray(solution, dtype=np.float64)
            b = np.ascontiguousarray(rhs, dtype=np.float64)
            check(lib().mgps_apply_vcycle_host_f64(self.h, _p(x), _p(b), int(bool(use_initial_guess))), self.h)
            return x
        x = _np_f32(solution)
        b = _np_f32(rhs)
        check(lib().mgps_apply_vcycle_host(self.h, _p(x), _p(b), int(bool(use_initial_guess))), self.h)
        return x

    def solvePcgHost(self, solution, rhs, tolerance=1e-5, max_iterations=2500, use_mg_preconditioner=True):

        def run(fn, x, b):
            st = PcgStats()
            try:
                _check_pcg(fn(self.h, _p(x), _p(b), C.c_double(tolerance), int(max_iterations), int(bool(use_mg_preconditioner)), C.byref(st)), self.h, st)
            except _lib.MgpsError as e:
                e.solution = x
                raise
            return x, {"outcome": PCG_OUTCOMES.get(st.outcome, st.outcome), "iterations": st.iterations, "rel_residual": st.rel_residual}

        if np.asarray(solution).dtype == np.float64:
            x = np.ascontiguousarray(solution, dtype=np.float64)
            b = np.ascontiguousarray(rhs, dtype=np.float64)
            return run(lib().mgps_solve_pcg_host_f64, x, b)
        x = _np_f32(solution)
        b = _np_f32(rhs)
        return run(lib().mgps_solve_pcg_host, x, b)
```

include/mgps.h:

```cpp
#ifndef MGPS_H
#define MGPS_H

#include <stddef.h>
#include <stdint.h>

#ifdef __cplusplus
extern "C" {
#endif

#define MGPS_VERSION 1

enum { MGPS_INTERIOR_CELL = 0, MGPS_EXTERIOR_CELL = 1, MGPS_DIRICHLET_CELL = 2, MGPS_BOUNDARY_CELL = 3 };

typedef enum mgps_status {
    MGPS_OK = 0,
    MGPS_ERR_INVALID_ARGUMENT = 1,
    MGPS_ERR_NO_DEVICE = 2,
    MGPS_ERR_HIP = 3,
    MGPS_ERR_ALLOC = 4,
    MGPS_ERR_HIERARCHY = 5,
    MGPS_ERR_COARSE_TOO_LARGE = 6,
    MGPS_ERR_COARSE_FACTOR = 7,
    MGPS_ERR_COMM = 8,
    MGPS_ERR_INTERRUPTED = 9,
    MGPS_ERR_INTERNAL = 10
} mgps_status;

enum { MGPS_PCG_CONVERGED = 0, MGPS_PCG_RHS_ZERO = 1, MGPS_PCG_ALREADY_CONVERGED = 2, MGPS_PCG_MAX_ITERATIONS = 3 };

typedef struct mgps_solver mgps_solver;
typedef struct mgps_hierarchy mgps_hierarchy;

typedef struct mgps_options {
    int struct_size;
    int band_width;
    int band_iterations;
    float jacobi_weight;
    int device;
    int print_stats;
    int max_coarse_unknowns;
    int fuse_band_passes;
    int deep_band_halo;
    int min_cells_per_rank;
    int pcg_fp64_vectors;
    int (*interrupt)(void *user);
    void *interrupt_user;
    int pre_sweeps, post_sweeps;
    int stencil_path;
    int precision;
    int host_setup;
    int borrow_device_weights;
    int enclosed_liquid;
} mgps_options;

typedef struct mgps_pcg_stats {
    int outcome;
    int iterations;
    double rel_residual;
    double rel_residual_recomputed;
    double rhs_norm2;
    double solve_ms;
} mgps_pcg_stats;

void mgps_default_options(mgps_options *opt);
const char *mgps_status_string(int status);
const char *mgps_last_error(const mgps_solver *h);
int mgps_device_count(int *count);
int mgps_level_array(mgps_solver *h, int level, int which, void *out, int64_t *count);

int mgps_expanded_layout(int bnx, int bny, int bnz, int levels_in, int power_of_two,
                         int out_dims[3], int *out_offset, int *out_levels);
int mgps_expand_labels(uint8_t *expanded, const uint8_t *base, int bnx, int bny, int bnz,
                       int enx, int eny, int enz, int offset);
int mgps_expand_weights(float *expanded, const float *base, int axis, int bnx, int bny, int bnz,
                        int enx, int eny, int enz, int offset);
int mgps_set_boundary_labels(uint8_t *labels, const float *wx, const float *wy, const float *wz,
                             int nx, int ny, int nz);
int mgps_check_boundary_cells(const uint8_t *labels, const float *wx, const float *wy,
                              const float *wz, int nx, int ny, int nz, int *pass);
int mgps_check_exterior_cells(const uint8_t *labels, int nx, int ny, int nz, int *pass);
int mgps_check_coarsening(const uint8_t *coarse, const uint8_t *fine, int fnx, int fny, int fnz, int *pass);

int mgps_hierarchy_create(mgps_hierarchy **out, int nx, int ny, int nz, const uint8_t *labels,
                          int mg_levels, const mgps_options *opt);
void mgps_hierarchy_destroy(mgps_hierarchy *hier);
int mgps_hierarchy_levels(const mgps_hierarchy *hier);
int mgps_hierarchy_level_dims(const mgps_hierarchy *hier, int level, int out_dims[3]);
int mgps_hierarchy_level_labels(const mgps_hierarchy *hier, int level, uint8_t *out);
int64_t mgps_hierarchy_band_count(const mgps_hierarchy *hier, int level);
int mgps_hierarchy_band_cells(const mgps_hierarchy *hier, int level, int32_t *out_ijk);
int mgps_hierarchy_check_band_boxes(const mgps_hierarchy *hier, int level, int depth, const float *wx, const float *wy, const float *wz,
                                    int64_t *out_groups, int64_t *out_region_cells, int64_t *out_general);
int mgps_hierarchy_coarse_unknowns(const mgps_hierarchy *hier);
int mgps_hierarchy_coarse_solve(const mgps_hierarchy *hier, float *x, const float *b);

int mgps_create(mgps_solver **out, int nx, int ny, int nz, const uint8_t *labels_host,
                const float *wx_host, const float *wy_host, const float *wz_host, int mg_levels,
                int use_gauss_seidel, const mgps_options *opt);
int mgps_create_device_weights(mgps_solver **out, int nx, int ny, int nz, const uint8_t *labels_host,
                               const float *wx_dev, const float *wy_dev, const float *wz_dev, int mg_levels,
                               int use_gauss_seidel, const mgps_options *opt);
int mgps_create_device(mgps_solver **out, int nx, int ny, int nz, const uint8_t *labels_dev, const float *wx_dev,
                       const float *wy_dev, const float *wz_dev, int mg_levels, int use_gauss_seidel,
                       const mgps_options *opt);
void mgps_destroy(mgps_solver *h);
void mgps_trim_host_cache(void);
void mgps_trim_device_cache(void);
void *mgps_host_alloc(size_t bytes);
void mgps_host_free(void *p);
int mgps_levels(const mgps_solver *h);
int mgps_level_dims(const mgps_solver *h, int level, int out_dims[3]);
const mgps_hierarchy *mgps_get_hierarchy(const mgps_solver *h);
int mgps_set_stream(mgps_solver *h, void *hip_stream);
int mgps_synchronize(mgps_solver *h);

int mgps_grid_alloc(mgps_solver *h, int level, float **out_dev);
int mgps_grid_free(mgps_solver *h, float *dev);
int mgps_grid_upload(mgps_solver *h, int level, float *dst_dev, const float *src_host);
int mgps_grid_download(mgps_solver *h, int level, float *dst_host, const float *src_dev);

int mgps_apply_vcycle(mgps_solver *h, float *x_dev, const float *b_dev, int use_initial_guess);

int mgps_jacobi_smooth(mgps_solver *h, int level, float *x_dev, const float *b_dev);
int mgps_tiled_gs_smooth(mgps_solver *h, int level, float *x_dev, const float *b_dev,
                         int smooth_odd_tiles, int smooth_forward);
int mgps_boundary_jacobi_smooth(mgps_solver *h, int level, float *x_dev, const float *b_dev);
int mgps_boundary_jacobi_stage(mgps_solver *h, int level, float *x_dev, const float *b_dev);
int mgps_apply_poisson(mgps_solver *h, int level, float *y_dev, const float *x_dev);
int mgps_residual(mgps_solver *h, int level, float *r_dev, const float *x_dev, const float *b_dev);
int mgps_downsample(mgps_solver *h, int fine_level, float *coarse_dev, const float *fine_dev);
int mgps_residual_downsample(mgps_solver *h, int fine_level, float *coarse_dev, const float *x_dev, const float *b_dev);

int mgps_upsample_add(mgps_solver *h, int fine_level, float *fine_dev, const float *coarse_dev);
int mgps_coarse_solve(mgps_solver *h, float *x_dev, const float *b_dev);
int mgps_dot(mgps_solver *h, int level, const float *a_dev, const float *b_dev, double *out);
int mgps_squared_l2_norm(mgps_solver *h, int level, const float *a_dev, double *out);
int mgps_l2_norm(mgps_solver *h, int level, const float *a_dev, double *out);
int mgps_inf_norm(mgps_solver *h, int level, const float *a_dev, int reference_signed_max, double *out);
int mgps_add_to_vector(mgps_solver *h, int level, float *dst_dev, const float *src_dev, double scale);
int mgps_add_vectors(mgps_solver *h, int level, float *dst_dev, const float *a_dev,
                     const float *scaled_dev, double scale);
int mgps_scale_vector(mgps_solver *h, int level, float *v_dev, double scale);

int mgps_zero_inactive(mgps_solver *h, int level, float *grid_dev);

int mgps_solve_pcg(mgps_solver *h, float *x_dev, const float *b_dev, double tolerance,
                   int max_iterations, int use_mg_preconditioner, mgps_pcg_stats *stats);

int mgps_enclosed_components(const mgps_solver *h, int64_t *components, int64_t *cells);
int mgps_project_enclosed(mgps_solver *h, float *v_dev, double *max_abs_mean_removed);

struct mgps_xfer2;
typedef struct mgps_comm {
    int struct_size;
    int rank, size;
    void *user;
    int (*exchange)(void *user, const void *send_lo, size_t send_lo_bytes, void *recv_lo, size_t recv_lo_bytes,
                    const void *send_hi, size_t send_hi_bytes, void *recv_hi, size_t recv_hi_bytes,
                    void *hip_stream);
    int (*allreduce)(void *user, double *values, int count, int op);
    int (*gather)(void *user, const void *send_dev, void *recv_dev, size_t bytes, int root, void *hip_stream);
    int (*scatter)(void *user, const void *send_dev, void *recv_dev, size_t bytes, int root, void *hip_stream);
    void (*destroy)(void *user);
    int (*gatherv)(void *user, const void *send_dev, size_t send_bytes, void *recv_dev, const size_t *counts, const size_t *displs,
                   int root, void *hip_stream);
    int (*scatterv)(void *user, const void *send_dev, const size_t *counts, const size_t *displs, void *recv_dev, size_t recv_bytes,
                    int root, void *hip_stream);
    int (*allreduce_device)(void *user, double *values_dev, int count, int op, void *hip_stream);
    int (*exchange2)(void *user, const struct mgps_xfer2 *send_lo, const struct mgps_xfer2 *recv_lo, const struct mgps_xfer2 *send_hi,
                     const struct mgps_xfer2 *recv_hi, void *hip_stream);
} mgps_comm;
typedef struct mgps_xfer2 {
    void *ptr[2];
    size_t bytes[2];
} mgps_xfer2;

int mgps_rccl_unique_id(unsigned char out_id[128]);
int mgps_comm_create_rccl(mgps_comm *out, int rank, int size, const unsigned char id[128], int device);
int mgps_comm_rccl_selftest(mgps_comm *comm, size_t floats);
int mgps_comm_rccl_selfbench(mgps_comm *comm, size_t floats, int reps, double *us_per_exchange);
int mgps_comm_preflight(const mgps_comm *comm, size_t floats, int *ranks_seen);
void mgps_comm_destroy(mgps_comm *comm);

int mgps_create_slab(mgps_solver **out, int nx, int ny, int nz_global, const uint8_t *labels_global_host,
                     const float *wx_slab, const float *wy_slab, const float *wz_slab, int mg_levels,
                     int use_gauss_seidel, const mgps_options *opt, const mgps_comm *comm);
int mgps_slab_partition(int nx, int ny, int nz, const uint8_t *labels_global_host, int mg_levels, int size, int use_gauss_seidel,
                        const mgps_options *opt, int *out_splits);
int mgps_create_slab_ranges(mgps_solver **out, int nx, int ny, int nz_global, const uint8_t *labels_global_host,
                            const float *wx_slab, const float *wy_slab, const float *wz_slab, int mg_levels,
                            int use_gauss_seidel, const mgps_options *opt, const mgps_comm *comm, const int *splits);
int mgps_create_slab_device_weights(mgps_solver **out, int nx, int ny, int nz_global, const uint8_t *labels_global_host,
                                    const float *wx_slab_dev, const float *wy_slab_dev, const float *wz_slab_dev, int mg_levels,
                                    int use_gauss_seidel, const mgps_options *opt, const mgps_comm *comm, const int *splits);
int mgps_create_slab_device_labels(mgps_solver **out, int nx, int ny, int nz_global, const uint8_t *labels_slab_dev,
                                   const float *wx_slab_dev, const float *wy_slab_dev, const float *wz_slab_dev, int mg_levels,
                                   int use_gauss_seidel, const mgps_options *opt, const mgps_comm *comm, const int *splits);
int mgps_slab_partition_device(int nx, int ny, int nz_global, const uint8_t *labels_slab_dev, const int *splits_now, int mg_levels,
                               int use_gauss_seidel, const mgps_options *opt, const mgps_comm *comm, int *out_splits);
int mgps_label_plane_counts(int nx, int ny, int planes, const uint8_t *labels_dev, int64_t *active, int64_t *boundary);
int mgps_slab_range(const mgps_solver *h, int level, int *z0, int *z1);
int mgps_distributed_levels(const mgps_solver *h);
int mgps_ghost_planes(const mgps_solver *h);
int mgps_band_stage_form(const mgps_solver *h, int level, int *form);
int mgps_residual_restrict_fused(const mgps_solver *h, int level, int *fused);
int mgps_residual_restrict_xfolded(const mgps_solver *h, int level, int *xfolded);
int mgps_up_stroke_fused(const mgps_solver *h, int level, int *fused);
int64_t mgps_overlapped_exchanges(const mgps_solver *h);
int64_t mgps_exchange_count(const mgps_solver *h);
int mgps_copy_to_host(mgps_solver *h, void *dst_host, const void *src_dev, size_t bytes);
int mgps_copy_to_device(mgps_solver *h, void *dst_dev, const void *src_host, size_t bytes);

int mgps_profile_enable(mgps_solver *h, int enable);
int mgps_stage_times(mgps_solver *h, double out_ms[6], int *cycles);
int mgps_stage_times_fine(mgps_solver *h, double out_ms[6]);
int mgps_profile_read(mgps_solver *h, double *fine_smoother_ms, int *fine_smoother_launches);
int mgps_swept_cells(const mgps_solver *h, int level, long long *stencil_cells, long long *gs_cells);
int mgps_stencil_kernel(const mgps_solver *h, int level, int *kernel);

int mgps_apply_vcycle_host(mgps_solver *h, float *x_host, const float *b_host, int use_initial_guess);
int mgps_solve_pcg_host(mgps_solver *h, float *x_host, const float *b_host, double tolerance,
                        int max_iterations, int use_mg_preconditioner, mgps_pcg_stats *stats);
int mgps_apply_vcycle_host_f64(mgps_solver *h, double *x_host, const double *b_host, int use_initial_guess);
int mgps_solve_pcg_host_f64(mgps_solver *h, double *x_host, const double *b_host, double tolerance,
                            int max_iterations, int use_mg_preconditioner, mgps_pcg_stats *stats);

#ifdef __cplusplus
}
#endif
#endif
```

Before: 122.2.

## Fuse final down-stroke Jacobi sweep with residual and z-restriction

Adds a fused kernel that performs the last Jacobi smoothing sweep of the fine-level down stroke and computes the residual plus z-direction restriction from the freshly smoothed values held in shared memory. This avoids a separate residual pass that re-reads x and b from global memory. Cross-tile seam contributions that depend on neighbouring tiles are corrected by a follow-up seam-fix kernel using saved column values. Kept-cell tile masks are precomputed so that cells which must stay fixed keep their values. The cost is extra kernels, more shared memory and more code, and the fused path only applies to single-device, even-sized levels without ghosts.

```diff
diff --git a/geometricmultigridpressuresolver_amd/csrc/mgps_internal.h b/geometricmultigridpressuresolver_amd/csrc/mgps_internal.h
--- a/geometricmultigridpressuresolver_amd/csrc/mgps_internal.h
+++ b/geometricmultigridpressuresolver_amd/csrc/mgps_internal.h
@@ -236,6 +236,12 @@
 int launchRestrictY(void *stream, const GridP &coarse, float *coarseOut, const float *rzx, const GridP &fine);
 int launchResidualEdgePlanes(void *stream, const GridP &g, float *r, const float *x, const float *b);
 int launchRestrictXY(void *stream, const GridP &coarse, float *coarseOut, const float *rz);
+bool downFusedFits(const GridP &fine);
+size_t keptTileWords(const GridP &g);
+int launchKeptTiles(void *stream, const GridP &g, const uint32_t *keep, unsigned long long *keptT);
+size_t downFusedColumnFloats(const GridP &fine);
+int launchDownFused(void *stream, const GridP &fine, float *out, float *rz, const float *x, const float *b, float omega, const int32_t *edges, int nedges,
+                    const uint32_t *keep, const unsigned long long *keptT, float *colX);
 bool mixedPrecisionShapeOk(int nx, int ny, int nz);
 int launchStencilMixed(void *stream, StencilOp op, const GridP &g, void *outH, const void *xH, const float *b, float omega, const MixScale &ms,
                        double *dotPartials = nullptr, unsigned *nparts = nullptr);
diff --git a/geometricmultigridpressuresolver_amd/csrc/mgps_kernels.hip b/geometricmultigridpressuresolver_amd/csrc/mgps_kernels.hip
--- a/geometricmultigridpressuresolver_amd/csrc/mgps_kernels.hip
+++ b/geometricmultigridpressuresolver_amd/csrc/mgps_kernels.hip
@@ -794,6 +794,239 @@
     storeXFolded(keepIf(wr, live), rz + size_t(K) * (sz >> 1), offX, storeX, false, seam + size_t(K) * sl.planeFloats(), seamOff, seamW);
 }
 
+__device__ __forceinline__ unsigned gLoadWord(const uint32_t *base, unsigned idx) { return *(const MGPS_GLOBAL_AS uint32_t *)((const MGPS_GLOBAL_AS char *)base + idx * 4u); }
+__device__ __forceinline__ void gStore1(float *base, unsigned cell, float v) { *(MGPS_GLOBAL_AS float *)((MGPS_GLOBAL_AS char *)base + cell * 4u) = v; }
+__global__ __launch_bounds__(64 * kPlaneRows, 8) void jacobiResidualZKernel(GridP g, float *out, float *__restrict__ rz, const float *__restrict__ x,
+                                                                           const float *__restrict__ b, float omega, unsigned nbx, unsigned nby, int zc,
+                                                                           const int32_t *__restrict__ blocks, float *__restrict__ seam,
+                                                                           const uint32_t *__restrict__ keep, const unsigned long long *__restrict__ keptT,
+                                                                           float *__restrict__ colX)
+{
+    __shared__ float plane[2][kPlaneBufFloats];
+    __shared__ float smooth[2][kPlaneBufFloats];
+    const PlaneTile t = planeTile(g, nbx, nby, zc, blocks);
+    const bool live = t.live, valid = t.valid, rowTop = t.rowTop, rowBot = t.rowBot, colL = t.colL, colR = t.colR;
+    const size_t sz = size_t(t.sz);
+    const int k0 = t.k0, k1 = t.k1;
+    const int ks = max(k0 - 1, 0), ke = min(k1, g.nz - 1);
+    const float4 zero4 = make_float4(0.f, 0.f, 0.f, 0.f);
+    for (int q = threadIdx.x; q < 2 * kPlaneBufFloats / 4; q += 64 * kPlaneRows) reinterpret_cast<float4 *>(&smooth[0][0])[q] = zero4;
+    const unsigned offL = unsigned(t.jc) * unsigned(g.nx) + unsigned(min(max(t.ic, g.xlo), max(g.xhi - 4, g.xlo)));
+    float *const mine0 = plane[0] + (t.ty + 1) * kPlanePitch + 4 + t.lane * 4;
+    float *const smooth0 = smooth[0] + (t.ty + 1) * kPlanePitch + 4 + t.lane * 4;
+    const unsigned offHy = (rowTop && t.jc > 0) ? offL - unsigned(g.nx) : (rowBot && t.jc < g.ny - 1) ? offL + unsigned(g.nx) : offL;
+    const int p0 = ks - 1;
+    {
+        const float4 xm = gLoad4(t.planeOf(x, p0 - 1), offL);
+        *reinterpret_cast<float4 *>(mine0 + kPlaneBufFloats) = keepIf(xm, live);
+    }
+    const float *xk = t.planeOf(x, p0);
+    float4 xc = gLoad4(xk, offL);
+    float4 xp = gLoad4(t.planeOf(x, p0 + 1), offL);
+    float4 hy = gLoad4(xk, offHy);
+    const bool useHx = live && t.hasHx();
+    const unsigned offHx = t.offHx(useHx, offL);
+    float hx = gLoad1(xk, offHx);
+    constexpr float w0 = 0.125f, w1 = 0.375f, w2 = 0.375f, w3 = 0.125f;
+    float accPrev[4] = {0.f, 0.f, 0.f, 0.f}, accCur[4] = {0.f, 0.f, 0.f, 0.f};
+    const unsigned rowX = t.rowS * (unsigned(g.nx) >> 1) + t.bx * 128u;
+    const bool storeX = t.i < g.nx && t.j < g.ny && t.ic >= g.xlo - 4 && t.ic < g.xhi + 4;
+    const bool seamL = colL && t.bx > 0, seamR = colR && t.i + 4 < g.nx;
+    const bool seamW = valid && (seamL || seamR);
+    const SeamLayout sl = seamLayout(g.nx, g.ny);
+    auto storeFolded = [&](int K, bool nt) {
+        const float4 v = keepIf(make_float4(accPrev[0], accPrev[1], accPrev[2], accPrev[3]), valid);
+        storeXFolded(v, scalarBase(rz + size_t(K) * (sz >> 1)), rowX + 2u * laneHere(), storeX, nt, scalarBase(seam + size_t(K) * sl.planeFloats()),
+                     colL ? sl.entry(t.rowS, t.bx, 1u) : sl.entry(t.rowS, t.bx + 1u, 0u), seamW);
+    };
+    auto inGrid = [&](int k) { return min(max(k, 0), g.nz - 1); };
+    const unsigned long long *const pt = g.plainT;
+    unsigned long long pw = pt ? plainWord64(pt, t.plainIdx(inGrid(p0))) : 0ull;
+    unsigned long long kw = plainWord64(keptT, t.plainIdx(inGrid(p0)));
+    float4 bPrev = zero4;
+    unsigned lcPrev = 0x01010101u * unsigned(MGPS_EXTERIOR_CELL);
+    auto opq = [](unsigned v) {
+        asm volatile("" : "+v"(v));
+        return v;
+    };
+    int buf = 0;
+    for (int kk = p0 - 1; kk <= ke; ++kk) {
+        const int p = kk + 1, pc = inGrid(p);
+        float *me = mine0 + buf * kPlaneBufFloats;
+        xc = keepIf(xc, live);
+        stagePlane(me, t, xc, keepIf(hy, live), hx, useHx);
+        const size_t cb = size_t(pc) * sz;
+        const float *bk = scalarBase(b + cb);
+        const uint8_t *lk = scalarBase(g.lab + cb);
+        const float *xn = t.planeOf(x, p + 1), *xq2 = t.planeOf(x, p + 2);
+        unsigned lcw = 0u;
+        if (!plainLane(pw)) lcw = gLoadCodesWnt(lk, opq(offL));
+        if (pt) pw = plainWord64(pt, t.plainIdx(inGrid(p + 1)));
+        const float4 bc = gLoad4nt(bk, opq(offL));
+        float4 kept4 = zero4;
+        unsigned nib = 0u;
+        if (plainLane(kw)) {
+            const unsigned q = unsigned(cb & 31u) + offL;
+            nib = (gLoadWord(scalarBase(keep + (cb >> 5)), q >> 5) >> (q & 31u)) & 15u;
+            kept4 = gLoad4(scalarBase(out + cb), opq(offL));
+        }
+        kw = plainWord64(keptT, t.plainIdx(inGrid(p + 1)));
+        const float hxn = gLoad1(xn, opq(offHx));
+        float4 hyn = hy;
+        if (rowTop || rowBot) hyn = gLoad4(xn, opq(offHy));
+        const float4 xq = gLoad4(xq2, opq(offL));
+        __syncthreads();
+        const StagedPlane n = readStaged(me, mine0 + (buf ^ 1) * kPlaneBufFloats);
+        float res[4];
+        simpleQuad<OP_JACOBI>(n.xl, xc, n.xr, n.ym, n.yp, n.zm, xp, bc, lcw, omega, res);
+        if (valid && p >= k0 && p < k1) {
+            float *op = scalarBase(out + size_t(p) * sz);
+            if (!nib) gStore4nt(op, opq(offL), make_float4(res[0], res[1], res[2], res[3]));
+            else {
+#pragma unroll
+                for (int e = 0; e < 4; ++e)
+                    if (!(nib & (1u << e))) gStore1(scalarBase(op + e), opq(offL), res[e]);
+            }
+        }
+        const float4 sp = keepIf(make_float4((nib & 1u) ? kept4.x : res[0], (nib & 2u) ? kept4.y : res[1], (nib & 4u) ? kept4.z : res[2], (nib & 8u) ? kept4.w : res[3]), live);
+        if (colX && seamW && p >= k0 && p < k1) {
+            const bool simple = simpleCell(colL ? (lcw & 255u) : (lcw >> 24));
+            gStore2(scalarBase(colX + (size_t(p) * size_t(g.ny) + t.rowS) * (sl.nseam * 4u)), colL ? t.bx * 4u - 2u : t.bx * 4u,
+                    make_float2(colL ? sp.x : sp.w, simple ? 1.f : 0.f));
+        }
+        float *sm = smooth0 + buf * kPlaneBufFloats;
+        if (kk >= ks) {
+            const float *sc = smooth0 + (buf ^ 1) * kPlaneBufFloats;
+            const StagedPlane m = readStaged(sc, sm);
+            const float4 xs = *reinterpret_cast<const float4 *>(sc);
+            *reinterpret_cast<float4 *>(sm) = sp;
+            float r[4];
+            simpleQuad<OP_RESIDUAL>(m.xl, xs, m.xr, m.ym, m.yp, m.zm, sp, bPrev, lcPrev, 0.f, r);
+            const int k = kk;
+            if (k & 1) {
+#pragma unroll
+                for (int e = 0; e < 4; ++e) {
+                    accPrev[e] = accCur[e] + w2 * r[e];
+                    accCur[e] = w0 * r[e];
+                }
+            } else {
+#pragma unroll
+                for (int e = 0; e < 4; ++e) {
+                    accPrev[e] += w3 * r[e];
+                    accCur[e] += w1 * r[e];
+                }
+                if (k >= k0 + 2) storeFolded((k >> 1) - 1, true);
+            }
+        } else {
+            *reinterpret_cast<float4 *>(sm) = sp;
+        }
+        bPrev = bc;
+        lcPrev = lcw;
+        xc = xp;
+        xp = xq;
+        hy = hyn;
+        hx = hxn;
+        buf ^= 1;
+    }
+    if (k1 == g.nz) storeFolded((g.nz >> 1) - 1, false);
+}
+
+constexpr size_t colXFloats(int nx, int ny, int nz) { return size_t(nz) * ny * seamLayout(nx, ny).nseam * 4u; }
+__global__ __launch_bounds__(64 * kPlaneRows) void downSeamFixKernel(GridP g, float *__restrict__ rz, float *__restrict__ seam, const float *__restrict__ xs,
+                                                                    const float *__restrict__ colX, unsigned nbx, unsigned nby, int zc,
+                                                                    const int32_t *__restrict__ blocks)
+{
+    PlaneCoords t;
+    planeCoords(t, g, blocks ? unsigned(blocks[blockIdx.x]) : blockIdx.x, nbx, nby, zc);
+    const size_t sy = size_t(g.nx), sz = sy * g.ny;
+    const SeamLayout sl = seamLayout(g.nx, g.ny);
+    const int nK = (t.k1 - t.k0) >> 1, K0 = t.k0 >> 1;
+    const float wz[4] = {0.125f, 0.375f, 0.375f, 0.125f};
+    const int j0 = int(t.by) * kPlaneRows;
+    {
+        const int i = t.i;
+        const bool mine = i < g.nx && i >= g.xlo && i < g.xhi;
+        const bool storeX = i < g.nx && i >= g.xlo - 4 && i < g.xhi + 4;
+        const bool seamL = t.lane == 0 && t.bx > 0, seamR = t.lane == kWave - 1 && i + 4 < g.nx;
+        for (int task = t.ty; task < 2 * ((nK + 1) >> 1); task += kPlaneRows) {
+            const int side = task & 1, Ka = K0 + 2 * (task >> 1), nKa = min(2, K0 + nK - Ka);
+            const int j = side ? j0 + kPlaneRows - 1 : j0, jn = side ? j + 1 : j - 1;
+            if (side ? jn >= g.ny : j == 0) continue;
+            float4 tq[6];
+#pragma unroll
+            for (int c = 0; c < 6; ++c) {
+                const int k = 2 * Ka - 1 + c;
+                tq[c] = make_float4(0.f, 0.f, 0.f, 0.f);
+                if (!mine || k < 0 || k >= g.nz || c >= 2 * nKa + 2) continue;
+                const size_t cell = size_t(k) * sz + size_t(j) * sy + size_t(i);
+                const uchar4 lc = codes4(*reinterpret_cast<const unsigned *>(g.lab + cell));
+                const float4 xn = *reinterpret_cast<const float4 *>(xs + size_t(k) * sz + size_t(jn) * sy + size_t(i));
+                tq[c] = make_float4(simpleCell(lc.x) ? xn.x : 0.f, simpleCell(lc.y) ? xn.y : 0.f, simpleCell(lc.z) ? xn.z : 0.f, simpleCell(lc.w) ? xn.w : 0.f);
+            }
+#pragma unroll
+            for (int q = 0; q < 2; ++q) {
+                if (q >= nKa) break;
+                const int K = Ka + q;
+                float4 v = make_float4(0.f, 0.f, 0.f, 0.f);
+#pragma unroll
+                for (int c = 0; c < 4; ++c) {
+                    v.x += wz[c] * tq[2 * q + c].x;
+                    v.y += wz[c] * tq[2 * q + c].y;
+                    v.z += wz[c] * tq[2 * q + c].z;
+                    v.w += wz[c] * tq[2 * q + c].w;
+                }
+                const float2 o = make_float2(foldX4(fromLeftLane(v.w), v.x, v.y, v.z), foldX4(v.y, v.z, v.w, fromRightLane(v.x)));
+                if (storeX) {
+                    float2 *e = reinterpret_cast<float2 *>(rz + size_t(K) * (sz >> 1) + size_t(j) * (sy >> 1) + size_t(i >> 1));
+                    const float2 old = *e;
+                    *e = make_float2(old.x + o.x, old.y + o.y);
+                }
+                if (mine && (seamL || seamR)) {
+                    float4 *e = reinterpret_cast<float4 *>(seam + size_t(K) * sl.planeFloats() + (seamL ? sl.entry(unsigned(j), t.bx, 1u) : sl.entry(unsigned(j), t.bx + 1u, 0u)));
+                    const float4 old = *e;
+                    *e = make_float4(old.x + v.x, old.y + v.y, old.z + v.z, old.w + v.w);
+                }
+            }
+        }
+    }
+    __syncthreads();
+    const int tid = threadIdx.x;
+    if (colX && tid < 2 * kPlaneRows * nK) {
+        const int side = tid & 1, j = j0 + ((tid >> 1) & (kPlaneRows - 1)), K = K0 + tid / (2 * kPlaneRows);
+        const int i = int(t.bx) * kPlaneCols + (side ? kPlaneCols - 1 : 0);
+        const int iq = i & ~3;
+        const unsigned s = t.bx + unsigned(side);
+        if (j < g.ny && (side ? i + 1 < g.nx : i > 0) && iq >= g.xlo && iq < g.xhi) {
+            float v = 0.f;
+#pragma unroll
+            for (int c = 0; c < 4; ++c) {
+                const int k = 2 * K - 1 + c;
+                if (k < 0 || k >= g.nz) continue;
+                const float4 e = *reinterpret_cast<const float4 *>(colX + ((size_t(k) * g.ny + size_t(j)) * sl.nseam + (s - 1u)) * 4u);
+                v += wz[c] * (side ? (e.y != 0.f ? e.z : 0.f) : (e.w != 0.f ? e.x : 0.f));
+            }
+            float *e = seam + size_t(K) * sl.planeFloats() + (side ? sl.entry(unsigned(j), s, 0u) + 3u : sl.entry(unsigned(j), s, 1u));
+            *e += v;
+        }
+    }
+}
+
+__global__ __launch_bounds__(256) void keptTilesKernel(const uint32_t *__restrict__ keep, unsigned nx, unsigned nbx, size_t rows, unsigned long long *__restrict__ keptT)
+{
+    const size_t t = size_t(blockIdx.x) * blockDim.x + threadIdx.x;
+    if (t >= rows * nbx) return;
+    const size_t row = t / nbx;
+    const unsigned tile = unsigned(t - row * nbx);
+    unsigned long long v = 0ull;
+    for (unsigned lane = 0; lane < 64u; ++lane) {
+        const unsigned i = tile * unsigned(kPlaneCols) + 4u * lane;
+        if (i >= nx) break;
+        const size_t c = row * nx + i;
+        if ((keep[c >> 5] >> (c & 31)) & 15u) v |= 1ull << lane;
+    }
+    keptT[t] = v;
+}
+
 template <int OP, bool DOT = false>
 __global__ void stencilScalarKernel(GridP g, float *__restrict__ out, const float *__restrict__ x,
                                     const float *__restrict__ b, float omega, double *__restrict__ dotPartials = nullptr)
@@ -2827,6 +3060,34 @@
         for (int phase = 0; phase < 4; ++phase) residualZGeneralKernel<<<blocksFor(size_t(fine.nbnd), 256), 256, 0, s>>>(fine, rz, x, b, phase);
     return int(hipGetLastError());
 }
+bool downFusedFits(const GridP &fine) { return fine.nbnd == 0 && fine.planeZc >= 4 && (fine.planeZc & 1) == 0 && (fine.nz & 1) == 0 && !fine.ghostLo && !fine.ghostHi; }
+int launchDownFused(void *stream, const GridP &fine, float *out, float *rz, const float *x, const float *b, float omega, const int32_t *edges, int nedges,
+                    const uint32_t *keep, const unsigned long long *keptT, float *colX)
+{
+    if (!downFusedFits(fine) || !keep || !keptT || (!colX && downFusedColumnFloats(fine) > 0)) return int(hipErrorInvalidValue);
+    const int zc = fine.planeZc;
+    const PlaneTiles pt = planeTiles(fine.nx, fine.ny, fine.nz, zc);
+    hipStream_t s = static_cast<hipStream_t>(stream);
+    const bool list = fine.planeBlocks != nullptr;
+    const unsigned nb = list ? unsigned(fine.nplaneBlocks) : unsigned(pt.count());
+    const int32_t *blocks = list ? fine.planeBlocks : nullptr;
+    float *seam = rz + rzxGridFloats(fine);
+    if (nb > 0) {
+        jacobiResidualZKernel<<<nb, 64 * kPlaneRows, 0, s>>>(fine, out, rz, x, b, omega, pt.nbx, pt.nby, zc, blocks, seam, keep, keptT, colX);
+        downSeamFixKernel<<<nb, 64 * kPlaneRows, 0, s>>>(fine, rz, seam, out, colX, pt.nbx, pt.nby, zc, blocks);
+    }
+    if (list && nedges > 0) residualZEdgeKernel<true><<<unsigned(nedges), 64 * kPlaneRows, 0, s>>>(fine, rz, out, b, pt.nbx, pt.nby, zc, edges, seam);
+    return int(hipGetLastError());
+}
+size_t downFusedColumnFloats(const GridP &fine) { return colXFloats(fine.nx, fine.ny, fine.nz); }
+size_t keptTileWords(const GridP &g) { return size_t(g.ny) * g.nz * planeTiles(g.nx, g.ny, g.nz, 0).nbx; }
+int launchKeptTiles(void *stream, const GridP &g, const uint32_t *keep, unsigned long long *keptT)
+{
+    const unsigned nbx = planeTiles(g.nx, g.ny, g.nz, 0).nbx;
+    const size_t rows = size_t(g.ny) * g.nz;
+    keptTilesKernel<<<blocksFor(rows * nbx, 256), 256, 0, static_cast<hipStream_t>(stream)>>>(keep, unsigned(g.nx), nbx, rows, keptT);
+    return int(hipGetLastError());
+}
 int launchRestrictXY(void *stream, const GridP &coarse, float *coarseOut, const float *rz)
 {
     int kc = 16;
diff --git a/geometricmultigridpressuresolver_amd/csrc/mgps_solver.hip b/geometricmultigridpressuresolver_amd/csrc/mgps_solver.hip
--- a/geometricmultigridpressuresolver_amd/csrc/mgps_solver.hip
+++ b/geometricmultigridpressuresolver_amd/csrc/mgps_solver.hip
@@ -58,6 +58,8 @@
     float *rz = nullptr;
     uint8_t *snapTile = nullptr;
     uint32_t *keepBits = nullptr;
+    unsigned long long *keptT = nullptr;
+    float *seamCols = nullptr;
     struct BoxHalo {
         int32_t *sendIdx[2] = {nullptr, nullptr}, *recvIdx[2] = {nullptr, nullptr};
         int nsend[2] = {0, 0}, nrecv[2] = {0, 0};
@@ -411,6 +413,8 @@
         (void)cacheFree(L.bandBoxes.list);
         (void)cacheFree(L.planeFlags);
         (void)cacheFree(L.keepBits);
+        (void)cacheFree(L.keptT);
+        (void)cacheFree(L.seamCols);
         (void)cacheFree(L.snapTile);
         (void)cacheFree(L.rz);
         (void)cacheFree(L.rzEdges);
@@ -685,18 +689,33 @@
     MGPS_LAUNCH(h, launchMarkClosure(h->stream, L.g, L.bandBoxes, L.keepBits));
     return MGPS_OK;
 }
+int ensureKeptTiles(mgps_solver *h, int l)
+{
+    DevLevel &L = h->lv[l];
+    if (L.keptT) return MGPS_OK;
+    MGPS_TRY(ensureKeepBits(h, l));
+    MGPS_TRY(devAlloc(h, &L.keptT, keptTileWords(L.g), false));
+    MGPS_LAUNCH(h, launchKeptTiles(h->stream, L.g, L.keepBits, L.keptT));
+    return MGPS_OK;
+}
 
 enum StrokeForm {
     SF_GS_SNAPSHOT,
     SF_THREE_LAUNCH,
     SF_FRONT,
     SF_PROLONG_FUSED,
+    SF_DOWN_FUSED,
     SF_FIRST_FUSED,
     SF_GENERIC,
 };
 
-StrokeForm strokeForm(const mgps_solver *h, int l, bool down, const float *cur, const float *other, const float *b, bool dot)
-{
+bool residualRestrictXFolded(const mgps_solver *h, int l);
+StrokeForm strokeForm(const mgps_solver *h, int l, bool down, const float *cur, const float *other, const float *b, bool dot, bool fromGuess = false)
+{
+    static const int fuseDown = [] {
+        const char *e = getenv("MGPS_FUSE_DOWN");
+        return !e ? -1 : (e[0] == '0' ? 0 : 1);
+    }();
     static const bool gsSnapshots = [] {
         const char *e = getenv("MGPS_GS_SNAPSHOT");
         return !(e && e[0] == '0');
@@ -714,6 +733,9 @@
     if (!down && fuseUp != 0 && (fuseUp > 0 || planes) && l + 1 < int(h->lv.size()) && !dot && !h->dist && !h->tailOfSlabRun && h->opt.precision == 0 &&
         !L.boxForm && prolongJacobiPlaneFits(L.g) && boxPlaneFits(L.d))
         return SF_PROLONG_FUSED;
+    if (down && fromGuess && fuseDown != 0 && (fuseDown > 0 || planes) && l + 1 < int(h->lv.size()) && !dot && !h->dist && !h->tailOfSlabRun &&
+        h->opt.precision == 0 && !L.boxForm && L.g.planeBlocks && downFusedFits(L.g) && (L.d.cells() & 31) == 0 && residualRestrictXFolded(h, l))
+        return SF_DOWN_FUSED;
     if (!dot && !sweepTimed(h, l) && !stageTimingOn(h) && !h->dist && L.d.cells() <= (size_t(1) << 24) && stencilKernelOf(L.g) == 1 && (L.d.cells() & 31) == 0)
         return SF_FRONT;
     return SF_THREE_LAUNCH;
@@ -748,25 +770,30 @@
     }();
     return allowed && residualRestrictFuses(h, l) && residualRestrictXFolds(h->lv[l].g);
 }
+int ensureRz(mgps_solver *h, int l, bool xfold)
+{
+    DevLevel &F = h->lv[l];
+    if (F.rz) return MGPS_OK;
+    MGPS_TRY(devAlloc(h, &F.rz, xfold ? rzxFloats(F.g) : F.d.cells() / 2, true));
+    if (F.g.planeBlocks) {
+        if (!F.planeFlags) {
+            MGPS_TRY(devAlloc(h, &F.planeFlags, planeBlockCount(F.g), true));
+            MGPS_LAUNCH(h, launchPlaneBlockFlags(h->stream, F.g, F.planeFlags));
+        }
+        std::vector<uint8_t> flags(planeBlockCount(F.g));
+        MGPS_HIP(h, hipMemcpyAsync(flags.data(), F.planeFlags, flags.size(), hipMemcpyDeviceToHost, h->stream));
+        MGPS_HIP(h, hipStreamSynchronize(h->stream));
+        const std::vector<int32_t> edges = planeBlockEdges(F.g, flags);
+        F.nrzEdges = int(edges.size());
+        if (F.nrzEdges) MGPS_TRY(devUpload(h, &F.rzEdges, edges));
+    }
+    return MGPS_OK;
+}
 int residualRestrict(mgps_solver *h, int l, const float *x, const float *rhs, float *out = nullptr)
 {
     DevLevel &F = h->lv[l], &C = h->lv[l + 1];
     const bool xfold = residualRestrictXFolded(h, l);
-    if (!F.rz) {
-        MGPS_TRY(devAlloc(h, &F.rz, xfold ? rzxFloats(F.g) : F.d.cells() / 2, true));
-        if (F.g.planeBlocks) {
-            if (!F.planeFlags) {
-                MGPS_TRY(devAlloc(h, &F.planeFlags, planeBlockCount(F.g), true));
-                MGPS_LAUNCH(h, launchPlaneBlockFlags(h->stream, F.g, F.planeFlags));
-            }
-            std::vector<uint8_t> flags(planeBlockCount(F.g));
-            MGPS_HIP(h, hipMemcpyAsync(flags.data(), F.planeFlags, flags.size(), hipMemcpyDeviceToHost, h->stream));
-            MGPS_HIP(h, hipStreamSynchronize(h->stream));
-            const std::vector<int32_t> edges = planeBlockEdges(F.g, flags);
-            F.nrzEdges = int(edges.size());
-            if (F.nrzEdges) MGPS_TRY(devUpload(h, &F.rzEdges, edges));
-        }
-    }
+    MGPS_TRY(ensureRz(h, l, xfold));
     {
         StageScope scope(h, ST_RESIDUAL, l);
         const bool cut = h->dist && (F.g.ghostLo || F.g.ghostHi);
@@ -942,6 +969,7 @@
     case SF_FRONT: return frontStroke(h, l, cur, other, b, xZero);
     case SF_PROLONG_FUSED: return prolongFusedStroke(h, l, cur, other, b, coarse);
     case SF_FIRST_FUSED: return firstFusedStroke(h, l, cur, other, b, down, dot);
+    case SF_DOWN_FUSED:
     case SF_GENERIC: break;
     }
     {
@@ -964,6 +992,28 @@
     const float nan = std::numeric_limits<float>::quiet_NaN();
     MGPS_LAUNCH(h, launchScale(h->stream, h->lv[l].g, a, nan));
     MGPS_LAUNCH(h, launchScale(h->stream, h->lv[l].g, b2, nan));
+    return MGPS_OK;
+}
+
+int fusedDownStroke(mgps_solver *h, int l, float *&cur, float *&other, const float *b, float *out = nullptr)
+{
+    DevLevel &L = h->lv[l], &C = h->lv[l + 1];
+    MGPS_TRY(ensureKeptTiles(h, l));
+    MGPS_TRY(ensureRz(h, l, true));
+    if (!L.seamCols && downFusedColumnFloats(L.g) > 0) MGPS_TRY(devAlloc(h, &L.seamCols, downFusedColumnFloats(L.g), true));
+    MGPS_TRY(poisonSpares(h, l, other, other));
+    {
+        StageScope scope(h, ST_BAND, l);
+        MGPS_LAUNCH(h, launchBandBox(h->stream, L.g, L.bandBoxes, true, cur, b, nullptr, L.r, h->opt.jacobi_weight));
+        MGPS_LAUNCH(h, launchBandBox(h->stream, L.g, L.bandBoxes, false, L.r, b, other, nullptr, h->opt.jacobi_weight, false, MixScale{}, nullptr, nullptr, true));
+    }
+    {
+        StageScope scope(h, ST_RESIDUAL, l);
+        MGPS_LAUNCH(h, launchDownFused(h->stream, L.g, other, L.rz, cur, b, h->opt.jacobi_weight, L.rzEdges, L.nrzEdges, L.keepBits, L.keptT, L.seamCols));
+    }
+    std::swap(cur, other);
+    StageScope scope(h, ST_RESTRICT, l);
+    MGPS_LAUNCH(h, launchRestrictY(h->stream, C.g, out ? out : C.b, L.rz, L.g));
     return MGPS_OK;
 }
 
@@ -1018,7 +1068,7 @@
     return smoothStroke(h, l, cur, other, b, true, true, dot, zero);
 }
 
-int cycleLevels(mgps_solver *h, int first, float *&x, float *spare, const float *b, bool poll)
+int cycleLevels(mgps_solver *h, int first, float *&x, float *spare, const float *b, bool poll, bool restricted = false)
 {
     const int nlv = int(h->lv.size()), bottom = nlv - 1;
     std::vector<float *> cur(nlv, nullptr), other(nlv, nullptr);
@@ -1036,6 +1086,7 @@
             }
             MGPS_TRY(downStrokeFromZero(h, l, cur[l], other[l], rhsOf(l), true, false));
         }
+        if (l == first && restricted) continue;
         if (residualRestrictFuses(h, l)) {
             MGPS_TRY(residualRestrict(h, l, cur[l], rhsOf(l)));
             continue;
@@ -1076,9 +1127,11 @@
     }
     const bool hasBottom = nlv > 1;
     float *cur = x, *other = h->lv[0].tmp;
-    if (useInitialGuess) MGPS_TRY(smoothStroke(h, 0, cur, other, b, true, false, h->gatherDot && !hasBottom));
+    const bool fused = useInitialGuess && hasBottom && strokeForm(h, 0, true, cur, other, b, false, true) == SF_DOWN_FUSED;
+    if (fused) MGPS_TRY(fusedDownStroke(h, 0, cur, other, b));
+    else if (useInitialGuess) MGPS_TRY(smoothStroke(h, 0, cur, other, b, true, false, h->gatherDot && !hasBottom));
     else MGPS_TRY(downStrokeFromZero(h, 0, cur, other, b, ownGrid, h->gatherDot && !hasBottom));
-    if (hasBottom) MGPS_TRY(cycleLevels(h, 0, cur, other, b, !h->dist && !h->tailOfSlabRun));
+    if (hasBottom) MGPS_TRY(cycleLevels(h, 0, cur, other, b, !h->dist && !h->tailOfSlabRun, fused));
     if (cur != x)
         MGPS_HIP(h, hipMemcpyAsync(x, cur, h->lv[0].d.cells() * sizeof(float), hipMemcpyDeviceToDevice, h->stream));
     if (h->gatherDot) MGPS_LAUNCH(h, launchFoldDot(h->stream, h->dotPartials, h->dotUsed, h->dotTarget ? h->dotTarget : h->resultDev));
@@ -4255,6 +4308,12 @@
         return rc;
     }
     case 15: src = L.g.plainQ, n = L.g.plainQ ? (L.d.cells() / 4 + 31) / 32 : 0; break;
+    case 17:
+        if (strokeForm(h, level, true, nullptr, nullptr, nullptr, false, true) == SF_DOWN_FUSED) {
+            MGPS_TRY(ensureKeptTiles(h, level));
+            src = L.keptT, n = keptTileWords(L.g), elem = 8;
+        } else src = nullptr, n = 0, elem = 8;
+        break;
     case 16: src = L.g.plainT, n = L.g.plainT ? size_t(L.d.ny) * L.d.nz * planeTiles(L.d.nx, L.d.ny, L.d.nz, 0).nbx : 0, elem = 8; break;
     default: return failH(h, MGPS_ERR_INVALID_ARGUMENT, "mgps_level_array: unknown array");
     }
@@ -4286,6 +4345,13 @@
 try {
     if (!h || !fused || level < 0 || level >= int(h->lv.size())) return MGPS_ERR_INVALID_ARGUMENT;
     *fused = strokeForm(h, level, false, nullptr, nullptr, nullptr, false) == SF_PROLONG_FUSED ? 1 : 0;
+    return MGPS_OK;
+}
+MGPS_API_CATCH(h)
+int mgps_down_stroke_fused(const mgps_solver *h, int level, int *fused)
+try {
+    if (!h || !fused || level < 0 || level >= int(h->lv.size())) return MGPS_ERR_INVALID_ARGUMENT;
+    *fused = strokeForm(h, level, true, nullptr, nullptr, nullptr, false, true) == SF_DOWN_FUSED ? 1 : 0;
     return MGPS_OK;
 }
 MGPS_API_CATCH(h)
@@ -4497,6 +4563,25 @@
     MGPS_TRY(applyOp(h, OP_RESIDUAL, fine_level, F.r, const_cast<float *>(x_dev), b_dev, true));
     MGPS_TRY(exchangeGhosts(h, fine_level, F.r));
     MGPS_LAUNCH(h, launchRestrict(h->stream, h->lv[fine_level + 1].g, coarse_dev, F.r));
+    return MGPS_OK;
+}
+MGPS_API_CATCH(h)
+
+int mgps_down_stroke(mgps_solver *h, int fine_level, float *x_dev, float *coarse_dev, const float *b_dev)
+try {
+    MGPS_TRY(checkLevel(h, fine_level + 1, "mgps_down_stroke"));
+    if (fine_level < 0 || !coarse_dev || !x_dev || !b_dev) return failH(h, MGPS_ERR_INVALID_ARGUMENT, "mgps_down_stroke: bad arguments");
+    DevLevel &F = h->lv[fine_level];
+    if (h->dist || h->opt.precision != 0 || !F.tmp) return failH(h, MGPS_ERR_INVALID_ARGUMENT, "mgps_down_stroke: single-device fp32 solvers only");
+    MGPS_LAUNCH(h, launchZero(h->stream, coarse_dev, h->lv[fine_level + 1].d.cells()));
+    float *cur = x_dev, *other = F.tmp;
+    if (strokeForm(h, fine_level, true, cur, other, b_dev, false, true) == SF_DOWN_FUSED) MGPS_TRY(fusedDownStroke(h, fine_level, cur, other, b_dev, coarse_dev));
+    else {
+        MGPS_TRY(smoothStroke(h, fine_level, cur, other, b_dev, true, false));
+        if (!residualRestrictFuses(h, fine_level)) return failH(h, MGPS_ERR_INVALID_ARGUMENT, "mgps_down_stroke: the level does not take the residual pair");
+        MGPS_TRY(residualRestrict(h, fine_level, cur, b_dev, coarse_dev));
+    }
+    if (cur != x_dev) MGPS_HIP(h, hipMemcpyAsync(x_dev, cur, F.d.cells() * sizeof(float), hipMemcpyDeviceToDevice, h->stream));
     return MGPS_OK;
 }
 MGPS_API_CATCH(h)
diff --git a/geometricmultigridpressuresolver_amd/solver.py b/geometricmultigridpressuresolver_amd/solver.py
--- a/geometricmultigridpressuresolver_amd/solver.py
+++ b/geometricmultigridpressuresolver_amd/solver.py
@@ -232,7 +232,7 @@
     LEVEL_ARRAYS = {"codes": (0, np.uint8), "band": (1, np.int32), "band_diag": (2, np.uint8), "rows": (3, np.float32), "chunks": (4, np.int32),
                     "plane_blocks": (5, np.int32), "pure_even": (6, np.int32), "pure_odd": (7, np.int32), "mixed_even": (8, np.int32),
                     "mixed_odd": (9, np.int32), "tile_bnd_start": (10, np.int32), "box_info": (11, np.int32), "box_list": (12, np.uint32),
-                    "box_general": (13, np.int32), "plain_quads": (15, np.uint32), "plain_tiles": (16, np.uint64)}
+                    "box_general": (13, np.int32), "plain_quads": (15, np.uint32), "plain_tiles": (16, np.uint64), "kept_tiles": (17, np.uint64)}
 
     def level_array(self, level, name):
         which, dt = self.LEVEL_ARRAYS[name]
@@ -295,6 +295,9 @@
 
     def residualDownsample(self, destination, solution, rhs, fine_level=0):
         check(lib().mgps_residual_downsample(self.h, fine_level, self._g(destination, fine_level + 1), self._g(solution, fine_level), self._g(rhs, fine_level)), self.h)
+
+    def downStroke(self, solution, destination, rhs, fine_level=0):
+        check(lib().mgps_down_stroke(self.h, fine_level, self._g(solution, fine_level), self._g(destination, fine_level + 1), self._g(rhs, fine_level)), self.h)
 
     def upsampleAndAdd(self, destination, source, fine_level=0):
         check(lib().mgps_upsample_add(self.h, fine_level, self._g(destination, fine_level), self._g(source, fine_level + 1)), self.h)
@@ -419,6 +422,11 @@
         check(lib().mgps_up_stroke_fused(self.h, int(level), C.byref(f)), self.h)
         return bool(f.value)
 
+    def down_stroke_fused(self, level=0):
+        f = C.c_int()
+        check(lib().mgps_down_stroke_fused(self.h, int(level), C.byref(f)), self.h)
+        return bool(f.value)
+
     def stencil_kernel(self, level=0):
         k = C.c_int()
         check(lib().mgps_stencil_kernel(self.h, int(level), C.byref(k)), self.h)
diff --git a/include/mgps.h b/include/mgps.h
--- a/include/mgps.h
+++ b/include/mgps.h
@@ -130,6 +130,7 @@
 int mgps_residual(mgps_solver *h, int level, float *r_dev, const float *x_dev, const float *b_dev);
 int mgps_downsample(mgps_solver *h, int fine_level, float *coarse_dev, const float *fine_dev);
 int mgps_residual_downsample(mgps_solver *h, int fine_level, float *coarse_dev, const float *x_dev, const float *b_dev);
+int mgps_down_stroke(mgps_solver *h, int fine_level, float *x_dev, float *coarse_dev, const float *b_dev);
 
 int mgps_upsample_add(mgps_solver *h, int fine_level, float *fine_dev, const float *coarse_dev);
 int mgps_coarse_solve(mgps_solver *h, float *x_dev, const float *b_dev);
@@ -206,6 +207,7 @@
 int mgps_residual_restrict_fused(const mgps_solver *h, int level, int *fused);
 int mgps_residual_restrict_xfolded(const mgps_solver *h, int level, int *xfolded);
 int mgps_up_stroke_fused(const mgps_solver *h, int level, int *fused);
+int mgps_down_stroke_fused(const mgps_solver *h, int level, int *fused);
 int64_t mgps_overlapped_exchanges(const mgps_solver *h);
 int64_t mgps_exchange_count(const mgps_solver *h);
 int mgps_copy_to_host(mgps_solver *h, void *dst_host, const void *src_dev, size_t bytes);
```

After: 130.9, median of 6. +7.1%, better.
